# RolandFaure/Hairsplitter

Hardware: AMD Instinct MI355X
Metric: aligned read-bp/sec through call_variants+separate_reads (higher is better)
Workload: dtype u8

## Files before the change

hairsplitter_amd/csrc/hs_driver.cpp:

```cpp
#include "hs_driver.h"

#include <sys/prctl.h>
#include <algorithm>
#include <atomic>
#include <chrono>
#include <ctime>
#include <cstdio>
#include <cstdlib>
#include <cstring>
#include <fstream>
#include <iostream>
#include <sstream>
#include <condition_variable>
#include <functional>
#include <mutex>
#include <thread>

namespace hs {

int host_threads();

namespace {

double now_ms() {
    return std::chrono::duration<double, std::milli>(std::chrono::steady_clock::now().time_since_epoch()).count();
}

class WorkerPool {
public:
    static WorkerPool& get() { static thread_local WorkerPool* p = new WorkerPool(); return *p; }
    void run(int n, int n_threads, const std::function<void(int)>& f) {
        if (n <= 0) return;
        if (n_threads <= 1 || n == 1) { for (int i = 0; i < n; ++i) f(i); return; }
        std::lock_guard<std::mutex> serial(run_mu_);
        ensure(std::min(n_threads, n) - 1);
        {
            std::lock_guard<std::mutex> g(mu_);
            job_ = &f; n_ = n; next_.store(0); active_ = std::min((int)workers_.size(), std::min(n_threads, n) - 1); pending_ = active_; gen_++;
            grain_ = std::max(1, n / (8 * (active_ + 1)));
        }
        cv_.notify_all();
        const int grain = grain_;
        for (;;) { const int i = next_.fetch_add(grain); if (i >= n) break; for (int k = i; k < std::min(n, i + grain); ++k) f(k); }
        std::unique_lock<std::mutex> g(mu_);
        done_cv_.wait(g, [&] { return pending_ == 0; });
        job_ = nullptr;
    }
private:
    void ensure(int want) {
        want = std::min(want, 255);
        while ((int)workers_.size() < want) {
            const int id = (int)workers_.size();
            workers_.emplace_back([this, id] { ::prctl(PR_SET_NAME, "hs-pool", 0, 0, 0); loop(id); });
            workers_.back().detach();
        }
    }
    void loop(int id) {
        uint64_t seen = 0;
        for (;;) {
            const std::function<void(int)>* job; int n, grain;
            {
                std::unique_lock<std::mutex> g(mu_);
                cv_.wait(g, [&] { return gen_ != seen && id < active_; });
                seen = gen_; job = job_; n = n_; grain = grain_;
            }
            for (;;) { const int i = next_.fetch_add(grain); if (i >= n) break; for (int k = i; k < std::min(n, i + grain); ++k) (*job)(k); }
            {
                std::lock_guard<std::mutex> g(mu_);
                if (--pending_ == 0) done_cv_.notify_one();
            }
        }
    }
    std::mutex mu_, run_mu_;
    std::condition_variable cv_, done_cv_;
    std::vector<std::thread> workers_;
    const std::function<void(int)>* job_ = nullptr;
    std::atomic<int> next_{0};
    int n_ = 0, active_ = 0, pending_ = 0, grain_ = 1;
    uint64_t gen_ = 0;
};

class SharedPool {
public:
    static SharedPool& get() { static SharedPool* p = new SharedPool(); return *p; }
    static bool on() { static const bool v = []() { const char* e = std::getenv("HS_SHARED_POOL"); return e && e[0] == '1'; }(); return v; }
    void run(int n, int n_threads, const std::function<void(int)>& f) {
        if (n <= 0) return;
        if (n_threads <= 1 || n == 1) { for (int i = 0; i < n; ++i) f(i); return; }
        Job job;
        job.f = &f; job.n = n;
        {
            std::lock_guard<std::mutex> g(mu_);
            ensure();
            job.grain = std::max(1, n / (8 * (std::min(n_threads, (int)workers_.size() + 1))));
            jobs_.push_back(&job);
        }
        cv_.notify_all();
        for (;;) { const int i = job.next.fetch_add(job.grain); if (i >= n) break; const int e = std::min(n, i + job.grain); for (int k = i; k < e; ++k) f(k); job.done.fetch_add(e - i); }
        std::unique_lock<std::mutex> g(mu_);
        jobs_.erase(std::find(jobs_.begin(), jobs_.end(), &job));
        done_cv_.wait(g, [&] { return job.done.load() >= n; });
    }
private:
    struct Job { const std::function<void(int)>* f = nullptr; int n = 0, grain = 1; std::atomic<int> next{0}, done{0}; };
    void ensure() {
        static const int want = []() { const char* e = std::getenv("HS_POOL_THREADS"); const int v = e ? std::atoi(e) : 0; return v > 0 ? v : host_threads(); }();
        while ((int)workers_.size() < want) { workers_.emplace_back([this] { ::prctl(PR_SET_NAME, "hs-spool", 0, 0, 0); loop(); }); workers_.back().detach(); }
    }
    void loop() {
        std::unique_lock<std::mutex> g(mu_);
        for (;;) {
            Job* job = nullptr;
            for (Job* j : jobs_) if (j->next.load(std::memory_order_relaxed) < j->n) { job = j; break; }
            if (!job) { cv_.wait(g); continue; }
            const int i = job->next.fetch_add(job->grain);
            if (i >= job->n) continue;
            const int n = job->n, e = std::min(n, i + job->grain);
            const std::function<void(int)>* f = job->f;
            g.unlock();
            for (int k = i; k < e; ++k) (*f)(k);
            const bool last = job->done.fetch_add(e - i) + (e - i) >= n;
            g.lock();
            if (last) done_cv_.notify_all();
        }
    }
    std::mutex mu_;
    std::condition_variable cv_, done_cv_;
    std::vector<std::thread> workers_;
    std::vector<Job*> jobs_;
};

template <class F>
void parallel_for(int n, int n_threads, F f) {
    std::function<void(int)> fn = f;
    if (SharedPool::on()) SharedPool::get().run(n, n_threads, fn); else WorkerPool::get().run(n, n_threads, fn);
}

template <class T> T* dup_vec(const std::vector<T>& v) {
    T* p = (T*)std::malloc(std::max<size_t>(1, v.size()) * sizeof(T));
    if (!v.empty()) std::memcpy(p, v.data(), v.size() * sizeof(T));
    return p;
}

}

void hs_parallel_for(int n, int n_threads, const std::function<void(int)>& f) { if (SharedPool::on()) SharedPool::get().run(n, n_threads, f); else WorkerPool::get().run(n, n_threads, f); }

int host_threads() {
    static const int n = [] {
        long q = -1, per = 100000;
        if (FILE* f = std::fopen("/sys/fs/cgroup/cpu.max", "r")) { char a[32]; if (std::fscanf(f, "%31s %ld", a, &per) == 2 && std::strcmp(a, "max") != 0) q = std::atol(a); std::fclose(f); }
        int t = (int)std::thread::hardware_concurrency();
        if (q > 0 && per > 0) t = std::min<int>(t, (int)((q + per - 1) / per));
        return std::max(1, std::min(t, 32));
    }();
    return n;
}

void free_cv_result(hs_cv_result* r) {
    if (!r) return;
    std::free(r->mean_distance); std::free(r->depth); std::free(r->snp_off); std::free(r->snp_pos); std::free(r->snp_ref);
    std::free(r->snp_alt); std::free(r->snp_n_ref); std::free(r->snp_n_alt); std::free(r->col_off);
    if (!r->entries_borrowed) { std::free(r->col_idx); std::free(r->col_code); }
    std::free(r);
}
namespace {
struct LabelBlockHeader { uint64_t magic; size_t cap; char pad[48]; };
constexpr uint64_t kLabelMagic = 0x48534c4142454c53ull;
constexpr size_t kLabelKeepMin = 8u << 20, kLabelKeepBlocks = 4;
std::mutex g_label_mu;
std::vector<LabelBlockHeader*> g_label_free;
}

int32_t* sr_labels_alloc(size_t n_labels) {
    const size_t need = std::max<size_t>(1, n_labels) * sizeof(int32_t);
    {
        std::lock_guard<std::mutex> g(g_label_mu);
        for (size_t i = 0; i < g_label_free.size(); ++i) {
            LabelBlockHeader* h = g_label_free[i];
            if (h->cap >= need && h->cap / 2 <= need) { g_label_free.erase(g_label_free.begin() + (long)i); return (int32_t*)(h + 1); }
        }
    }
    const size_t cap = need >= kLabelKeepMin ? need + need / 8 : need;
    LabelBlockHeader* h = (LabelBlockHeader*)std::malloc(sizeof(LabelBlockHeader) + cap);
    if (!h) return nullptr;
    h->magic = kLabelMagic; h->cap = cap;
    return (int32_t*)(h + 1);
}

void sr_labels_free(int32_t* labels) {
    if (!labels) return;
    LabelBlockHeader* h = (LabelBlockHeader*)labels - 1;
    if (h->magic != kLabelMagic) { std::free(labels); return; }
    if (h->cap >= kLabelKeepMin) {
        std::lock_guard<std::mutex> g(g_label_mu);
        if (g_label_free.size() < kLabelKeepBlocks) { g_label_free.push_back(h); return; }
    }
    std::free(h);
}

void free_sr_result(hs_sr_result* r) {
    if (!r) return;
    std::free(r->win_off); std::free(r->win_start); std::free(r->win_end); std::free(r->label_off); sr_labels_free(r->labels);
    std::free(r);
}

static std::atomic<double> g_trace_origin{0.0};
void set_trace_origin() { g_trace_origin.store(std::chrono::duration<double, std::milli>(std::chrono::steady_clock::now().time_since_epoch()).count()); }
double trace_ms() { return std::chrono::duration<double, std::milli>(std::chrono::steady_clock::now().time_since_epoch()).count() - g_trace_origin.load(); }
namespace {
struct Laps {
    bool on = std::getenv("HS_TIMING") != nullptr;
    bool cpu = on && std::string(std::getenv("HS_TIMING")) == "cpu";
    bool abs_ = on && std::string(std::getenv("HS_TIMING")) == "abs";
    double t = now_ms(), c = cpu_ms();
    std::string line;
    const char* tag;
    explicit Laps(const char* t_) : tag(t_) {}
    static double cpu_ms() { timespec ts; clock_gettime(CLOCK_THREAD_CPUTIME_ID, &ts); return ts.tv_sec * 1e3 + ts.tv_nsec * 1e-6; }
    void lap(const char* what) {
        if (!on) return;
        const double n = now_ms();
        char buf[96];
        if (abs_) std::snprintf(buf, sizeof buf, " %s @%.2f", what, n - g_trace_origin.load());
        else if (cpu) { const double cn = cpu_ms(); std::snprintf(buf, sizeof buf, " %s %.2f/%.2f", what, n - t, cn - c); c = cn; }
        else std::snprintf(buf, sizeof buf, " %s %.2f", what, n - t);
        line += buf; t = n;
    }
    ~Laps() { if (on) std::fprintf(stderr, "[hs timing] %s laps (ms) thread %zu:%s\n", tag, std::hash<std::thread::id>()(std::this_thread::get_id()) % 1000, line.c_str()); }
};
}

int cv_pileup(CvDeviceOps& dev, const CvMeta& b, CvSelection& sel) {
    const double t_start = now_ms();
    for (int k = 0; k < 4; ++k) sel.k_ms[k] = 0;
    sel.rec_stats.assign((size_t)b.n_rec * 4, 0);
    if (int rc = dev.pileup(sel.rec_stats, sel.k_ms)) return rc;
    sel.t_device_ms = now_ms() - t_start; sel.t_host_ms = 0;
    return HS_OK;
}

int cv_run_range(CvDeviceOps& dev, const CvMeta& b, const std::vector<int32_t>& rec_stats, int c0, int c1, float automatic_snp_threshold, int n_threads,
                 hs_cv_result** out, bool resident, const std::function<void(const float*)>* on_mean_distance) {
    if (n_threads <= 0) n_threads = host_threads();
    if (c0 < 0 || c1 > b.n_contigs || c0 > c1) { set_error("cv_run_range: bad contig range"); return HS_EINVAL; }
    const int C = c1 - c0;
    const double t_start = now_ms();
    float k_ms[4] = {0, 0, 0, 0};
    float k_ms_k4 = 0;
    std::vector<ContigCvResult> res((size_t)C);
    const bool derive = rec_stats.empty() && b.n_rec > 0;
    std::vector<int32_t> min_reads((size_t)(derive ? 0 : C), 5);
    for (int c = 0; c < C; ++c) {
        const int gc = c0 + c;
        ContigCvResult& o = res[(size_t)c];
        if (!derive) {
            int64_t nerr = 0, nlen = 0;
            for (int r = b.contig_rec_off[(size_t)gc]; r < b.contig_rec_off[(size_t)gc + 1]; ++r) { nerr += rec_stats[(size_t)r * 4 + 1]; nlen += rec_stats[(size_t)r * 4 + 2]; }
            o.mean_distance = mean_distance_from_counts(nerr, nlen);
            min_reads[(size_t)c] = o.mean_distance < 0.015 ? 3 : 5;
        }
        const int64_t L = b.contig_off[(size_t)gc + 1] - b.contig_off[(size_t)gc];
        const int64_t entries = b.pile_off[(size_t)b.contig_rec_off[(size_t)gc + 1]] - b.pile_off[(size_t)b.contig_rec_off[(size_t)gc]];
        o.depth = (float)((double)entries / (double)L);
    }
    CvCandidates cand;
    float k_ms_x[3] = {0, 0, 0};
    if (int rc = dev.extract_candidates(c0, c1, min_reads, automatic_snp_threshold, cand, k_ms_x, true)) return rc;
    k_ms[1] = k_ms_x[0]; k_ms[2] = k_ms_x[1] + k_ms_x[2];
    if (derive) {
        if ((int)cand.contig_mean_distance.size() != C) { set_error("cv_run_range: the device interface did not report the contigs' mean distances"); return HS_EINVAL; }
        for (int c = 0; c < C; ++c) res[(size_t)c].mean_distance = cand.contig_mean_distance[(size_t)c];
    }
    if (on_mean_distance) { std::vector<float> md((size_t)C); for (int c = 0; c < C; ++c) md[(size_t)c] = res[(size_t)c].mean_distance; (*on_mean_distance)(md.data()); }
    const double t_dev_done = now_ms();
    Laps laps("cv glue");
    std::vector<int64_t> cand_base((size_t)C + 1, 0);
    for (int c = 0; c < C; ++c) cand_base[(size_t)c + 1] = cand_base[(size_t)c] + cand.contig_n_cand[(size_t)c];
    if (cand_base[(size_t)C] != cand.n_cand) { set_error("cv_run_range: candidate counts do not add up"); return HS_EINVAL; }

    std::vector<CvContigState*> cst((size_t)C, nullptr);
    for (int c = 0; c < C; ++c) cst[(size_t)c] = cv_state_new();
    std::vector<int32_t> n_reads_of((size_t)C);
    parallel_for(C, n_threads, [&](int c) {
        const int gc = c0 + c;
        const int r0 = b.contig_rec_off[(size_t)gc];
        const int n_reads_c = b.contig_rec_off[(size_t)gc + 1] - r0;
        n_reads_of[(size_t)c] = n_reads_c;
        cv_phase_begin(*cst[(size_t)c], n_reads_c, cand.contig_n_cand[(size_t)c], res[(size_t)c].mean_distance, res[(size_t)c]);
    });
    laps.lap("begin");
    const bool some_on_device = (int)cand.contig_on_device.size() == C;
    auto on_device = [&](int c) { return some_on_device && cand.contig_on_device[(size_t)c] != 0; };
    bool host_has_bits = cand.bits != nullptr || cand.n_cand == 0;
    auto candidates_of = [&](int c) {
        CandidateSet cs;
        cs.n = cand.contig_n_cand[(size_t)c];
        cs.rec = cand.rec + cand_base[(size_t)c]; cs.bits = cand.bits + cand_base[(size_t)c]; cs.words = cand.words;
        if (cand.idx) { cs.off = cand.off + cand_base[(size_t)c]; cs.idx = cand.idx; cs.code = cand.code; }
        return cs;
    };
    static const bool loop_b_pairs = []() { const char* e = std::getenv("HS_LOOP_B_PAIRS_ON_DEVICE"); return e && e[0] != '0'; }();
    const bool pairs_on_device = loop_b_pairs && dev.has_partition_pairs();
    const bool ranked = (int)b.rank_of.size() == b.n_rec && (int)b.orig_of.size() == b.n_rec;
    auto walk_on_host = [&](int c) {
        const int r0 = b.contig_rec_off[(size_t)(c0 + c)];
        cv_phase_a_host(*cst[(size_t)c], candidates_of(c), b.rec_pos.data() + r0, ranked ? b.rank_of.data() + r0 : nullptr, ranked ? b.orig_of.data() + r0 : nullptr);
        if (!pairs_on_device) cv_phase_b(*cst[(size_t)c], res[(size_t)c]);
    };
    std::vector<int> host_list, dev_list;
    for (int c = 0; c < C; ++c) (on_device(c) ? dev_list : host_list).push_back(c);
    std::stable_sort(host_list.begin(), host_list.end(), [&](int x, int y) { return cand.contig_n_cand[(size_t)x] > cand.contig_n_cand[(size_t)y]; });
    if (!host_list.empty() && !host_has_bits) { set_error("cv_run_range: the device interface handed no bit sets of the candidate columns"); return HS_EINVAL; }
    parallel_for((int)host_list.size(), n_threads, [&](int k) { walk_on_host(host_list[(size_t)k]); });
    laps.lap("loop_a_host");
    int n_dev_failed = 0;
    if (!dev_list.empty()) {
        CvLoopAResult la;
        if (int rc = dev.collect_partitions(la)) return rc;
        if ((int)la.failed.size() != C || (int)la.part_base.size() != C + 1) { set_error("cv_run_range: the device interface did not hand over the partitions of its contigs"); return HS_EINVAL; }
        laps.lap("loop_a_device");
        std::vector<int> redo;
        for (int c : dev_list) if (la.failed[(size_t)c]) redo.push_back(c);
        n_dev_failed = (int)redo.size();
        if (!redo.empty()) {
            if (int rc = dev.fetch_candidates(cand)) return rc;
            if (cand.n_cand > 0 && !cand.bits) { set_error("cv_run_range: the device interface handed no bit sets of the candidate columns"); return HS_EINVAL; }
        }
        std::stable_sort(dev_list.begin(), dev_list.end(), [&](int x, int y) { return cand.contig_n_cand[(size_t)x] > cand.contig_n_cand[(size_t)y]; });
        parallel_for((int)dev_list.size(), n_threads, [&](int k) {
            const int c = dev_list[(size_t)k];
            if (la.failed[(size_t)c]) { walk_on_host(c); return; }
            const int r0 = b.contig_rec_off[(size_t)(c0 + c)];
            cv_phase_a_import(*cst[(size_t)c], b.rec_pos.data() + r0, (int)(la.part_base[(size_t)c + 1] - la.part_base[(size_t)c]), la.rec + la.part_base[(size_t)c], la.bits, la.cnt,
                              ranked ? b.rank_of.data() + r0 : nullptr, ranked ? b.orig_of.data() + r0 : nullptr);
            if (!pairs_on_device) cv_phase_b(*cst[(size_t)c], res[(size_t)c]);
        });
    }
    if (pairs_on_device) {
        std::vector<int32_t> n_surv((size_t)C, 0);
        parallel_for(C, n_threads, [&](int c) { n_surv[(size_t)c] = cv_loop_b_survivors(*cst[(size_t)c]); });
        std::vector<int64_t> part_first((size_t)C + 1, 0), elem_first((size_t)C + 1, 0), pair_first((size_t)C + 1, 0);
        for (int c = 0; c < C; ++c) {
            part_first[(size_t)c + 1] = part_first[(size_t)c] + n_surv[(size_t)c];
            elem_first[(size_t)c + 1] = elem_first[(size_t)c] + (int64_t)n_surv[(size_t)c] * n_reads_of[(size_t)c];
            pair_first[(size_t)c + 1] = pair_first[(size_t)c] + (int64_t)n_surv[(size_t)c] * (n_surv[(size_t)c] - 1) / 2;
        }
        std::vector<int8_t> pstate((size_t)elem_first[(size_t)C]);
        std::vector<int32_t> pmore((size_t)elem_first[(size_t)C]), pless((size_t)elem_first[(size_t)C]), part_n((size_t)part_first[(size_t)C]);
        std::vector<int64_t> part_off((size_t)part_first[(size_t)C]);
        std::vector<int32_t> pair_a((size_t)pair_first[(size_t)C]), pair_b((size_t)pair_first[(size_t)C]);
        parallel_for(C, n_threads, [&](int c) {
            const int S = n_surv[(size_t)c], N = n_reads_of[(size_t)c];
            cv_export_survivors(*cst[(size_t)c], pstate.data() + elem_first[(size_t)c], pmore.data() + elem_first[(size_t)c], pless.data() + elem_first[(size_t)c]);
            for (int k = 0; k < S; ++k) { part_off[(size_t)part_first[(size_t)c] + k] = elem_first[(size_t)c] + (int64_t)k * N; part_n[(size_t)part_first[(size_t)c] + k] = N; }
            int64_t q = pair_first[(size_t)c];
            for (int j = 1; j < S; ++j) for (int i = 0; i < j; ++i, ++q) { pair_a[(size_t)q] = (int32_t)(part_first[(size_t)c] + i); pair_b[(size_t)q] = (int32_t)(part_first[(size_t)c] + j); }
        });
        std::vector<int32_t> table;
        if (int rc = dev.partition_pairs(pstate, pmore, pless, part_off, part_n, pair_a, pair_b, cv_three_sigma_table(), table)) return rc;
        parallel_for(C, n_threads, [&](int c) { cv_phase_b(*cst[(size_t)c], res[(size_t)c], table.data() + 8 * pair_first[(size_t)c]); });
        if (std::getenv("HS_TIMING")) std::fprintf(stderr, "[hs timing] cv loop B: %ld partition pairs of %ld gated partitions from the device\n", (long)pair_first[(size_t)C], (long)part_first[(size_t)C]);
    }
    if (std::getenv("HS_TIMING") && !dev_list.empty()) std::fprintf(stderr, "[hs timing] cv loop A: %zu of %d contigs on the device (%d handed back), %zu on the host\n", dev_list.size(), C, n_dev_failed, host_list.size());
    laps.lap("phase_ab");
    CvSnpSet snps;
    {
        CvPartitionTest t;
        t.part_off.assign((size_t)C + 1, 0);
        t.contig_n_reads.resize((size_t)C);
        std::vector<int64_t> st_base((size_t)C + 1, 0);
        for (int c = 0; c < C; ++c) {
            t.contig_n_reads[(size_t)c] = b.contig_rec_off[(size_t)(c0 + c) + 1] - b.contig_rec_off[(size_t)(c0 + c)];
            const int nf = cv_final_partitions(*cst[(size_t)c]);
            t.part_off[(size_t)c + 1] = t.part_off[(size_t)c] + nf;
            st_base[(size_t)c + 1] = st_base[(size_t)c] + (int64_t)nf * t.contig_n_reads[(size_t)c];
        }
        t.part_state.resize((size_t)st_base[(size_t)C]); t.part_state_off.resize((size_t)t.part_off[(size_t)C]);
        parallel_for(C, n_threads, [&](int c) {
            cv_export_partitions(*cst[(size_t)c], t.part_state.data() + st_base[(size_t)c], st_base[(size_t)c], t.part_state_off.data() + t.part_off[(size_t)c]);
            cv_state_free(cst[(size_t)c]);
        });
        laps.lap("k4_prep");
        if (int rc = dev.finish_columns(t, !resident, snps, &k_ms_k4)) return rc;
        laps.lap("k4+snps");
    }
    const double t_glue_done = now_ms();

    hs_cv_result* R = (hs_cv_result*)std::calloc(1, sizeof(hs_cv_result));
    R->n_contigs = C;
    std::vector<float> md((size_t)C), dp((size_t)C);
    std::vector<int64_t> snp_off((size_t)C + 1, 0);
    float total_error = 0; int n_err_contigs = 0;
    for (int c = 0; c < C; ++c) {
        md[(size_t)c] = res[(size_t)c].mean_distance; dp[(size_t)c] = res[(size_t)c].depth;
        if (res[(size_t)c].mean_distance > 0) { total_error += res[(size_t)c].mean_distance; n_err_contigs++; }
        snp_off[(size_t)c + 1] = snp_off[(size_t)c] + snps.contig_n_snp[(size_t)c];
    }
    const int64_t S = snps.n_snp, E = snps.n_entries;
    if (snp_off[(size_t)C] != S) { set_error("cv_run_range: SNP counts do not add up"); return HS_EINVAL; }
    R->snp_pos = (int32_t*)std::malloc(std::max<int64_t>(1, S) * sizeof(int32_t));
    R->snp_ref = (uint8_t*)std::malloc(std::max<int64_t>(1, S));
    R->snp_alt = (uint8_t*)std::malloc(std::max<int64_t>(1, S));
    R->snp_n_ref = (int32_t*)std::malloc(std::max<int64_t>(1, S) * sizeof(int32_t));
    R->snp_n_alt = (int32_t*)std::malloc(std::max<int64_t>(1, S) * sizeof(int32_t));
    R->col_off = (int64_t*)std::malloc((S + 1) * sizeof(int64_t));
    const bool with_entries = snps.idx != nullptr || E == 0;
    R->col_idx = with_entries ? (int32_t*)std::malloc(std::max<int64_t>(1, E) * sizeof(int32_t)) : nullptr;
    R->col_code = with_entries ? (uint8_t*)std::malloc(std::max<int64_t>(1, E)) : nullptr;
    R->n_columns_extracted = cand.n_columns;
    R->n_columns_downloaded = cand.n_cand;
    R->n_columns_downloaded_late = cand.n_tie;
    {
        const int nb = (int)std::min<int64_t>(std::max<int64_t>(1, S / 4096), 4 * (int64_t)n_threads);
        parallel_for(nb, n_threads, [&](int blk) {
            const int64_t a = S * blk / nb, e = S * (blk + 1) / nb;
            for (int64_t s = a; s < e; ++s) {
                const hs_colrec& r = snps.rec[s];
                R->snp_pos[s] = r.pos; R->snp_ref[s] = r.k0; R->snp_alt[s] = r.k1; R->snp_n_ref[s] = r.c0; R->snp_n_alt[s] = r.c1;
            }
            if (S) std::memcpy(R->col_off + a, snps.off + a, (size_t)(e - a) * sizeof(int64_t));
            if (with_entries && e > a) {
                const int64_t ea = snps.off[a], ee = snps.off[e];
                std::memcpy(R->col_idx + ea, snps.idx + ea, (size_t)(ee - ea) * sizeof(int32_t));
                std::memcpy(R->col_code + ea, snps.code + ea, (size_t)(ee - ea));
            }
        });
        R->col_off[S] = E;
        if (S == 0) R->col_off[0] = 0;
    }
    laps.lap("result");
    R->mean_distance = dup_vec(md); R->depth = dup_vec(dp); R->snp_off = dup_vec(snp_off);
    R->error_rate = total_error / n_err_contigs;
    R->n_contigs_with_error_rate = n_err_contigs;
    R->t_kernel_ms[0] = k_ms[0]; R->t_kernel_ms[1] = k_ms[1]; R->t_kernel_ms[2] = k_ms[2]; R->t_kernel_ms[3] = k_ms[3]; R->t_kernel_k4_ms = k_ms_k4;
    R->t_device_ms = t_dev_done - t_start;
    R->t_host_ms = now_ms() - t_dev_done;
    if (std::getenv("HS_TIMING"))
        std::fprintf(stderr, "[hs timing] cv range [%d,%d): columns + candidates %.2f ms, host glue %.2f ms (up to the SNPs %.2f); columns: %lld extracted, %lld candidates, %lld with tied counts (%lld beyond 16 keys), %lld SNPs\n",
                     c0, c1, t_dev_done - t_start, R->t_host_ms, t_glue_done - t_dev_done, (long long)cand.n_columns,
                     (long long)cand.n_cand, (long long)cand.n_tie, (long long)cand.n_tie_big, (long long)S);
    *out = R;
    return HS_OK;
}


int cv_attach_entries(CvDeviceOps& dev, hs_cv_result* R, int n_threads, bool borrow) {
    if (!R || R->col_idx) return HS_OK;
    const int64_t S = R->snp_off[R->n_contigs], E = R->col_off[S];
    CvSnpSet snps;
    if (int rc = dev.late_entries(snps)) return rc;
    if (E > 0 && (!snps.idx || !snps.code)) return HS_OK;
    if (borrow && E > 0) {
        R->col_idx = const_cast<int32_t*>(snps.idx); R->col_code = const_cast<uint8_t*>(snps.code); R->entries_borrowed = 1;
        return HS_OK;
    }
    R->col_idx = (int32_t*)std::malloc(std::max<int64_t>(1, E) * sizeof(int32_t));
    R->col_code = (uint8_t*)std::malloc(std::max<int64_t>(1, E));
    if (n_threads <= 0) n_threads = host_threads();
    const int nb = (int)std::min<int64_t>(std::max<int64_t>(1, E >> 20), 4 * (int64_t)n_threads);
    parallel_for(nb, n_threads, [&](int blk) {
        const int64_t a = E * blk / nb, e = E * (blk + 1) / nb;
        if (e > a) { std::memcpy(R->col_idx + a, snps.idx + a, (size_t)(e - a) * sizeof(int32_t)); std::memcpy(R->col_code + a, snps.code + a, (size_t)(e - a)); }
    });
    return HS_OK;
}

hs_cv_result* cv_concat_results(hs_cv_result* a, hs_cv_result* b) {
    hs_cv_result* R = (hs_cv_result*)std::calloc(1, sizeof(hs_cv_result));
    const int Ca = a->n_contigs, Cb = b->n_contigs, C = Ca + Cb;
    const int64_t Sa = a->snp_off[Ca], Sb = b->snp_off[Cb], S = Sa + Sb;
    const int64_t Ea = a->col_off[Sa], Eb = b->col_off[Sb], E = Ea + Eb;
    R->n_contigs = C;
    R->mean_distance = (float*)std::malloc(std::max(1, C) * sizeof(float)); R->depth = (float*)std::malloc(std::max(1, C) * sizeof(float));
    R->snp_off = (int64_t*)std::malloc(((size_t)C + 1) * sizeof(int64_t));
    R->snp_pos = (int32_t*)std::malloc(std::max<int64_t>(1, S) * sizeof(int32_t));
    R->snp_ref = (uint8_t*)std::malloc(std::max<int64_t>(1, S)); R->snp_alt = (uint8_t*)std::malloc(std::max<int64_t>(1, S));
    R->snp_n_ref = (int32_t*)std::malloc(std::max<int64_t>(1, S) * sizeof(int32_t)); R->snp_n_alt = (int32_t*)std::malloc(std::max<int64_t>(1, S) * sizeof(int32_t));
    R->col_off = (int64_t*)std::malloc(((size_t)S + 1) * sizeof(int64_t));
    const bool with_entries = (a->col_idx || Ea == 0) && (b->col_idx || Eb == 0);
    R->col_idx = with_entries ? (int32_t*)std::malloc(std::max<int64_t>(1, E) * sizeof(int32_t)) : nullptr;
    R->col_code = with_entries ? (uint8_t*)std::malloc(std::max<int64_t>(1, E)) : nullptr;
    float total_error = 0; int n_err = 0;
    auto put = [&](const hs_cv_result* r, int cbase, int64_t sbase, int64_t ebase) {
        const int Cr = r->n_contigs; const int64_t Sr = r->snp_off[Cr], Er = r->col_off[Sr];
        for (int c = 0; c < Cr; ++c) {
            R->mean_distance[cbase + c] = r->mean_distance[c]; R->depth[cbase + c] = r->depth[c];
            if (r->mean_distance[c] > 0) { total_error += r->mean_distance[c]; n_err++; }
            R->snp_off[cbase + c] = sbase + r->snp_off[c];
        }
        if (Sr) {
            std::memcpy(R->snp_pos + sbase, r->snp_pos, (size_t)Sr * sizeof(int32_t)); std::memcpy(R->snp_ref + sbase, r->snp_ref, (size_t)Sr); std::memcpy(R->snp_alt + sbase, r->snp_alt, (size_t)Sr);
            std::memcpy(R->snp_n_ref + sbase, r->snp_n_ref, (size_t)Sr * sizeof(int32_t)); std::memcpy(R->snp_n_alt + sbase, r->snp_n_alt, (size_t)Sr * sizeof(int32_t));
        }
        for (int64_t q = 0; q < Sr; ++q) R->col_off[sbase + q] = ebase + r->col_off[q];
        if (with_entries && Er) { std::memcpy(R->col_idx + ebase, r->col_idx, (size_t)Er * sizeof(int32_t)); std::memcpy(R->col_code + ebase, r->col_code, (size_t)Er); }
        R->t_device_ms += r->t_device_ms; R->t_host_ms += r->t_host_ms;
        for (int k = 0; k < 4; ++k) R->t_kernel_ms[k] += r->t_kernel_ms[k];
        R->t_kernel_k4_ms += r->t_kernel_k4_ms;
        R->n_columns_extracted += r->n_columns_extracted; R->n_columns_downloaded += r->n_columns_downloaded; R->n_columns_downloaded_late += r->n_columns_downloaded_late;
    };
    put(a, 0, 0, 0); put(b, Ca, Sa, Ea);
    R->snp_off[C] = S; R->col_off[S] = E;
    R->error_rate = total_error / n_err; R->n_contigs_with_error_rate = n_err;
    free_cv_result(a); free_cv_result(b);
    return R;
}

int cv_run(CvDeviceOps& dev, const CvMeta& b, float automatic_snp_threshold, int n_threads, hs_cv_result** out) {
    CvSelection sel;
    if (int rc = cv_pileup(dev, b, sel)) return rc;
    if (int rc = cv_run_range(dev, b, sel.rec_stats, 0, b.n_contigs, automatic_snp_threshold, n_threads, out)) return rc;
    hs_cv_result* R = *out;
    R->t_kernel_ms[0] = sel.k_ms[0]; R->t_kernel_ms[3] = sel.k_ms[3];
    R->t_device_ms += sel.t_device_ms; R->t_host_ms += sel.t_host_ms;
    return HS_OK;
}

int sr_run(SrDeviceOps& dev, const hs_sr_contig* contigs, int32_t n_contigs, int32_t window_size, float error_rate,
           int32_t low_memory, uint32_t seed, int32_t n_threads, hs_sr_result** out, SrSparseLabels* sparse, SrWorkspace* keep, SrTaps* taps) {
    Laps laps("sr");
    if (n_threads <= 0) n_threads = host_threads();
    const int C = n_contigs;
    const bool lowmem = low_memory != 0;
    const double t_start = now_ms();
    double dev_ms = 0;
    float k_ms[4] = {0, 0, 0, 0};

    const bool resident = dev.columns_resident();
    std::vector<hs_sr_contig> cs_local(contigs, contigs + C);
    std::vector<SrContigState> st_local;
    if (keep) keep->st.resize((size_t)C); else st_local.resize((size_t)C);
    std::vector<SrContigState>& st = keep ? keep->st : st_local;
    parallel_for(C, n_threads, [&](int c) {
        SrContigState& s = st[(size_t)c];
        s.c = &cs_local[(size_t)c];
        s.N = contigs[c].n_reads;
        s.low_memory_now = lowmem || sr_coverage_above_1000(contigs[c]);
        if (contigs[c].n_snps == 0) { for (SrWindowPlan& old : s.windows) s.spare.push_back(std::move(old)); s.windows.clear(); return; }
        s.words = (contigs[c].n_snps + 63) / 64;
        if (!s.low_memory_now && ((int)s.pos_key.size() != s.N || std::memcmp(s.pos_key.data(), contigs[c].read_start, (size_t)s.N * 4) != 0)) {
            s.pos_key.assign(contigs[c].read_start, contigs[c].read_start + s.N);
            s.pos_orig.resize((size_t)s.N); s.pos_rank.resize((size_t)s.N);
            for (int k = 0; k < s.N; ++k) s.pos_orig[(size_t)k] = k;
            const int32_t* st0 = contigs[c].read_start;
            std::sort(s.pos_orig.begin(), s.pos_orig.end(), [st0](int32_t a, int32_t b2) { return st0[a] != st0[b2] ? st0[a] < st0[b2] : a < b2; });
            for (int k = 0; k < s.N; ++k) s.pos_rank[(size_t)s.pos_orig[(size_t)k]] = k;
        }
        if (s.perm_n != s.N || s.perm_seed != seed) {
            s.perm = shuffled_order(s.N, seed);
            s.rank.resize((size_t)s.N);
            for (int k = 0; k < s.N; ++k) s.rank[(size_t)s.perm[(size_t)k]] = k;
            s.perm_n = s.N; s.perm_seed = seed;
        }
    });

    laps.lap("perm");
    const bool lm_on_device = dev.low_memory_graphs();
    bool matrices_by_position = false;
    CwChain ch;
    std::vector<int64_t> col_base_of_contig((size_t)C, 0);
    {
        SimdiffJob job;
        job.cols = &ch;
        job.contig_snp_base.assign((size_t)C, 0); job.plane_off.assign((size_t)C, 0); job.out_off.assign((size_t)C, 0);
        job.n_reads.assign((size_t)C, 0); job.words.assign((size_t)C, 0); job.plane_n.assign((size_t)C, 0); job.read_base.assign((size_t)C, 0);
        int64_t n_ent = 0, n_col = 0;
        for (int c = 0; c < C; ++c) { n_col += contigs[c].n_snps; if (contigs[c].n_snps) n_ent += contigs[c].col_off[contigs[c].n_snps] - contigs[c].col_off[0]; }
        bool contiguous = n_col > 0;
        {
            const int64_t* off_next = nullptr; const int32_t* idx0 = nullptr; const uint8_t* code0 = nullptr;
            bool first = true;
            for (int c = 0; c < C && contiguous; ++c) {
                const hs_sr_contig& hc = contigs[c];
                if (hc.n_snps == 0) continue;
                if (first) { first = false; idx0 = hc.col_idx; code0 = hc.col_code; if (hc.col_off[0] != 0) contiguous = false; }
                else if (hc.col_idx != idx0 || hc.col_code != code0 || hc.col_off != off_next) contiguous = false;
                off_next = hc.col_off + hc.n_snps;
            }
        }
        if (resident && n_col > 0 && !contiguous) { set_error("sr_run: resident columns need one offset array in contig order"); return HS_EINVAL; }
        int64_t* own_off = nullptr; int32_t* own_idx = nullptr; uint8_t* own_code = nullptr;
        if (contiguous) {
            const hs_sr_contig* first = nullptr;
            for (int c = 0; c < C && !first; ++c) if (contigs[c].n_snps) first = &contigs[c];
            ch.col_off.view(first->col_off, (size_t)n_col + 1);
            if (!resident) { ch.col_idx.view(first->col_idx, (size_t)n_ent); ch.col_code.view(first->col_code, (size_t)n_ent); }
        } else {
            own_off = ch.col_off.alloc((size_t)n_col + 1); own_idx = ch.col_idx.alloc((size_t)n_ent); own_code = ch.col_code.alloc((size_t)n_ent);
            own_off[0] = 0;
        }
        job.snp_ref.resize((size_t)n_col); job.snp_alt.resize((size_t)n_col); job.snp_contig.resize((size_t)n_col);
        std::vector<int64_t> ent_base_of_contig((size_t)C, 0);
        {
            int64_t cb = 0, eb = 0, rows_total = 0;
            for (int c = 0; c < C; ++c) {
                col_base_of_contig[(size_t)c] = cb; ent_base_of_contig[(size_t)c] = eb;
                job.contig_snp_base[(size_t)c] = cb;
                const hs_sr_contig& hc = contigs[c];
                if (hc.n_snps == 0) continue;
                cb += hc.n_snps; eb += hc.col_off[hc.n_snps] - hc.col_off[0];
                if (st[(size_t)c].low_memory_now && !lm_on_device) continue;
                job.plane_off[(size_t)c] = job.plane_total; job.words[(size_t)c] = st[(size_t)c].words; job.plane_n[(size_t)c] = st[(size_t)c].N;
                job.plane_total += (int64_t)st[(size_t)c].N * st[(size_t)c].words;
                job.read_base[(size_t)c] = rows_total; rows_total += st[(size_t)c].N;
                if (st[(size_t)c].low_memory_now) continue;
                job.out_off[(size_t)c] = job.out_total;
                job.n_reads[(size_t)c] = st[(size_t)c].N;
                job.out_total += (int64_t)st[(size_t)c].N * st[(size_t)c].N;
            }
        }
        {
            const bool read_order = false;
            int64_t rows_all = 0;
            for (int c = 0; c < C; ++c) rows_all = std::max<int64_t>(rows_all, job.read_base[(size_t)c] + job.plane_n[(size_t)c]);
            if (!read_order) job.pos_orig.assign((size_t)rows_all, 0);
            if (!read_order) for (int c = 0; c < C; ++c) if (job.plane_n[(size_t)c] > 0 && job.n_reads[(size_t)c] == 0)
                for (int k = 0; k < job.plane_n[(size_t)c]; ++k) job.pos_orig[(size_t)(job.read_base[(size_t)c] + k)] = k;
        }
        parallel_for(C, n_threads, [&](int c) {
            const hs_sr_contig& hc = contigs[c];
            if (hc.n_snps == 0) return;
            const int64_t cb = col_base_of_contig[(size_t)c], e_base = ent_base_of_contig[(size_t)c], o0 = hc.col_off[0];
            if (!contiguous) {
                for (int s = 0; s < hc.n_snps; ++s) own_off[(size_t)(cb + s) + 1] = e_base + hc.col_off[s + 1] - o0;
                const int64_t n = hc.col_off[hc.n_snps] - o0;
                std::memcpy(own_idx + e_base, hc.col_idx + o0, (size_t)n * sizeof(int32_t));
                std::memcpy(own_code + e_base, hc.col_code + o0, (size_t)n);
            }
            if (!job.pos_orig.empty() && job.n_reads[(size_t)c] > 0) {
                if ((int)st[(size_t)c].pos_orig.size() == st[(size_t)c].N) std::memcpy(job.pos_orig.data() + job.read_base[(size_t)c], st[(size_t)c].pos_orig.data(), (size_t)st[(size_t)c].N * 4);
                else for (int k = 0; k < st[(size_t)c].N; ++k) job.pos_orig[(size_t)(job.read_base[(size_t)c] + k)] = k;
            }
            std::memcpy(job.snp_ref.data() + cb, hc.snp_ref, (size_t)hc.n_snps);
            std::memcpy(job.snp_alt.data() + cb, hc.snp_alt, (size_t)hc.n_snps);
            std::fill(job.snp_contig.begin() + cb, job.snp_contig.begin() + cb + hc.n_snps, c);
        });
        laps.lap("columns");
        matrices_by_position = !job.pos_orig.empty();
        const double t0 = now_ms();
        if (int rc = dev.simdiff_columns(job, &k_ms[0])) return rc;
        dev_ms += now_ms() - t0;
    }

    const double t_simdiff_done = now_ms();
    laps.lap("simdiff");
    std::vector<int32_t> fetched_idx; std::vector<uint8_t> fetched_code;
    bool columns_here = !resident;
    auto need_columns = [&]() -> int {
        if (columns_here) return HS_OK;
        const double t0 = now_ms();
        if (int rc = dev.fetch_columns(fetched_idx, fetched_code)) return rc;
        dev_ms += now_ms() - t0;
        for (int c = 0; c < C; ++c) { cs_local[(size_t)c].col_idx = fetched_idx.data(); cs_local[(size_t)c].col_code = fetched_code.data(); }
        ch.col_idx.view(fetched_idx.data(), fetched_idx.size()); ch.col_code.view(fetched_code.data(), fetched_code.size());
        columns_here = true;
        return HS_OK;
    };
    parallel_for(C, n_threads, [&](int c) {
        if (contigs[c].n_snps == 0) return;
        sr_plan_windows(st[(size_t)c], window_size, error_rate, lowmem, !resident);
    });
    laps.lap("plan_windows");
    if (resident) {
        struct WR { int c, w; };
        std::vector<WR> wr;
        for (int c = 0; c < C; ++c)
            for (size_t w = 0; w < st[(size_t)c].windows.size(); ++w) if (st[(size_t)c].windows[w].has_snps) wr.push_back(WR{c, (int)w});
        const size_t W = wr.size();
        std::vector<int64_t> col_a(W), col_b(W), slot_off(W + 1, 0);
        for (size_t i = 0; i < W; ++i) {
            const SrWindowPlan& wp = st[(size_t)wr[i].c].windows[(size_t)wr[i].w];
            col_a[i] = col_base_of_contig[(size_t)wr[i].c] + wp.col_a; col_b[i] = col_base_of_contig[(size_t)wr[i].c] + wp.col_b;
            slot_off[i + 1] = slot_off[i] + (ch.col_off[(size_t)col_a[i] + 1] - ch.col_off[(size_t)col_a[i]]);
        }
        std::vector<int32_t> ids, win_m;
        if (W) {
            const double t0 = now_ms();
            if (int rc = dev.window_masks(col_a, col_b, slot_off, ids, win_m)) return rc;
            dev_ms += now_ms() - t0;
        }
        parallel_for((int)W, n_threads, [&](int i) {
            SrWindowPlan& wp = st[(size_t)wr[(size_t)i].c].windows[(size_t)wr[(size_t)i].w];
            wp.ids.assign(ids.begin() + slot_off[(size_t)i], ids.begin() + slot_off[(size_t)i] + win_m[(size_t)i]);
        });
        laps.lap("window_masks");
    }
    struct WRef { int c, w; };
    std::vector<WRef> wrefs;
    SrWindowSet ws;
    ws.error_rate = error_rate;
    {
        std::vector<uint8_t> lm_dev((size_t)C, 0);
        bool any_lm = false;
        for (int c = 0; c < C; ++c) if (contigs[c].n_snps > 0 && st[(size_t)c].low_memory_now) any_lm = true;
        if (any_lm && lm_on_device) {
            if (int rc = need_columns()) return rc;
            parallel_for(C, n_threads, [&](int c) {
                const hs_sr_contig& hc = cs_local[(size_t)c];
                if (hc.n_snps == 0 || !st[(size_t)c].low_memory_now) return;
                std::vector<int32_t> first((size_t)st[(size_t)c].N, -1), last((size_t)st[(size_t)c].N, -1), cnt((size_t)st[(size_t)c].N, 0);
                for (int s = 0; s < hc.n_snps; ++s)
                    for (int64_t e = hc.col_off[s]; e < hc.col_off[s + 1]; ++e) {
                        const int r = hc.col_idx[e];
                        if (first[(size_t)r] < 0) first[(size_t)r] = s;
                        last[(size_t)r] = s; cnt[(size_t)r]++;
                    }
                bool ok = true;
                for (int r = 0; r < st[(size_t)c].N && ok; ++r) if (cnt[(size_t)r] > 0 && cnt[(size_t)r] != last[(size_t)r] - first[(size_t)r] + 1) ok = false;
                lm_dev[(size_t)c] = ok ? 1 : 0;
            });
        }
        if (any_lm && std::getenv("HS_TIMING")) {
            int n_lm = 0, n_ok = 0;
            for (int c = 0; c < C; ++c) if (contigs[c].n_snps > 0 && st[(size_t)c].low_memory_now) { n_lm++; n_ok += lm_dev[(size_t)c]; }
            std::fprintf(stderr, "[hs timing] sr: %d contigs on the low-memory path, %d of them with graphs from the device\n", n_lm, n_ok);
        }
        std::vector<WRef> lm_w, host_w;
        for (int c = 0; c < C; ++c)
            for (size_t w = 0; w < st[(size_t)c].windows.size(); ++w) {
                if (!st[(size_t)c].windows[w].has_snps) continue;
                (!st[(size_t)c].low_memory_now ? wrefs : (lm_dev[(size_t)c] ? lm_w : host_w)).push_back(WRef{c, (int)w});
            }
        ws.n_matrix_windows = (int32_t)wrefs.size();
        wrefs.insert(wrefs.end(), lm_w.begin(), lm_w.end());
        ws.n_dev_windows = (int32_t)wrefs.size();
        wrefs.insert(wrefs.end(), host_w.begin(), host_w.end());
        ws.ctg_reads.resize((size_t)C);
        for (int c = 0; c < C; ++c) ws.ctg_reads[(size_t)c] = st[(size_t)c].N;
        const size_t W = wrefs.size();
        ws.win_contig.resize(W); ws.win_row0.assign(W + 1, 0); ws.win_final_empty.resize(W);
        for (size_t i = 0; i < W; ++i) {
            SrWindowPlan& wp = st[(size_t)wrefs[i].c].windows[(size_t)wrefs[i].w];
            wp.row0 = ws.win_row0[i];
            ws.win_contig[i] = wrefs[i].c;
            ws.win_final_empty[i] = wp.final_graph_empty ? 1 : 0;
            ws.win_row0[i + 1] = ws.win_row0[i] + (int64_t)wp.ids.size();
        }
        ws.mask_ids.resize((size_t)ws.win_row0[W]);
        parallel_for((int)W, n_threads, [&](int i) {
            const SrWindowPlan& wp = st[(size_t)wrefs[(size_t)i].c].windows[(size_t)wrefs[(size_t)i].w];
            std::copy(wp.ids.begin(), wp.ids.end(), ws.mask_ids.begin() + ws.win_row0[(size_t)i]);
        });
        ws.ctg_rank_off.assign((size_t)C, 0);
        int64_t ro = 0;
        for (int c = 0; c < C; ++c) { ws.ctg_rank_off[(size_t)c] = ro; ro += (int64_t)st[(size_t)c].rank.size(); }
        ws.rank.resize((size_t)ro);
        parallel_for(C, n_threads, [&](int c) { std::copy(st[(size_t)c].rank.begin(), st[(size_t)c].rank.end(), ws.rank.begin() + ws.ctg_rank_off[(size_t)c]); });
        if (matrices_by_position) {
            ws.pos_rank.assign((size_t)ro, 0);
            parallel_for(C, n_threads, [&](int c) {
                const SrContigState& s = st[(size_t)c];
                if (s.rank.empty()) return;
                int32_t* o = ws.pos_rank.data() + ws.ctg_rank_off[(size_t)c];
                if (!s.low_memory_now && (int)s.pos_rank.size() == s.N) std::copy(s.pos_rank.begin(), s.pos_rank.end(), o);
                else for (int k = 0; k < (int)s.rank.size(); ++k) o[k] = k;
            });
        }
        const int n_host = (int)host_w.size();
        if (n_host > 0) {
            if (int rc = need_columns()) return rc;
            std::vector<std::vector<std::vector<int32_t>>> lists((size_t)n_host);
            parallel_for(n_host, n_threads, [&](int i) {
                const WRef& r = wrefs[(size_t)ws.n_dev_windows + (size_t)i];
                sr_build_window_graph_low_memory(st[(size_t)r.c], st[(size_t)r.c].windows[(size_t)r.w], error_rate, lists[(size_t)i]);
            });
            ws.host_off.assign(1, 0);
            for (auto& wl : lists)
                for (auto& row : wl) { ws.host_nbr.insert(ws.host_nbr.end(), row.begin(), row.end()); ws.host_off.push_back((int64_t)ws.host_nbr.size()); }
        }
    }
    laps.lap("window_set");
    int64_t rows_on_host = 0, n_finish_host = 0;
    float k6_ms = 0;
    const bool two_phase = !wrefs.empty() && dev.two_phase_graphs();
    if (!wrefs.empty()) {
        const double t0 = now_ms();
        if (two_phase) { if (int rc = dev.build_graphs_begin(ws, &k6_ms)) return rc; }
        else if (int rc = dev.build_graphs(ws, &rows_on_host, &k6_ms)) return rc;
        dev_ms += now_ms() - t0;
    }
    const double t_plan_done = now_ms();
    laps.lap("build_graphs");

    int64_t n_cw = 0;
    std::vector<int64_t> chain_index(wrefs.size(), -1);
    {
        ch.win_seed_begin.assign(1, 0);
        ch.chain_row0.assign(1, 0);
        ch.finish_on_device = !lowmem;
        for (int c = 0; c < C && ch.finish_on_device; ++c)
            if (contigs[c].n_snps > 0 && !st[(size_t)c].snp_pos_sorted) ch.finish_on_device = false;
        if (ch.finish_on_device) {
            ch.col_pos.reserve(ch.col_off.size());
            for (int c = 0; c < C; ++c) ch.col_pos.insert(ch.col_pos.end(), contigs[c].snp_pos, contigs[c].snp_pos + contigs[c].n_snps);
        }
        for (size_t i = 0; i < wrefs.size(); ++i) {
            const SrWindowPlan& w = st[(size_t)wrefs[i].c].windows[(size_t)wrefs[i].w];
            if (w.local_snps.empty()) continue;
            chain_index[i] = (int64_t)ch.win.size();
            ch.win.push_back((int32_t)i);
            ch.win_seed_begin.push_back(ch.win_seed_begin.back() + (int64_t)w.local_snps.size());
            ch.chain_row0.push_back(ch.chain_row0.back() + (int64_t)w.ids.size());
            n_cw += (int64_t)w.local_snps.size() + 2;
        }
        const size_t Wc = ch.win.size();
        ch.seed_col.resize((size_t)ch.win_seed_begin.back());
        if (ch.finish_on_device) { ch.win_snp_first.resize(Wc); ch.win_snp_last.resize(Wc); ch.win_pos_lo.resize(Wc); ch.win_pos_hi.resize(Wc); }
        parallel_for((int)Wc, n_threads, [&](int k) {
            const size_t i = (size_t)ch.win[(size_t)k];
            const SrWindowPlan& w = st[(size_t)wrefs[i].c].windows[(size_t)wrefs[i].w];
            const int64_t base = col_base_of_contig[(size_t)wrefs[i].c];
            int64_t at = ch.win_seed_begin[(size_t)k];
            for (int snp : w.local_snps) ch.seed_col[(size_t)at++] = base + snp;
            if (ch.finish_on_device) {
                const hs_sr_contig& hc = contigs[wrefs[i].c];
                ch.win_snp_first[(size_t)k] = base + (std::lower_bound(hc.snp_pos, hc.snp_pos + hc.n_snps, w.final_lo) - hc.snp_pos);
                ch.win_snp_last[(size_t)k] = base + (std::lower_bound(hc.snp_pos, hc.snp_pos + hc.n_snps, w.final_hi) - hc.snp_pos);
                ch.win_pos_lo[(size_t)k] = w.final_lo; ch.win_pos_hi[(size_t)k] = w.final_hi;
            }
        });
    }
    laps.lap("chain_build");
    if (two_phase) {
        const double t0 = now_ms();
        if (int rc = dev.build_graphs_end(ws, &rows_on_host)) return rc;
        dev_ms += now_ms() - t0;
        laps.lap("graphs_end");
    }
    std::vector<int32_t> chain_labels, final_labels;
    std::vector<uint8_t> final_ok;
    SrChainStats cst;
    {
        const double t0 = now_ms();
        if (taps) dev.tap_chain(&taps->run_off, &taps->run_labels);
        if (!ch.win.empty()) { if (int rc = dev.cw_chain(ch, chain_labels, final_labels, final_ok, &k_ms[1], &cst)) return rc; }
        dev_ms += now_ms() - t0;
    }
    if (taps) {
        dev.tap_chain(nullptr, nullptr);
        taps->win_row0.assign(1, 0); taps->run_begin.assign(1, 0);
        for (size_t k = 0; k < ch.win.size(); ++k) {
            const WRef& wr = wrefs[(size_t)ch.win[k]];
            const SrWindowPlan& w = st[(size_t)wr.c].windows[(size_t)wr.w];
            taps->win_contig.push_back(wr.c); taps->win_start.push_back(w.start);
            taps->mask_ids.insert(taps->mask_ids.end(), w.ids.begin(), w.ids.end());
            taps->win_row0.push_back((int64_t)taps->mask_ids.size());
            for (int snp : w.local_snps) taps->run_snp.push_back(snp);
            taps->run_begin.push_back((int64_t)taps->run_snp.size());
        }
        taps->third = chain_labels;
    }

    const double t_waves_done = now_ms();
    laps.lap("cw_chain");
    std::vector<int64_t> g_off; std::vector<int32_t> g_nbr;
    bool graphs_here = false;
    auto need_graphs = [&]() -> int {
        if (graphs_here) return HS_OK;
        const double t0 = now_ms();
        if (int rc = dev.fetch_graphs(g_off, g_nbr)) return rc;
        dev_ms += now_ms() - t0;
        graphs_here = true;
        return HS_OK;
    };
    {
        bool any_host = false;
        for (size_t i = 0; i < wrefs.size() && !any_host; ++i)
            if (chain_index[i] >= 0 && (final_ok.empty() || !final_ok[(size_t)chain_index[i]])) any_host = true;
        if (any_host) { if (int rc = need_graphs()) return rc; if (int rc = need_columns()) return rc; }
    }
    parallel_for((int)wrefs.size(), n_threads, [&](int i) {
        SrContigState& s = st[(size_t)wrefs[(size_t)i].c];
        SrWindowPlan& w = s.windows[(size_t)wrefs[(size_t)i].w];
        const int64_t k = chain_index[(size_t)i];
        if (k < 0) w.labels.assign(w.ids.size(), -1);
        else if (!final_ok.empty() && final_ok[(size_t)k]) {
            const int32_t* f = final_labels.data() + ch.chain_row0[(size_t)k];
            w.labels.assign(f, f + w.ids.size());
        } else {
            SrLocalGraph g; g.off = g_off.data() + w.row0; g.nbr = g_nbr.data();
            sr_finish_window(s, w, chain_labels.data() + ch.chain_row0[(size_t)k], g, lowmem);
        }
    });
    for (size_t i = 0; i < wrefs.size(); ++i)
        if (chain_index[i] >= 0 && (final_ok.empty() || !final_ok[(size_t)chain_index[i]])) n_finish_host++;

    const double t_finish_done = now_ms();
    laps.lap("finish");
    {
        CwWave w4;
        std::vector<size_t> who;
        for (size_t i = 0; i < wrefs.size(); ++i) {
            SrContigState& s = st[(size_t)wrefs[i].c];
            SrWindowPlan& w = s.windows[(size_t)wrefs[i].w];
            if (contigs[wrefs[i].c].ploidy <= 0) continue;
            std::vector<int32_t> init(w.ids.size());
            if (!sr_ploidy_init_labels(w, contigs[wrefs[i].c].ploidy, init.data())) continue;
            who.push_back(i);
            w4.inst_win.push_back((int32_t)i);
            w4.inst_label_off.push_back((int64_t)w4.labels.size());
            w4.labels.insert(w4.labels.end(), init.begin(), init.end());
        }
        if (!w4.inst_win.empty()) {
            const double t0 = now_ms();
            if (int rc = dev.cw(w4, &k_ms[3])) return rc;
            n_cw += (int64_t)w4.inst_win.size();
            dev_ms += now_ms() - t0;
        }
        for (size_t k = 0; k < who.size(); ++k) {
            SrWindowPlan& w = st[(size_t)wrefs[who[k]].c].windows[(size_t)wrefs[who[k]].w];
            w.labels.assign(w4.labels.begin() + w4.inst_label_off[k], w4.labels.begin() + w4.inst_label_off[k] + (int64_t)w.ids.size());
        }
    }

    hs_sr_result* R = (hs_sr_result*)std::calloc(1, sizeof(hs_sr_result));
    R->n_contigs = C;
    std::vector<int64_t> win_off((size_t)C + 1, 0), label_off(1, 0);
    std::vector<int32_t> ws_, we_;
    std::vector<const SrWindowPlan*> wl;
    for (int c = 0; c < C; ++c) {
        for (auto& w : st[(size_t)c].windows) {
            ws_.push_back(w.start); we_.push_back(w.end);
            wl.push_back(&w);
            label_off.push_back(label_off.back() + (int64_t)st[(size_t)c].N);
        }
        win_off[(size_t)c + 1] = (int64_t)ws_.size();
    }
    R->win_off = dup_vec(win_off); R->win_start = dup_vec(ws_); R->win_end = dup_vec(we_); R->label_off = dup_vec(label_off);
    if (sparse) {
        sparse->off.assign(wl.size() + 1, 0);
        for (size_t i = 0; i < wl.size(); ++i) sparse->off[i + 1] = sparse->off[i] + (int64_t)wl[i]->ids.size();
        sparse->ids.resize((size_t)sparse->off.back()); sparse->labels.resize((size_t)sparse->off.back());
        parallel_for((int)wl.size(), n_threads, [&](int i) {
            const SrWindowPlan& w = *wl[(size_t)i];
            std::copy(w.ids.begin(), w.ids.end(), sparse->ids.begin() + sparse->off[(size_t)i]);
            std::copy(w.labels.begin(), w.labels.end(), sparse->labels.begin() + sparse->off[(size_t)i]);
        });
        R->labels = nullptr;
    } else {
        R->labels = sr_labels_alloc((size_t)label_off.back());
        parallel_for((int)wl.size(), n_threads, [&](int i) {
            int32_t* o = R->labels + label_off[(size_t)i];
            const int64_t n = label_off[(size_t)i + 1] - label_off[(size_t)i];
            std::fill(o, o + n, -2);
            const SrWindowPlan& w = *wl[(size_t)i];
            for (size_t j = 0; j < w.ids.size(); ++j) o[w.ids[j]] = w.labels[j];
        });
    }
    laps.lap("result");
    R->n_cw_instances = n_cw;
    R->t_kernel_graph_ms = k6_ms; R->n_graph_rows_host = rows_on_host; R->n_windows_finished_on_host = n_finish_host;
    R->n_cw_sweeps = cst.sweeps; R->cw_bytes = cst.bytes; R->graph_nnz = cst.graph_nnz; R->n_graph_rows = ws.rows();
    for (int c = 0; c < C; ++c)
        if (contigs[c].n_snps > 0 && !st[(size_t)c].low_memory_now)
            R->simdiff_bytes += (int64_t)st[(size_t)c].N * contigs[c].n_snps / 4 + 16 * (int64_t)st[(size_t)c].N * st[(size_t)c].N;
    for (int k = 0; k < 4; ++k) R->t_kernel_ms[k] = k_ms[k];
    R->t_device_ms = dev_ms;
    R->t_host_ms = (now_ms() - t_start) - dev_ms;
    if (std::getenv("HS_TIMING"))
        std::fprintf(stderr, "[hs timing] sr: graph rows resolved by std::sort on the host: %ld, k_read_graph_rows %.3f ms; windows finished on the host: %ld of %zu\n",
                     (long)rows_on_host, k6_ms, (long)n_finish_host, ch.win.size());
    if (std::getenv("HS_TIMING"))
        std::fprintf(stderr, "[hs timing] sr: planes+simdiff %.2f ms, plan windows+graphs %.2f ms, clustering chain %.2f ms, finish %.2f ms, total %.2f ms (device %.2f)\n",
                     t_simdiff_done - t_start, t_plan_done - t_simdiff_done, t_waves_done - t_plan_done, t_finish_done - t_waves_done, now_ms() - t_start, dev_ms);
    *out = R;
    return HS_OK;
}

void sr_expand_labels(const SrSparseLabels& sp, const int64_t* label_off, int64_t w0, int64_t w1, int32_t* dense) {
    for (int64_t w = w0; w < w1; ++w) {
        int32_t* o = dense + (label_off[w] - label_off[0]);
        std::fill(o, o + (label_off[w + 1] - label_off[w]), -2);
        for (int64_t e = sp.off[(size_t)w]; e < sp.off[(size_t)w + 1]; ++e) o[sp.ids[(size_t)e]] = sp.labels[(size_t)e];
    }
}

int sr_run_from_cv(SrDeviceOps& dev, const CvMeta& b, int c0, int c1, const hs_cv_result* cv, float error_rate, float rsa, int32_t low_memory,
                   int32_t amplicon, uint32_t seed, int32_t n_threads, int32_t window_size, hs_sr_result** out, SrSparseLabels* sparse, SrWorkspace* keep) {
    if (c0 < 0 || c1 > b.n_contigs || c0 > c1 || cv->n_contigs != c1 - c0) { set_error("sr_run_from_cv: contig range does not match the stage-3 result"); return HS_EINVAL; }
    const int C = c1 - c0;
    const double t_prep0 = now_ms();
    std::vector<int32_t> fetched_idx; std::vector<uint8_t> fetched_code;
    const int32_t* cv_idx = cv->col_idx; const uint8_t* cv_code = cv->col_code;
    const bool have_snps = cv->snp_off[C] > 0 && cv->col_off[cv->snp_off[C]] > 0;
    const bool resident_in = have_snps && (cv->col_idx == nullptr || dev.columns_resident());
    if (resident_in && !dev.columns_resident()) { set_error("sr_run_from_cv: the stage-3 result has no columns and the device has none either"); return HS_EINVAL; }
    if (resident_in) {
        bool all = true;
        for (int64_t s = 0; s < cv->snp_off[C] && all; ++s)
            if (!((float)cv->snp_n_alt[s] >= rsa * (float)(cv->snp_n_ref[s] + cv->snp_n_alt[s]))) all = false;
        if (!all) {
            if (int rc = dev.fetch_columns(fetched_idx, fetched_code)) return rc;
            dev.drop_resident_columns();
            cv_idx = fetched_idx.data(); cv_code = fetched_code.data();
        }
    } else if (dev.columns_resident()) dev.drop_resident_columns();
    std::vector<hs_sr_contig> hc((size_t)C);
    std::vector<std::vector<int32_t>> rs((size_t)C), re((size_t)C), spos((size_t)C);
    std::vector<std::vector<uint8_t>> sref((size_t)C), salt((size_t)C);
    std::vector<std::vector<int64_t>> coff((size_t)C);
    if (n_threads <= 0) n_threads = host_threads();
    parallel_for(C, n_threads, [&](int c) {
        const int gc = c0 + c;
        const int r0 = b.contig_rec_off[(size_t)gc], r1 = b.contig_rec_off[(size_t)gc + 1];
        rs[(size_t)c].resize((size_t)(r1 - r0)); re[(size_t)c].resize((size_t)(r1 - r0));
        for (int r = r0; r < r1; ++r) {
            rs[(size_t)c][(size_t)(r - r0)] = b.rec_pos[(size_t)r];
            re[(size_t)c][(size_t)(r - r0)] = (int32_t)(b.rec_pos[(size_t)r] + 1 + b.rec_refspan[(size_t)r]);
        }
        const int64_t s0 = cv->snp_off[c], s1 = cv->snp_off[c + 1];
        bool all_kept = true;
        std::vector<char> keep((size_t)(s1 - s0), 1);
        for (int64_t s = s0; s < s1; ++s) {
            int maj = 0, sec = 0;
            if (cv->snp_n_ref && cv->snp_n_alt) { maj = cv->snp_n_ref[s]; sec = cv->snp_n_alt[s]; }
            else for (int64_t e = cv->col_off[s]; e < cv->col_off[s + 1]; ++e) { if (cv_code[e] == cv->snp_ref[s]) maj++; else if (cv_code[e] == cv->snp_alt[s]) sec++; }
            if (!((float)sec >= rsa * (float)(maj + sec))) { keep[(size_t)(s - s0)] = 0; all_kept = false; }
        }
        hs_sr_contig& h = hc[(size_t)c];
        h.length = b.contig_off[(size_t)gc + 1] - b.contig_off[(size_t)gc];
        h.n_reads = r1 - r0; h.read_start = rs[(size_t)c].data(); h.read_end = re[(size_t)c].data();
        h.col_idx = cv_idx; h.col_code = cv_code; h.ploidy = b.ploidy.empty() ? 0 : b.ploidy[(size_t)gc];
        if (all_kept) {
            h.n_snps = (int32_t)(s1 - s0); h.snp_pos = cv->snp_pos + s0; h.snp_ref = cv->snp_ref + s0; h.snp_alt = cv->snp_alt + s0;
            h.col_off = cv->col_off + s0;
        } else {
            coff[(size_t)c].assign(1, 0);
            for (int64_t s = s0; s < s1; ++s) {
                if (!keep[(size_t)(s - s0)]) continue;
                spos[(size_t)c].push_back(cv->snp_pos[s]); sref[(size_t)c].push_back(cv->snp_ref[s]); salt[(size_t)c].push_back(cv->snp_alt[s]);
            }
            h.n_snps = -1;
        }
    });
    std::vector<std::vector<int32_t>> cidx((size_t)C);
    std::vector<std::vector<uint8_t>> ccode((size_t)C);
    for (int c = 0; c < C; ++c) {
        hs_sr_contig& h = hc[(size_t)c];
        if (h.n_snps != -1) continue;
        size_t k = 0;
        for (int64_t s = cv->snp_off[c]; s < cv->snp_off[c + 1]; ++s) {
            if (k < spos[(size_t)c].size() && cv->snp_pos[s] == spos[(size_t)c][k]) {
                cidx[(size_t)c].insert(cidx[(size_t)c].end(), cv_idx + cv->col_off[s], cv_idx + cv->col_off[s + 1]);
                ccode[(size_t)c].insert(ccode[(size_t)c].end(), cv_code + cv->col_off[s], cv_code + cv->col_off[s + 1]);
                coff[(size_t)c].push_back((int64_t)cidx[(size_t)c].size());
                k++;
            }
        }
        h.n_snps = (int32_t)spos[(size_t)c].size(); h.snp_pos = spos[(size_t)c].data(); h.snp_ref = sref[(size_t)c].data(); h.snp_alt = salt[(size_t)c].data();
        h.col_off = coff[(size_t)c].data(); h.col_idx = cidx[(size_t)c].data(); h.col_code = ccode[(size_t)c].data();
    }
    if (std::getenv("HS_TIMING")) std::fprintf(stderr, "[hs timing] sr hand-over from stage 3: %.2f ms\n", now_ms() - t_prep0);
    const int32_t w = window_size > 0 ? window_size : sr_window_size(hc.data(), C, amplicon != 0);
    return sr_run(dev, hc.data(), C, w, error_rate, low_memory, seed, n_threads, out, sparse, keep);
}

}
```

hairsplitter_amd/csrc/hs_driver.h:

```cpp
#pragma once
#include <cstdint>
#include <functional>
#include <vector>
#include "hs_host.h"
#include "hs_host_sr.h"

namespace hs {

struct CvMeta {
    int32_t n_contigs = 0, n_rec = 0;
    std::vector<int64_t> contig_off;
    std::vector<int32_t> contig_rec_off;
    std::vector<int64_t> pile_off;
    std::vector<int32_t> rec_pos;
    std::vector<int64_t> rec_refspan;
    int64_t total_len = 0;
    std::vector<int32_t> ploidy;
    std::vector<int32_t> rank_of, orig_of;
};

struct CvPartitionTest {
    std::vector<int32_t> contig_n_reads;
    std::vector<int32_t> part_off;
    std::vector<int64_t> part_state_off;
    std::vector<int8_t> part_state;
};

struct CvCandidates {
    int64_t n_columns = 0, n_entries = 0;
    int64_t n_tie = 0, n_tie_big = 0;
    std::vector<int32_t> contig_n_cand;
    std::vector<float> contig_mean_distance;
    int64_t n_cand = 0;
    const hs_colrec* rec = nullptr;
    const int32_t* col = nullptr;
    const int64_t* off = nullptr;
    const int32_t* idx = nullptr;
    const uint8_t* code = nullptr;
    const CandBits* bits = nullptr;
    const uint64_t* words = nullptr;
    std::vector<uint8_t> contig_on_device;
};
struct CvSnpSet {
    std::vector<int32_t> contig_n_snp;
    int64_t n_snp = 0, n_entries = 0;
    const hs_colrec* rec = nullptr;
    const int64_t* off = nullptr;
    const int32_t* idx = nullptr;
    const uint8_t* code = nullptr;
};

struct CvLoopAResult {
    std::vector<uint8_t> on_device;
    std::vector<int32_t> failed;
    std::vector<int64_t> part_base;
    const CvPartRecord* rec = nullptr;
    const uint64_t* bits = nullptr;
    const int32_t* cnt = nullptr;
};

struct CvDeviceOps {
    virtual ~CvDeviceOps() {}
    virtual int pileup(std::vector<int32_t>& rec_stats, float k_ms[4]) = 0;
    virtual int extract_candidates(int c0, int c1, const std::vector<int32_t>& min_reads, float automatic_snp_threshold, CvCandidates& out,
                                   float k_ms[3], bool want_entries = true) = 0;
    virtual int fetch_candidates(CvCandidates& out) { (void)out; return -1; }
    virtual int finish_columns(const CvPartitionTest& t, bool want_entries, CvSnpSet& out, float* k_ms) = 0;
    virtual int late_entries(CvSnpSet& out) { (void)out; return 0; }
    virtual bool has_partition_pairs() const { return false; }
    virtual int partition_pairs(const std::vector<int8_t>& state, const std::vector<int32_t>& more, const std::vector<int32_t>& less, const std::vector<int64_t>& part_off,
                                const std::vector<int32_t>& part_n, const std::vector<int32_t>& pair_a, const std::vector<int32_t>& pair_b, const std::vector<float>& sigma3,
                                std::vector<int32_t>& out) { (void)state; (void)more; (void)less; (void)part_off; (void)part_n; (void)pair_a; (void)pair_b; (void)sigma3; (void)out; return -1; }
    virtual int collect_partitions(CvLoopAResult& out) { out = CvLoopAResult(); return 0; }
};

struct CvSelection {
    std::vector<int32_t> rec_stats;
    float k_ms[4] = {0, 0, 0, 0};
    double t_device_ms = 0, t_host_ms = 0;
};
int cv_pileup(CvDeviceOps& dev, const CvMeta& meta, CvSelection& sel);
int cv_run_range(CvDeviceOps& dev, const CvMeta& meta, const std::vector<int32_t>& rec_stats, int c0, int c1, float automatic_snp_threshold, int n_threads,
                 hs_cv_result** out, bool resident = false, const std::function<void(const float*)>* on_mean_distance = nullptr);
int cv_run(CvDeviceOps& dev, const CvMeta& meta, float automatic_snp_threshold, int n_threads, hs_cv_result** out);
hs_cv_result* cv_concat_results(hs_cv_result* a, hs_cv_result* b);
int cv_attach_entries(CvDeviceOps& dev, hs_cv_result* r, int n_threads, bool borrow = false);

struct SrWindowSet {
    std::vector<int32_t> win_contig;
    std::vector<int64_t> win_row0;
    std::vector<int32_t> mask_ids;
    int32_t n_dev_windows = 0;
    int32_t n_matrix_windows = 0;
    std::vector<int32_t> ctg_reads;
    std::vector<int64_t> host_off;
    std::vector<int32_t> host_nbr;
    std::vector<uint8_t> win_final_empty;
    std::vector<int32_t> rank;
    std::vector<int32_t> pos_rank;
    std::vector<int64_t> ctg_rank_off;
    float error_rate = 0;
    int64_t rows() const { return win_row0.empty() ? 0 : win_row0.back(); }
};

template <class T> struct ArrayView {
    const T* p = nullptr;
    size_t n = 0;
    std::vector<T> own;
    void view(const T* ptr, size_t count) { own.clear(); p = ptr; n = count; }
    T* alloc(size_t count) { own.resize(count); p = own.data(); n = count; return own.data(); }
    const T* data() const { return p; }
    size_t size() const { return n; }
    const T& operator[](size_t i) const { return p[i]; }
};

struct CwChain {
    ArrayView<int64_t> col_off;
    ArrayView<int32_t> col_idx;
    ArrayView<uint8_t> col_code;
    std::vector<int32_t> win;
    std::vector<int64_t> chain_row0;
    std::vector<int64_t> win_seed_begin;
    std::vector<int64_t> seed_col;
    bool finish_on_device = false;
    std::vector<int32_t> col_pos;
    std::vector<int64_t> win_snp_first, win_snp_last;
    std::vector<int32_t> win_pos_lo, win_pos_hi;
};

struct CwWave {
    std::vector<int32_t> inst_win;
    std::vector<int64_t> inst_label_off;
    std::vector<int32_t> labels;
};

struct SimdiffJob {
    const CwChain* cols = nullptr;
    std::vector<uint8_t> snp_ref, snp_alt;
    std::vector<int32_t> snp_contig;
    std::vector<int64_t> contig_snp_base;
    std::vector<int64_t> plane_off, out_off;
    std::vector<int32_t> n_reads, words;
    std::vector<int32_t> plane_n;
    int64_t plane_total = 0, out_total = 0;
    std::vector<int32_t> pos_orig;
    std::vector<int64_t> read_base;
};

struct SrChainStats {
    int64_t n_instances = 0;
    int64_t sweeps = 0;
    int64_t bytes = 0;
    int64_t graph_nnz = 0;
};

struct SrDeviceOps {
    virtual ~SrDeviceOps() {}
    virtual int simdiff_columns(const SimdiffJob& job, float* k_ms) = 0;
    virtual int build_graphs(const SrWindowSet& ws, int64_t* rows_on_host, float* k_ms) = 0;
    virtual bool two_phase_graphs() const { return false; }
    virtual int build_graphs_begin(const SrWindowSet& ws, float* k_ms) { (void)ws; (void)k_ms; return -1; }
    virtual int build_graphs_end(const SrWindowSet& ws, int64_t* rows_on_host) { (void)ws; (void)rows_on_host; return -1; }
    virtual int fetch_graphs(std::vector<int64_t>& off, std::vector<int32_t>& nbr) = 0;
    virtual int cw_chain(const CwChain& chain, std::vector<int32_t>& labels, std::vector<int32_t>& final_labels,
                         std::vector<uint8_t>& final_ok, float k_ms[3], SrChainStats* stats) = 0;
    virtual int cw(CwWave& wave, float* k_ms) = 0;
    virtual void tap_chain(std::vector<int64_t>* run_off, std::vector<int32_t>* run_labels) { (void)run_off; (void)run_labels; }
    virtual bool low_memory_graphs() const { return false; }
    virtual bool columns_resident() const { return false; }
    virtual void drop_resident_columns() {}
    virtual int window_masks(const std::vector<int64_t>& col_a, const std::vector<int64_t>& col_b, const std::vector<int64_t>& slot_off,
                             std::vector<int32_t>& ids, std::vector<int32_t>& win_m) { (void)col_a; (void)col_b; (void)slot_off; (void)ids; (void)win_m; return -1; }
    virtual int fetch_columns(std::vector<int32_t>& idx, std::vector<uint8_t>& code) { (void)idx; (void)code; return -1; }
};

void set_trace_origin();
double trace_ms();
int host_threads();

struct SrSparseLabels {
    std::vector<int64_t> off;
    std::vector<int32_t> ids, labels;
};
struct SrWorkspace { std::vector<SrContigState> st; };
struct SrTaps {
    std::vector<int32_t> win_contig, win_start;
    std::vector<int64_t> win_row0;
    std::vector<int32_t> mask_ids;
    std::vector<int64_t> run_begin;
    std::vector<int32_t> run_snp;
    std::vector<int64_t> run_off;
    std::vector<int32_t> run_labels, third;
};
int sr_run(SrDeviceOps& dev, const hs_sr_contig* contigs, int32_t n_contigs, int32_t window_size, float error_rate,
           int32_t low_memory, uint32_t seed, int32_t n_threads, hs_sr_result** out, SrSparseLabels* sparse = nullptr, SrWorkspace* keep = nullptr, SrTaps* taps = nullptr);

int sr_run_from_cv(SrDeviceOps& dev, const CvMeta& meta, int c0, int c1, const hs_cv_result* cv, float error_rate, float rarest_strain_abundance,
                   int32_t low_memory, int32_t amplicon, uint32_t seed, int32_t n_threads, int32_t window_size, hs_sr_result** out,
                   SrSparseLabels* sparse = nullptr, SrWorkspace* keep = nullptr);

int32_t* sr_labels_alloc(size_t n_labels);
void sr_labels_free(int32_t* labels);
void sr_expand_labels(const SrSparseLabels& sp, const int64_t* label_off, int64_t w0, int64_t w1, int32_t* dense);

struct ColFileContig {
    std::string contig_line, name;
    long length = 0;
    std::vector<std::string> read_lines;
    std::vector<int32_t> read_start, read_end;
    std::vector<int32_t> snp_pos;
    std::vector<uint8_t> snp_ref, snp_alt;
    std::vector<int64_t> col_off{0};
    std::vector<int32_t> col_idx;
    std::vector<uint8_t> col_code;
};
int parse_col(const std::string& path, float rarest_strain_abundance, std::vector<ColFileContig>& cs, int n_threads = 1);
int read_col_sidecar(const std::string& col_path, float rarest_strain_abundance, std::vector<ColFileContig>& cs, int n_threads = 1);

int write_cv_outputs(const CvFileInput& in, const hs_cv_result* res, const std::string& error_rate_out,
                     const std::string& col_path, const std::string& vcf_path, int n_threads = 1);
int write_gro(const std::vector<ColFileContig>& cs, const hs_sr_result* res, const std::string& path, int n_threads = 1);
int write_gro_companion(const std::string& col_path, const std::vector<ColFileContig>& cs, const hs_sr_result* res, float error_rate, float rsa, bool low_memory, bool amplicon,
                        uint32_t seed, int32_t window, int n_threads);
int take_gro_companion(const std::string& col_path, float error_rate, float rsa, bool low_memory, bool amplicon, uint32_t seed, const std::string& outfile, int n_threads);
void remove_gro_companion(const std::string& col_path);
bool mark_gro_companion_pending(const std::string& col_path, float error_rate, float rsa, bool low_memory, bool amplicon, uint32_t seed);

void free_cv_result(hs_cv_result* r);
void free_sr_result(hs_sr_result* r);

}
```

hairsplitter_amd/csrc/hs_kernels_graph.hip:

```cpp
#pragma once

namespace hsdev {

static __device__ __forceinline__ float wave_max_f01(float v) { return __int_as_float(wave_max_i32(__float_as_int(v))); }

template <int FILTER>
static __device__ __forceinline__ void next_level(const float* __restrict__ dv, int m, int lane, float cur, float below, float above,
                                                  int extra_zeros, float* v_out, int* c_out) {
    float best = -1.f;
    for (int j = lane; j < m; j += 64) {
        const float d = dv[j];
        const bool ok = FILTER == 0 ? (d != 1.f) : (d > below && d != 1.f && d < above);
        if (ok && d < cur && d > best) best = d;
    }
    if (FILTER == 0 && extra_zeros > 0 && 0.f < cur && best < 0.f) best = 0.f;
    const int key = best < 0.f ? -1 : __float_as_int(best);
    const int kmax = wave_max_i32(key);
    const float vv = kmax < 0 ? -1.f : __int_as_float(kmax);
    int c = 0;
    if (kmax >= 0) {
        for (int j = lane; j < m; j += 64) {
            const float d = dv[j];
            const bool ok = FILTER == 0 ? (d != 1.f) : (d > below && d != 1.f && d < above);
            if (ok && d == vv) c++;
        }
        c = wave_sum_i32(c);
        if (FILTER == 0 && vv == 0.f) c += extra_zeros;
    }
    *v_out = vv; *c_out = c;
}

template <bool LM>
__global__ __launch_bounds__(256) void k_read_graph_rows(
    const int32_t* __restrict__ sim, const int32_t* __restrict__ diff, const int64_t* __restrict__ ctg_out_off,
    const int32_t* __restrict__ ctg_n, const int32_t* __restrict__ win_contig, const int64_t* __restrict__ win_mask_off,
    const int32_t* __restrict__ mask_ids, const int32_t* __restrict__ row_win, const int64_t* __restrict__ win_bits_off,
    int row_base, int n_rows, float below, int cap, unsigned long long* __restrict__ bits, unsigned long long* __restrict__ amb_head ,
    int32_t* __restrict__ amb_rows, int amb_cap, const int64_t* __restrict__ win_mat_off, int es ,
    long long* __restrict__ amb_stage_off , int32_t* __restrict__ stage_sim, int32_t* __restrict__ stage_diff,
    long long stage_cap, const int32_t* __restrict__ pos_rank , const int64_t* __restrict__ rank_off) {
    extern __shared__ unsigned char s_dyn[];
    const int lane = lane_id();
    const int wv = wave_id(), waves = (int)(blockDim.x >> 6);
    const int row = row_base + (int)blockIdx.x * waves + wv;
    if (row >= row_base + n_rows) return;
    float* __restrict__ dv = reinterpret_cast<float*>(s_dyn) + (size_t)wv * 2 * cap;
    int* __restrict__ tv = reinterpret_cast<int*>(dv + cap);
    const int w = row_win[row];
    const int64_t m0 = win_mask_off[w];
    const int m = (int)(win_mask_off[w + 1] - m0);
    const int i = row - (int)m0;
    const int c = win_contig[w];
    const int N = ctg_n[c];
    const int32_t* __restrict__ ids = mask_ids + m0;
    const int r1 = ids[i];
    const int32_t* __restrict__ prk = (!LM && pos_rank) ? pos_rank + rank_off[c] : nullptr;
    const int r1k = prk ? prk[r1] : r1;
    const int32_t* __restrict__ srow = LM ? sim + (win_mat_off[w] + (int64_t)i * m) * es : sim + (ctg_out_off[c] + (int64_t)r1k * N) * es;
    const int32_t* __restrict__ drow = LM ? diff + (win_mat_off[w] + (int64_t)i * m) * es : diff + (ctg_out_off[c] + (int64_t)r1k * N) * es;
    auto give_up = [&]() {
        const int len = LM ? m : N;
        long long so = -1;
        if (lane == 0) {
            const long long k = (long long)atomicAdd(&amb_head[0], 1ull);
            if (k < amb_cap) {
                amb_rows[k] = row;
                if (stage_sim) { so = (long long)atomicAdd(&amb_head[1], (unsigned long long)len); if (so + len > stage_cap) so = -1; }
                amb_stage_off[k] = so;
            }
        }
        so = (long long)(((unsigned long long)(unsigned)__builtin_amdgcn_readlane((int)(so & 0xffffffffll), 0)) |
                         ((unsigned long long)(unsigned)__builtin_amdgcn_readlane((int)((unsigned long long)so >> 32), 0) << 32));
        if (so >= 0) for (int j = lane; j < len; j += 64) { const int64_t at = (int64_t)(prk ? prk[j] : j) * es; stage_sim[so + j] = srow[at]; stage_diff[so + j] = drow[at]; }
    };
    if (m > cap || N < 2 || !(below >= 0.f)) { give_up(); return; }

    int max_compat = 0;
    bool nan_l = false;
    for (int j = lane; j < m; j += 64) {
        const int r = ids[j];
        const int64_t at = (int64_t)(LM ? j : (prk ? prk[r] : r)) * es;
        const int s = srow[at], dd = drow[at];
        float d = 0.f;
        if (LM) {
            if (r != r1) {
                const float df = (float)(dd - 1 > 0 ? dd - 1 : 0);
                d = 1.f - df / (float)(s + dd);
                if (s > max_compat) max_compat = s;
            }
        } else if (r != r1 && s > 0) {
            const float df = (float)(dd - 1 > 0 ? dd - 1 : 0);
            d = 1.f - df / (float)(s + dd);
            if (s > max_compat) max_compat = s;
        }
        dv[j] = d; tv[j] = r != r1 ? s + dd : 0x7fffffff;
    }
    max_compat = wave_max_i32(max_compat);
    const double thr = 0.7 * (double)max_compat;
    for (int j = lane; j < m; j += 64) {
        if ((double)tv[j] < thr) dv[j] = 0.f;
        if (LM && dv[j] != dv[j]) nan_l = true;
    }
    wave_lds_sync();
    if (LM && __ballot(nan_l) != 0ull) { give_up(); return; }

    const int extra_zeros = N - m;
    float s0, s1; int c0, ones = 0;
    {
        float best = 0.f;
        for (int j = lane; j < m; j += 64) { const float d = dv[j]; if (d > best) best = d; if (d == 1.f) ones++; }
        s0 = wave_max_f01(best);
        ones = wave_sum_i32(ones);
        int cnt = 0; float second = -1.f;
        for (int j = lane; j < m; j += 64) { const float d = dv[j]; if (d == s0) cnt++; else if (d > second) second = d; }
        c0 = wave_sum_i32(cnt) + (s0 == 0.f ? extra_zeros : 0);
        if (extra_zeros > 0 && s0 > 0.f && second < 0.f) second = 0.f;
        const int key = second < 0.f ? -1 : __float_as_int(second);
        const int kmax = wave_max_i32(key);
        s1 = c0 >= 2 ? s0 : (kmax < 0 ? -1.f : __int_as_float(kmax));
    }
    float above = s0 - (s0 - s1) * 3;
    if (above == 1.f && ones < N) {
        const int idx = (ones + 4) < (N - 1) ? (ones + 4) : (N - 1);
        int k = idx - ones;
        float cur = 2.f, v = 0.f; int cc = 0;
        for (int it = 0; it < 5; ++it) {
            next_level<0>(dv, m, lane, cur, below, above, extra_zeros, &v, &cc);
            if (cc == 0) { v = 0.f; break; }
            if (k < cc) break;
            k -= cc; cur = v;
        }
        above = v;
    }
    const int mw64 = (m + 63) >> 6;
    unsigned long long* __restrict__ wb = bits + win_bits_off[w];
    int nA = 0;
    for (int j = lane; j < m; j += 64) { const float d = dv[j]; if (d > below && (d == 1.f || d >= above)) nA++; }
    nA = wave_sum_i32(nA);
    float cut = 3.f;
    if (nA < 5) {
        const int need = 5 - nA;
        int nB = 0;
        for (int j = lane; j < m; j += 64) { const float d = dv[j]; if (d > below && d != 1.f && d < above) nB++; }
        nB = wave_sum_i32(nB);
        if (nB > 0 && nB <= need) cut = -1.f;
        else if (nB > need) {
            int remaining = need; float cur = 2.f, v = 0.f; int cc = 0;
            bool ambiguous = false;
            for (int it = 0; it < 5; ++it) {
                next_level<1>(dv, m, lane, cur, below, above, 0, &v, &cc);
                if (remaining <= cc) { ambiguous = remaining != cc; break; }
                remaining -= cc; cur = v;
            }
            if (ambiguous) { give_up(); return; }
            cut = v;
        }
    }
    for (int j = lane; j < m; j += 64) {
        const float d = dv[j];
        const bool take = d > below && ((d == 1.f || d >= above) || (d != 1.f && d < above && d >= cut));
        if (take) {
            atomicOr(&wb[(int64_t)i * mw64 + (j >> 6)], 1ull << (j & 63));
            atomicOr(&wb[(int64_t)j * mw64 + (i >> 6)], 1ull << (i & 63));
        }
    }
}

__global__ __launch_bounds__(256) void k_read_graph_fetch_rows(
    const int32_t* __restrict__ sim, const int32_t* __restrict__ diff, const int64_t* __restrict__ src_off,
    const int32_t* __restrict__ len, const int64_t* __restrict__ dst_off, int32_t* __restrict__ out_sim, int32_t* __restrict__ out_diff, int es) {
    const int k = (int)blockIdx.x;
    const int n = len[k];
    for (int j = (int)threadIdx.x; j < n; j += 256) { out_sim[dst_off[k] + j] = sim[(src_off[k] + j) * es]; out_diff[dst_off[k] + j] = diff[(src_off[k] + j) * es]; }
}

__global__ __launch_bounds__(256) void k_read_graph_patch(const int64_t* __restrict__ base, const int32_t* __restrict__ mw64,
                                                         const int32_t* __restrict__ pi, const int32_t* __restrict__ pj, int n,
                                                         unsigned long long* __restrict__ bits) {
    const int k = (int)(blockIdx.x * 256 + threadIdx.x);
    if (k >= n) return;
    unsigned long long* wb = bits + base[k];
    atomicOr(&wb[(int64_t)pi[k] * mw64[k] + (pj[k] >> 6)], 1ull << (pj[k] & 63));
    atomicOr(&wb[(int64_t)pj[k] * mw64[k] + (pi[k] >> 6)], 1ull << (pi[k] & 63));
}

__global__ __launch_bounds__(256) void k_read_graph_degrees(const unsigned long long* __restrict__ bits, const int32_t* __restrict__ row_win,
                                                           const int64_t* __restrict__ win_mask_off, const int64_t* __restrict__ win_bits_off,
                                                           int n_rows, int32_t* __restrict__ deg) {
    const int row = (int)(blockIdx.x * 256 + threadIdx.x);
    if (row >= n_rows) return;
    const int w = row_win[row];
    const int m = (int)(win_mask_off[w + 1] - win_mask_off[w]);
    const int mw64 = (m + 63) >> 6;
    const unsigned long long* p = bits + win_bits_off[w] + (int64_t)(row - win_mask_off[w]) * mw64;
    int d = 0;
    for (int k = 0; k < mw64; ++k) d += __popcll(p[k]);
    deg[row] = d;
}

#define HS_SCAN_TILE 4096
__global__ __launch_bounds__(256) void k_scan_tile_sums(const int32_t* __restrict__ in, int n, long long* __restrict__ tile_sum) {
    __shared__ int s_w[4];
    const int t = (int)threadIdx.x;
    const int64_t base = (int64_t)blockIdx.x * HS_SCAN_TILE;
    int s = 0;
#pragma unroll
    for (int k = 0; k < HS_SCAN_TILE / 256; ++k) { const int64_t i = base + k * 256 + t; if (i < n) s += in[i]; }
    s = wave_sum_i32(s);
    if ((t & 63) == 0) s_w[t >> 6] = s;
    __syncthreads();
    if (t == 0) tile_sum[blockIdx.x] = (long long)s_w[0] + s_w[1] + s_w[2] + s_w[3];
}

__global__ __launch_bounds__(1024) void k_scan_tile_offsets(const long long* __restrict__ tile_sum, int n_tiles, long long* __restrict__ tile_off,
                                                           int64_t* __restrict__ total_out) {
    __shared__ long long s_part[1024];
    const int t = (int)threadIdx.x;
    long long carry = 0;
    for (int base = 0; base < n_tiles; base += 1024) {
        const long long v = base + t < n_tiles ? tile_sum[base + t] : 0;
        s_part[t] = v;
        __syncthreads();
        for (int d = 1; d < 1024; d <<= 1) {
            const long long a = t >= d ? s_part[t - d] : 0;
            __syncthreads();
            s_part[t] += a;
            __syncthreads();
        }
        if (base + t < n_tiles) tile_off[base + t] = carry + s_part[t] - v;
        carry += s_part[1023];
        __syncthreads();
    }
    if (t == 0) *total_out = carry;
}

__global__ __launch_bounds__(256) void k_scan_apply(const int32_t* __restrict__ in, int n, const long long* __restrict__ tile_off,
                                                    int64_t* __restrict__ out) {
    __shared__ int s_w[2][4];
    const int t = (int)threadIdx.x, lane = t & 63, wv = t >> 6;
    const int64_t base = (int64_t)blockIdx.x * HS_SCAN_TILE;
    long long run = tile_off[blockIdx.x];
#pragma unroll 1
    for (int k = 0; k < HS_SCAN_TILE / 256; ++k) {
        const int64_t i = base + k * 256 + t;
        const int v = i < n ? in[i] : 0;
        const int incl = wave_scan_incl(v);
        if (lane == 63) s_w[k & 1][wv] = incl;
        __syncthreads();
        const int w0 = s_w[k & 1][0], w1 = s_w[k & 1][1], w2 = s_w[k & 1][2], w3 = s_w[k & 1][3];
        const int before = (wv > 0 ? w0 : 0) + (wv > 1 ? w1 : 0) + (wv > 2 ? w2 : 0);
        if (i < n) out[i] = run + before + incl - v;
        run += (long long)w0 + w1 + w2 + w3;
    }
}

__global__ __launch_bounds__(256) void k_read_graph_fill(const unsigned long long* __restrict__ bits, const int32_t* __restrict__ row_win,
                                                        const int64_t* __restrict__ win_mask_off, const int64_t* __restrict__ win_bits_off,
                                                        const int64_t* __restrict__ nbr_off, int n_rows, int32_t* __restrict__ nbr) {
    const int row = (int)(blockIdx.x * 256 + threadIdx.x);
    if (row >= n_rows) return;
    const int w = row_win[row];
    const int64_t m0 = win_mask_off[w];
    const int m = (int)(win_mask_off[w + 1] - m0);
    const int mw64 = (m + 63) >> 6;
    const unsigned long long* p = bits + win_bits_off[w] + (int64_t)(row - m0) * mw64;
    int32_t* o = nbr + nbr_off[row];
    for (int k = 0; k < mw64; ++k) {
        unsigned long long x = p[k];
        while (x) { const int b = __builtin_ctzll(x); x &= x - 1; *o++ = (k << 6) + b; }
    }
}

}
```

hairsplitter_amd/csrc/hs_rh8.h:

```cpp
#pragma once
#include <stdint.h>
#include "hs_rules.h"

namespace hs {

struct Rh8 {
    static constexpr int kCap = 784;
    uint64_t mult;
    int mask;
    int nslots;
    int count, limit;
    uint32_t inc, shift;
    uint8_t info[kCap];
    uint8_t key[kCap];

    HS_HD void clear() { mult = kRh8Mult; mask = 0; nslots = 0; count = 0; limit = 0; inc = 32; shift = 0; }

    HS_HD static int load_limit(int buckets) { return buckets * 80 / 100; }
    HS_HD static int slots_for(int buckets) { int m = load_limit(buckets); return buckets + (m < 255 ? m : 255); }

    HS_HD void home(uint8_t k, int& idx, uint32_t& inf) const {
        const uint64_t h = rh8_mix(k, mult);
        inf = inc + (uint32_t)((h & 31u) >> shift);
        idx = (int)((h >> 5) & (uint64_t)mask);
    }
    HS_HD void alloc(int buckets) {
        mask = buckets - 1; nslots = slots_for(buckets); count = 0; limit = load_limit(buckets);
        inc = 32; shift = 0;
        for (int i = 0; i < nslots + 8; ++i) info[i] = 0;
    }
    HS_HD bool widen_distance_bits() {
        if (inc <= 2) return false;
        inc >>= 1; shift++;
        for (int i = 0; i < nslots; ++i) info[i] = (uint8_t)((info[i] >> 1) & 0x7f);
        limit = load_limit(mask + 1);
        return true;
    }
    HS_HD void place(uint8_t k, int idx, uint32_t inf) {
        const int ins = idx;
        const uint32_t ins_inf = inf;
        if (ins_inf + inc > 0xFF) limit = 0;
        while (info[idx] != 0) idx++;
        for (int i = idx; i != ins; --i) {
            key[i] = key[i - 1];
            info[i] = (uint8_t)(info[i - 1] + inc);
            if ((uint32_t)info[i] + inc > 0xFF) limit = 0;
        }
        key[ins] = k; info[ins] = (uint8_t)ins_inf; count++;
    }
    HS_HD void reinsert(uint8_t k) {
        if (limit == 0) widen_distance_bits();
        int idx; uint32_t inf;
        home(k, idx, inf);
        while (inf <= info[idx]) { idx++; inf += inc; }
        place(k, idx, inf);
    }
    HS_HD void rebuild(int buckets) {
        uint8_t old_key[kCap];
        int n_old = 0;
        for (int i = 0; i < nslots; ++i) if (info[i] != 0) old_key[n_old++] = key[i];
        alloc(buckets);
        for (int i = 0; i < n_old; ++i) reinsert(old_key[i]);
    }
    HS_HD void grow() {
        if (mask == 0) { alloc(8); return; }
        if (count < load_limit(mask + 1) && widen_distance_bits()) return;
        mult += kRh8MultStep;
        if (count * 2 < load_limit(mask + 1)) rebuild(mask + 1);
        else rebuild((mask + 1) * 2);
    }
    HS_HD void insert(uint8_t k) {
        for (int attempt = 0; attempt < 256; ++attempt) {
            if (mask == 0) { grow(); continue; }
            int idx; uint32_t inf;
            home(k, idx, inf);
            while (inf < info[idx]) { idx++; inf += inc; }
            while (inf == info[idx]) {
                if (key[idx] == k) return;
                idx++; inf += inc;
            }
            if (count >= limit) { grow(); continue; }
            place(k, idx, inf);
            return;
        }
    }
    HS_HD int order(uint8_t* out) const {
        int n = 0;
        for (int i = 0; i < nslots; ++i) if (info[i] != 0) out[n++] = key[i];
        return n;
    }
};


struct Rh8View {
    uint8_t* info; uint8_t* key; uint8_t* tmp;
    int cap;
    uint64_t mult;
    int mask, nslots, count, limit;
    uint32_t inc, shift;
    bool overflow;

    HS_HD void init(uint8_t* info_, uint8_t* key_, uint8_t* tmp_, int cap_) {
        info = info_; key = key_; tmp = tmp_; cap = cap_;
        mult = kRh8Mult; mask = 0; nslots = 0; count = 0; limit = 0; inc = 32; shift = 0; overflow = false;
    }
    HS_HD void home(uint8_t k, int& idx, uint32_t& inf) const {
        const uint64_t h = rh8_mix(k, mult);
        inf = inc + (uint32_t)((h & 31u) >> shift);
        idx = (int)((h >> 5) & (uint64_t)mask);
    }
    HS_HD bool alloc(int buckets) {
        if (Rh8::slots_for(buckets) + 8 > cap) { overflow = true; return false; }
        mask = buckets - 1; nslots = Rh8::slots_for(buckets); count = 0; limit = Rh8::load_limit(buckets);
        inc = 32; shift = 0;
        for (int i = 0; i < nslots + 8; ++i) info[i] = 0;
        return true;
    }
    HS_HD bool widen_distance_bits() {
        if (inc <= 2) return false;
        inc >>= 1; shift++;
        for (int i = 0; i < nslots; ++i) info[i] = (uint8_t)((info[i] >> 1) & 0x7f);
        limit = Rh8::load_limit(mask + 1);
        return true;
    }
    HS_HD void place(uint8_t k, int idx, uint32_t inf) {
        const int ins = idx;
        const uint32_t ins_inf = inf;
        if (ins_inf + inc > 0xFF) limit = 0;
        while (info[idx] != 0) idx++;
        for (int i = idx; i != ins; --i) {
            key[i] = key[i - 1];
            info[i] = (uint8_t)(info[i - 1] + inc);
            if ((uint32_t)info[i] + inc > 0xFF) limit = 0;
        }
        key[ins] = k; info[ins] = (uint8_t)ins_inf; count++;
    }
    HS_HD void reinsert(uint8_t k) {
        if (limit == 0) widen_distance_bits();
        int idx; uint32_t inf;
        home(k, idx, inf);
        while (inf <= info[idx]) { idx++; inf += inc; }
        place(k, idx, inf);
    }
    HS_HD void rebuild(int buckets) {
        int n_old = 0;
        for (int i = 0; i < nslots; ++i) if (info[i] != 0) tmp[n_old++] = key[i];
        if (!alloc(buckets)) return;
        for (int i = 0; i < n_old; ++i) reinsert(tmp[i]);
    }
    HS_HD void grow() {
        if (mask == 0) { alloc(8); return; }
        if (count < Rh8::load_limit(mask + 1) && widen_distance_bits()) return;
        mult += kRh8MultStep;
        if (count * 2 < Rh8::load_limit(mask + 1)) rebuild(mask + 1);
        else rebuild((mask + 1) * 2);
    }
    HS_HD void insert(uint8_t k) {
        for (int attempt = 0; attempt < 256 && !overflow; ++attempt) {
            if (mask == 0) { grow(); continue; }
            int idx; uint32_t inf;
            home(k, idx, inf);
            while (inf < info[idx]) { idx++; inf += inc; }
            while (inf == info[idx]) {
                if (key[idx] == k) return;
                idx++; inf += inc;
            }
            if (count >= limit) { grow(); continue; }
            place(k, idx, inf);
            return;
        }
    }
    HS_HD int order(uint8_t* out) const {
        int n = 0;
        for (int i = 0; i < nslots; ++i) if (info[i] != 0) out[n++] = key[i];
        return n;
    }
};

struct CountSort {
    static HS_HD bool comp(uint32_t a, uint32_t b) { return (a >> 8) > (b >> 8); }
    static HS_HD void swp(uint32_t* a, int i, int j) { const uint32_t t = a[i]; a[i] = a[j]; a[j] = t; }
    static HS_HD void unguarded_linear_insert(uint32_t* a, int last) {
        const uint32_t val = a[last];
        int next = last - 1;
        while (comp(val, a[next])) { a[last] = a[next]; last = next; --next; }
        a[last] = val;
    }
    static HS_HD void insertion_sort(uint32_t* a, int first, int last) {
        if (first == last) return;
        for (int i = first + 1; i != last; ++i) {
            if (comp(a[i], a[first])) { const uint32_t val = a[i]; for (int j = i; j > first; --j) a[j] = a[j - 1]; a[first] = val; }
            else unguarded_linear_insert(a, i);
        }
    }
    static HS_HD void adjust_heap(uint32_t* a, int first, int hole, int len, uint32_t value) {
        const int top = hole;
        int child = hole;
        while (child < (len - 1) / 2) {
            child = 2 * (child + 1);
            if (comp(a[first + child], a[first + (child - 1)])) child--;
            a[first + hole] = a[first + child];
            hole = child;
        }
        if ((len & 1) == 0 && child == (len - 2) / 2) {
            child = 2 * (child + 1);
            a[first + hole] = a[first + (child - 1)];
            hole = child - 1;
        }
        int parent = (hole - 1) / 2;
        while (hole > top && comp(a[first + parent], value)) { a[first + hole] = a[first + parent]; hole = parent; parent = (hole - 1) / 2; }
        a[first + hole] = value;
    }
    static HS_HD void heap_sort(uint32_t* a, int first, int last) {
        const int len = last - first;
        if (len >= 2) {
            for (int parent = (len - 2) / 2;; --parent) { adjust_heap(a, first, parent, len, a[first + parent]); if (parent == 0) break; }
        }
        while (last - first > 1) {
            --last;
            const uint32_t value = a[last];
            a[last] = a[first];
            adjust_heap(a, first, 0, last - first, value);
        }
    }
    static HS_HD int partition_pivot(uint32_t* a, int first, int last) {
        const int mid = first + (last - first) / 2;
        const int x = first + 1, y = mid, z = last - 1;
        if (comp(a[x], a[y])) {
            if (comp(a[y], a[z])) swp(a, first, y);
            else if (comp(a[x], a[z])) swp(a, first, z);
            else swp(a, first, x);
        } else if (comp(a[x], a[z])) swp(a, first, x);
        else if (comp(a[y], a[z])) swp(a, first, z);
        else swp(a, first, y);
        int lo = first + 1, hi = last;
        for (;;) {
            while (comp(a[lo], a[first])) ++lo;
            --hi;
            while (comp(a[first], a[hi])) --hi;
            if (!(lo < hi)) return lo;
            swp(a, lo, hi);
            ++lo;
        }
    }
    static HS_HD void sort(uint32_t* a, int n) { int stack[120]; sort_with_stack(a, n, stack); }
    static HS_HD void sort_with_stack(uint32_t* a, int n, int* stack) {
        if (n <= 0) return;
        int lg = 0;
        for (int v = n; v > 1; v >>= 1) lg++;
        int* st_first = stack; int* st_last = stack + 40; int* st_depth = stack + 80;
        int sp = 0;
        st_first[0] = 0; st_last[0] = n; st_depth[0] = 2 * lg; sp = 1;
        while (sp > 0) {
            --sp;
            const int first = st_first[sp];
            int last = st_last[sp], depth = st_depth[sp];
            while (last - first > 16) {
                if (depth == 0) { heap_sort(a, first, last); break; }
                --depth;
                const int cut = partition_pivot(a, first, last);
                if (sp < 40) { st_first[sp] = cut; st_last[sp] = last; st_depth[sp] = depth; ++sp; }
                last = cut;
            }
        }
        if (n > 16) { insertion_sort(a, 0, 16); for (int i = 16; i < n; ++i) unguarded_linear_insert(a, i); }
        else insertion_sort(a, 0, n);
    }
};

}
```

hairsplitter_amd/csrc/hs_sr_backend.inc:

```
struct GraphRows {
    DBuf d_oo, d_n, d_wc, d_row0, d_ids, d_rw, d_bo, d_fe, d_rank, d_rank_off, d_pos_rank;
    bool by_pos = false;
    UploadPack pack;
    DBuf d_off, d_nbr, d_visit, d_visit_n, d_prog_info, d_prog_bytes, d_prog_steps, d_prog_adj;
    int64_t rows = 0, rows_dev = 0, total = 0;
    bool total_exact = true;
    int W = 0, max_m = 1;
    std::vector<int32_t> win_m;
    DBuf d_bits, d_amb, d_deg, d_scan, d_wmo, d_ltw, d_lti, d_ltj, d_wsim, d_wdiff, d_stage, d_src, d_len, d_dst, d_os, d_od, d_pb, d_pm, d_pi, d_pj;
    UploadPack pk_amb, pk_patch;
    HBuf h_amb, h_rows, h_deg, h_nbr;
    std::vector<int32_t> row_win;
    std::vector<int64_t> win_bits_off, win_mat_off;
    std::vector<int32_t> lt_w, lt_i, lt_j;
    int Wd = 0, Wmx = 0, rows_mx = 0;
    size_t amb_cap = 0;
    int64_t stage_cap = 0, stage_hint = 0;
    EventPair ev;
    bool timed = false, begun = false;
    const int32_t* d_sim = nullptr; const int32_t* d_diff = nullptr; int es = 1;
    std::vector<int64_t> ctg_out_off; std::vector<int32_t> ctg_n;
    float* k_ms = nullptr;
};

struct PlaneRows { const uint64_t* d_alt = nullptr; const uint64_t* d_ref = nullptr; const int64_t* d_plane_off = nullptr; const int32_t* d_words = nullptr; };

static int graph_rows_begin(const int32_t* d_sim, const int32_t* d_diff, const std::vector<int64_t>& ctg_out_off, const std::vector<int32_t>& ctg_n_matrix,
                            const hs::SrWindowSet& ws, GraphRows& G, hipStream_t stream, float* k_ms, KernelClock* kc = nullptr,
                            const PlaneRows* planes = nullptr, int es = 1 ) {
    G.ctg_n = ws.ctg_reads.empty() ? ctg_n_matrix : ws.ctg_reads;
    G.ctg_out_off = ctg_out_off;
    const std::vector<int32_t>& ctg_n = G.ctg_n;
    const int W = (int)ws.win_contig.size();
    G.W = W; G.rows = ws.rows(); G.total = 0; G.total_exact = true; G.max_m = 1; G.begun = true; G.timed = false; G.k_ms = k_ms;
    G.d_sim = d_sim; G.d_diff = d_diff; G.es = es;
    if (G.rows > 0x7fffffff) { set_error("read graphs: too many rows"); return HS_EINVAL; }
    const int rows = (int)G.rows;
    const int Wd = ws.n_dev_windows;
    const int Wmx = ws.ctg_reads.empty() ? Wd : ws.n_matrix_windows;
    const int rows_dev = (int)ws.win_row0[(size_t)Wd];
    const int rows_mx = (int)ws.win_row0[(size_t)Wmx];
    G.rows_dev = rows_dev; G.Wd = Wd; G.Wmx = Wmx; G.rows_mx = rows_mx;
    if (Wmx < Wd && (!planes || !planes->d_alt)) { set_error("read graphs: low-memory windows without bit rows"); return HS_EINVAL; }
    if ((int64_t)ws.host_off.size() != (int64_t)(rows - rows_dev) + 1 && rows != rows_dev) { set_error("read graphs: host rows do not match the window set"); return HS_EINVAL; }
    std::vector<int32_t>& row_win = G.row_win; row_win.assign((size_t)rows_dev, 0);
    std::vector<int64_t>& win_bits_off = G.win_bits_off; win_bits_off.assign((size_t)Wd + 1, 0);
    G.win_m.resize((size_t)W);
    int max_m_dev = 1, max_len = 1;
    for (int w = 0; w < W; ++w) {
        const int64_t m0 = ws.win_row0[(size_t)w], m = ws.win_row0[(size_t)w + 1] - m0;
        G.win_m[(size_t)w] = (int32_t)m;
        G.max_m = std::max(G.max_m, (int)m);
        if (w < Wd) {
            for (int64_t r = 0; r < m; ++r) row_win[(size_t)(m0 + r)] = w;
            win_bits_off[(size_t)w + 1] = win_bits_off[(size_t)w] + m * ((m + 63) >> 6);
            max_m_dev = std::max(max_m_dev, (int)m);
            max_len = std::max(max_len, w < Wmx ? ctg_n[(size_t)ws.win_contig[(size_t)w]] : (int)m);
        }
    }
    std::vector<int64_t>& win_mat_off = G.win_mat_off; win_mat_off.assign((size_t)Wd + 1, 0);
    std::vector<int32_t>& lt_w = G.lt_w; std::vector<int32_t>& lt_i = G.lt_i; std::vector<int32_t>& lt_j = G.lt_j;
    lt_w.clear(); lt_i.clear(); lt_j.clear();
    for (int w = 0; w < Wd; ++w) {
        const int64_t m = w >= Wmx ? G.win_m[(size_t)w] : 0;
        win_mat_off[(size_t)w + 1] = win_mat_off[(size_t)w] + m * m;
        const int nt = (int)((m + 63) / 64);
        for (int i = 0; i < nt; ++i) for (int j = 0; j < nt; ++j) { lt_w.push_back(w); lt_i.push_back(i); lt_j.push_back(j); }
    }
    if (Wmx < Wd) { G.pack.add(win_mat_off, G.d_wmo); G.pack.add(lt_w, G.d_ltw); G.pack.add(lt_i, G.d_lti); G.pack.add(lt_j, G.d_ltj); }
    G.pack.add(ctg_out_off, G.d_oo);
    G.pack.add(ctg_n, G.d_n);
    G.pack.add(ws.win_contig, G.d_wc);
    G.pack.add(ws.win_row0, G.d_row0);
    G.pack.add(ws.mask_ids, G.d_ids);
    G.pack.add(row_win, G.d_rw);
    G.pack.add(win_bits_off, G.d_bo);
    G.pack.add(ws.win_final_empty, G.d_fe);
    G.pack.add(ws.rank, G.d_rank);
    G.pack.add(ws.ctg_rank_off, G.d_rank_off);
    G.by_pos = !ws.pos_rank.empty();
    if (G.by_pos) G.pack.add(ws.pos_rank, G.d_pos_rank);
    if (int rc = G.pack.commit(stream)) return rc;
    if (int rc = G.d_off.alloc(((size_t)rows + 1) * 8 + 32)) return rc;
    if (int rc = G.d_visit.alloc(std::max<size_t>((size_t)rows, 1) * 4)) return rc;
    if (int rc = G.d_visit_n.alloc(std::max<size_t>((size_t)W, 1) * 4)) return rc;
    if (rows == 0) { hipLaunchKernelGGL(hsdev::k_fill16, dim3(1), dim3(64), 0, stream, G.d_off.as<uint4>(), 1ll, 0u); HS_HIP(hipGetLastError()); return HS_OK; }
    if (int rc = G.d_deg.alloc((size_t)rows * 4)) return rc;
    if (int rc = G.ev.init()) return rc;
    if (rows_dev > 0) {
        if (rows_mx > 0 && !d_sim) { set_error("read graphs before simdiff"); return HS_EINVAL; }
        const size_t bits_bytes = ((size_t)win_bits_off.back() * 8 + 15) & ~(size_t)15;
        if (int rc = G.d_bits.alloc(std::max<size_t>(bits_bytes, 16))) return rc;
        G.amb_cap = (size_t)rows_dev;
        G.stage_cap = std::max<int64_t>(G.stage_hint + G.stage_hint / 2, 64 * (int64_t)max_len);
        const size_t amb_bytes = 16 + (((size_t)G.amb_cap * 4 + 15) & ~(size_t)15) + (((size_t)G.amb_cap * 8 + 15) & ~(size_t)15);
        if (int rc = G.d_amb.alloc(amb_bytes)) return rc;
        if (int rc = G.d_stage.alloc((size_t)G.stage_cap * 8 + 32)) return rc;
        hipLaunchKernelGGL(hsdev::k_fill16, dim3((unsigned)std::min<size_t>(256, bits_bytes / 4096 + 1)), dim3(256), 0, stream, G.d_bits.as<uint4>(), (long long)(std::max<size_t>(bits_bytes, 16) / 16), 0u);
        hipLaunchKernelGGL(hsdev::k_fill16, dim3(1), dim3(64), 0, stream, G.d_amb.as<uint4>(), 1ll, 0u);
        unsigned long long* amb_head = G.d_amb.as<unsigned long long>();
        int32_t* amb_rows = reinterpret_cast<int32_t*>((char*)G.d_amb.p + 16);
        long long* amb_so = reinterpret_cast<long long*>((char*)G.d_amb.p + 16 + (((size_t)G.amb_cap * 4 + 15) & ~(size_t)15));
        int32_t* st_sim = G.d_stage.as<int32_t>(); int32_t* st_diff = st_sim + (((size_t)G.stage_cap + 3) & ~(size_t)3);
        int cap = ((max_m_dev + 63) / 64) * 64, waves = 4;
        if ((size_t)cap * 8 * 4 > 57344) waves = 1;
        if ((size_t)cap * 8 > 57344) cap = 7168;
        const float below = 1 - ws.error_rate * 2;
        HS_HIP(ev_rec(G.ev.a, stream));
        if (rows_mx > 0) {
            if (kc) { if (int rc = kc->begin(HS_K_GRAPH_ROWS, stream)) return rc; }
            hipLaunchKernelGGL(hsdev::k_read_graph_rows<false>, dim3((rows_mx + waves - 1) / waves), dim3(64 * waves), (size_t)cap * 8 * waves, stream, d_sim, d_diff,
                               G.d_oo.as<int64_t>(), G.d_n.as<int32_t>(), G.d_wc.as<int32_t>(), G.d_row0.as<int64_t>(), G.d_ids.as<int32_t>(), G.d_rw.as<int32_t>(),
                               G.d_bo.as<int64_t>(), 0, rows_mx, below, cap, G.d_bits.as<unsigned long long>(), amb_head, amb_rows, (int)G.amb_cap,
                               (const int64_t*)nullptr, es, amb_so, st_sim, st_diff, (long long)G.stage_cap, G.by_pos ? G.d_pos_rank.as<int32_t>() : nullptr, G.d_rank_off.as<int64_t>());
            HS_HIP(hipGetLastError());
            if (kc) {
                int64_t by = 0;
                for (int w = 0; w < Wmx; ++w) { const int64_t m = G.win_m[(size_t)w]; by += m * (8 * m + (m + 7) / 8); }
                if (int rc = kc->end(by, stream)) return rc;
            }
        }
        if (rows_dev > rows_mx) {
            const size_t mat = (size_t)win_mat_off.back();
            if (int rc = G.d_wsim.alloc(std::max<size_t>(mat, 1) * 8)) return rc;
            G.d_wdiff.release(); G.d_wdiff.p = (char*)G.d_wsim.p + 4; G.d_wdiff.bytes = 0; G.d_wdiff.cap = 0; G.d_wdiff.view = true;
            if (kc) { if (int rc = kc->begin(HS_K_SIMDIFF, stream)) return rc; }
            hipLaunchKernelGGL(hsdev::k_simdiff_windows, dim3((unsigned)lt_w.size()), dim3(256), 0, stream, planes->d_alt, planes->d_ref, planes->d_plane_off, planes->d_words,
                               G.d_wc.as<int32_t>(), G.d_row0.as<int64_t>(), G.d_ids.as<int32_t>(), G.d_wmo.as<int64_t>(), G.d_ltw.as<int32_t>(), G.d_lti.as<int32_t>(),
                               G.d_ltj.as<int32_t>(), G.d_wsim.as<int32_t>(), G.d_wdiff.as<int32_t>(), 2);
            HS_HIP(hipGetLastError());
            if (kc) { if (int rc = kc->end(8 * (int64_t)mat, stream)) return rc; }
            if (kc) { if (int rc = kc->begin(HS_K_GRAPH_ROWS, stream)) return rc; }
            const int n_lm = rows_dev - rows_mx;
            hipLaunchKernelGGL(hsdev::k_read_graph_rows<true>, dim3((n_lm + waves - 1) / waves), dim3(64 * waves), (size_t)cap * 8 * waves, stream, G.d_wsim.as<int32_t>(),
                               G.d_wdiff.as<int32_t>(), G.d_oo.as<int64_t>(), G.d_n.as<int32_t>(), G.d_wc.as<int32_t>(), G.d_row0.as<int64_t>(), G.d_ids.as<int32_t>(),
                               G.d_rw.as<int32_t>(), G.d_bo.as<int64_t>(), rows_mx, n_lm, below, cap, G.d_bits.as<unsigned long long>(), amb_head, amb_rows, (int)G.amb_cap,
                               G.d_wmo.as<int64_t>(), 2, amb_so, st_sim, st_diff, (long long)G.stage_cap, (const int32_t*)nullptr, (const int64_t*)nullptr);
            HS_HIP(hipGetLastError());
            if (kc) { if (int rc = kc->end(8 * (int64_t)mat, stream)) return rc; }
        }
        HS_HIP(ev_rec(G.ev.b, stream));
        G.timed = true;
        const size_t rows_part = ((size_t)G.amb_cap * 4 + 15) & ~(size_t)15, stage_half = (((size_t)G.stage_cap + 3) & ~(size_t)3) * 4;
        if (int rc = G.h_amb.alloc(amb_bytes + 2 * stage_half + 64)) return rc;
        Shipment sh;
        char* hb = (char*)G.h_amb.p;
        sh.add(hb, G.d_amb.p, 16);
        sh.add_counted(hb + 16, (char*)G.d_amb.p + 16, reinterpret_cast<const long long*>(amb_head), 4, (long long)G.amb_cap);
        sh.add_counted(hb + 16 + rows_part, (char*)G.d_amb.p + 16 + rows_part, reinterpret_cast<const long long*>(amb_head), 8, (long long)G.amb_cap);
        sh.add_counted(hb + amb_bytes, st_sim, reinterpret_cast<const long long*>(amb_head + 1), 4, G.stage_cap);
        sh.add_counted(hb + amb_bytes + stage_half, st_diff, reinterpret_cast<const long long*>(amb_head + 1), 4, G.stage_cap);
        if (kc) { if (int rc = kc->begin(HS_K_SHIP, stream)) return rc; }
        if (int rc = sh.launch(stream, 16)) return rc;
        if (kc) { if (int rc = kc->end(0, stream)) return rc; }
    }
    return HS_OK;
}

static int graph_rows_end(const hs::SrWindowSet& ws, GraphRows& G, hipStream_t stream, int64_t* rows_on_host, KernelClock* kc = nullptr) {
    if (rows_on_host) *rows_on_host = 0;
    const int rows = (int)G.rows, rows_dev = (int)G.rows_dev, rows_mx = G.rows_mx, Wd = G.Wd, Wmx = G.Wmx, W = G.W;
    if (rows == 0) return HS_OK;
    const std::vector<int32_t>& ctg_n = G.ctg_n;
    const std::vector<int32_t>& row_win = G.row_win;
    const std::vector<int64_t>& win_bits_off = G.win_bits_off;
    const std::vector<int64_t>& win_mat_off = G.win_mat_off;
    if (rows_dev > 0) {
        if (int rc = stream_wait(stream)) return rc;
        const size_t rows_part = ((size_t)G.amb_cap * 4 + 15) & ~(size_t)15, amb_bytes = 16 + rows_part + (((size_t)G.amb_cap * 8 + 15) & ~(size_t)15), stage_half = (((size_t)G.stage_cap + 3) & ~(size_t)3) * 4;
        const char* hb = (const char*)G.h_amb.p;
        const int64_t n_amb = (int64_t)((const unsigned long long*)hb)[0];
        const int64_t staged = (int64_t)((const unsigned long long*)hb)[1];
        G.stage_hint = staged;
        if (n_amb > (int64_t)G.amb_cap) { set_error("read graphs: more undecided rows than rows"); return HS_EINVAL; }
        if (n_amb > 0) {
            const int32_t* amb_rows = (const int32_t*)(hb + 16);
            const long long* amb_so = (const long long*)(hb + 16 + rows_part);
            const int32_t* st_sim = (const int32_t*)(hb + amb_bytes); const int32_t* st_diff = (const int32_t*)(hb + amb_bytes + stage_half);
            std::vector<int32_t> order((size_t)n_amb);
            for (int64_t k = 0; k < n_amb; ++k) order[(size_t)k] = (int32_t)k;
            std::sort(order.begin(), order.end(), [&](int32_t x, int32_t y) { return amb_rows[x] < amb_rows[y]; });
            std::vector<int32_t> late;
            for (int32_t k : order) if (amb_so[k] < 0) late.push_back(k);
            std::vector<int64_t> late_dst((size_t)late.size() + 1, 0);
            const int32_t* late_sim = nullptr; const int32_t* late_diff = nullptr;
            if (!late.empty()) {
                std::vector<int64_t> src(late.size()); std::vector<int32_t> len(late.size());
                int n_mx = 0;
                for (size_t q = 0; q < late.size(); ++q) {
                    const int row = amb_rows[late[q]];
                    const int w = row_win[(size_t)row];
                    const int c = ws.win_contig[(size_t)w];
                    const int N = ctg_n[(size_t)c];
                    const int r1 = ws.mask_ids[(size_t)row];
                    if (row < rows_mx) { const int r1k = G.by_pos ? ws.pos_rank[(size_t)ws.ctg_rank_off[(size_t)c] + (size_t)r1] : r1; src[q] = G.ctg_out_off[(size_t)c] + (int64_t)r1k * N; len[q] = N; n_mx++; }
                    else { const int64_t m = G.win_m[(size_t)w]; src[q] = win_mat_off[(size_t)w] + (int64_t)(row - ws.win_row0[(size_t)w]) * m; len[q] = (int32_t)m; }
                    late_dst[q + 1] = late_dst[q] + len[q];
                }
                G.pk_amb.add(src, G.d_src); G.pk_amb.add(len, G.d_len); G.pk_amb.add(late_dst, G.d_dst);
                if (int rc = G.pk_amb.commit(stream)) return rc;
                if (int rc = G.d_os.alloc((size_t)late_dst.back() * 4 + 16)) return rc;
                if (int rc = G.d_od.alloc((size_t)late_dst.back() * 4 + 16)) return rc;
                if (n_mx > 0)
                    hipLaunchKernelGGL(hsdev::k_read_graph_fetch_rows, dim3(n_mx), dim3(256), 0, stream, G.d_sim, G.d_diff, G.d_src.as<int64_t>(), G.d_len.as<int32_t>(),
                                       G.d_dst.as<int64_t>(), G.d_os.as<int32_t>(), G.d_od.as<int32_t>(), G.es);
                if ((int)late.size() > n_mx)
                    hipLaunchKernelGGL(hsdev::k_read_graph_fetch_rows, dim3((unsigned)late.size() - n_mx), dim3(256), 0, stream, G.d_wsim.as<int32_t>(), G.d_wdiff.as<int32_t>(),
                                       G.d_src.as<int64_t>() + n_mx, G.d_len.as<int32_t>() + n_mx, G.d_dst.as<int64_t>() + n_mx, G.d_os.as<int32_t>(), G.d_od.as<int32_t>(), 2);
                HS_HIP(hipGetLastError());
                const size_t row_bytes = (((size_t)late_dst.back() * 4) + 15) & ~(size_t)15;
                if (int rc = G.h_rows.alloc(2 * row_bytes + 16)) return rc;
                Shipment sh; sh.add(G.h_rows.p, G.d_os.p, row_bytes); sh.add((char*)G.h_rows.p + row_bytes, G.d_od.p, row_bytes);
                if (int rc = sh.launch(stream, 16)) return rc;
                if (int rc_w = stream_wait(stream)) return rc_w;
                late_sim = (const int32_t*)G.h_rows.p; late_diff = (const int32_t*)((const char*)G.h_rows.p + row_bytes);
                G.stage_hint = std::max<int64_t>(G.stage_hint, staged + late_dst.back());
            }
            std::vector<int64_t> pbase; std::vector<int32_t> pmw, pi, pj;
            std::vector<uint8_t> mask;
            std::vector<int> picked;
            size_t late_q = 0;
            for (int32_t k : order) {
                const int row = amb_rows[k];
                const int w = row_win[(size_t)row];
                const int64_t m0 = ws.win_row0[(size_t)w];
                const int m = (int)(ws.win_row0[(size_t)w + 1] - m0);
                const int32_t* ids = ws.mask_ids.data() + m0;
                const int N = ctg_n[(size_t)ws.win_contig[(size_t)w]];
                const int32_t* rs; const int32_t* rd;
                std::vector<int32_t> perm_s, perm_d;
                if (late_q < late.size() && late[late_q] == k) {
                    rs = late_sim + late_dst[late_q]; rd = late_diff + late_dst[late_q]; late_q++;
                    if (G.by_pos && row < rows_mx) {
                        const int32_t* pr = ws.pos_rank.data() + ws.ctg_rank_off[(size_t)ws.win_contig[(size_t)w]];
                        perm_s.resize((size_t)N); perm_d.resize((size_t)N);
                        for (int r = 0; r < N; ++r) { perm_s[(size_t)r] = rs[pr[r]]; perm_d[(size_t)r] = rd[pr[r]]; }
                        rs = perm_s.data(); rd = perm_d.data();
                    }
                }
                else { rs = st_sim + amb_so[k]; rd = st_diff + amb_so[k]; }
                mask.assign((size_t)N, 0);
                for (int j = 0; j < m; ++j) mask[(size_t)ids[j]] = 1;
                if (row < rows_mx) hs::sr_pick_row_sorted(rs, rd, N, ids[row - m0], mask.data(), ws.error_rate, picked);
                else hs::sr_pick_row_sorted_low_memory(rs, rd, ids, m, (int)(row - m0), N, mask.data(), ws.error_rate, picked);
                for (int nb : picked) {
                    const int j = (int)(std::lower_bound(ids, ids + m, nb) - ids);
                    pbase.push_back(win_bits_off[(size_t)w]); pmw.push_back((m + 63) >> 6); pi.push_back((int32_t)(row - m0)); pj.push_back(j);
                }
            }
            if (!pi.empty()) {
                G.pk_patch.add(pbase, G.d_pb); G.pk_patch.add(pmw, G.d_pm); G.pk_patch.add(pi, G.d_pi); G.pk_patch.add(pj, G.d_pj);
                if (int rc = G.pk_patch.commit(stream)) return rc;
                const int np = (int)pi.size();
                hipLaunchKernelGGL(hsdev::k_read_graph_patch, dim3((np + 255) / 256), dim3(256), 0, stream, G.d_pb.as<int64_t>(), G.d_pm.as<int32_t>(), G.d_pi.as<int32_t>(),
                                   G.d_pj.as<int32_t>(), np, G.d_bits.as<unsigned long long>());
                HS_HIP(hipGetLastError());
            }
            if (rows_on_host) *rows_on_host = n_amb;
            if (std::getenv("HS_TIMING") && Wmx < Wd) {
                int64_t n_lm = 0; for (int64_t k = 0; k < n_amb; ++k) n_lm += amb_rows[k] >= rows_mx;
                std::fprintf(stderr, "[hs timing] sr: low-memory path on the device: %d windows, %d rows, %ld of them resolved on the host (NaN distances / std::sort ties)\n",
                             Wd - Wmx, rows_dev - rows_mx, (long)n_lm);
            }
        } else if (std::getenv("HS_TIMING") && Wmx < Wd)
            std::fprintf(stderr, "[hs timing] sr: low-memory path on the device: %d windows, %d rows, none resolved on the host\n", Wd - Wmx, rows_dev - rows_mx);
        if (kc) { if (int rc = kc->begin(HS_K_GRAPH_CSR, stream)) return rc; }
        hipLaunchKernelGGL(hsdev::k_read_graph_degrees, dim3((rows_dev + 255) / 256), dim3(256), 0, stream, G.d_bits.as<unsigned long long>(), G.d_rw.as<int32_t>(),
                           G.d_row0.as<int64_t>(), G.d_bo.as<int64_t>(), rows_dev, G.d_deg.as<int32_t>());
        HS_HIP(hipGetLastError());
        if (kc) { if (int rc = kc->end((int64_t)win_bits_off.back() * 8 + 4 * (int64_t)rows_dev, stream)) return rc; }
    }
    if (rows > rows_dev) {
        const size_t nh = (size_t)(rows - rows_dev);
        if (int rc = G.h_deg.alloc(nh * 4 + 16)) return rc;
        int32_t* hd = (int32_t*)G.h_deg.p;
        for (size_t r = 0; r < nh; ++r) hd[r] = (int32_t)(ws.host_off[r + 1] - ws.host_off[r]);
        HS_HIP(HS_COPY_ASYNC(G.d_deg.as<int32_t>() + rows_dev, hd, nh * 4, hipMemcpyHostToDevice, stream));
    }
    if (int rc = exclusive_scan_launch(G.d_deg.as<int32_t>(), rows, G.d_off.as<int64_t>(), G.d_scan, stream)) return rc;
    int64_t bound = (int64_t)ws.host_nbr.size();
    for (int w = 0; w < Wd; ++w) bound += (int64_t)G.win_m[(size_t)w] * G.win_m[(size_t)w];
    int64_t total = bound;
    G.total_exact = false;
    if (!ws.host_nbr.empty() || bound > ((int64_t)1 << 28)) {
        if (int rc = d2h_pinned(&total, G.d_off.as<int64_t>() + rows, 8, stream)) return rc;
        G.total_exact = true;
    }
    G.total = total;
    if (int rc = G.d_nbr.alloc(std::max<size_t>((size_t)total, 1) * 4)) return rc;
    if (total > 0) {
        if (rows_dev > 0) {
            if (kc) { if (int rc = kc->begin(HS_K_GRAPH_CSR, stream)) return rc; }
            hipLaunchKernelGGL(hsdev::k_read_graph_fill, dim3((rows_dev + 255) / 256), dim3(256), 0, stream, G.d_bits.as<unsigned long long>(), G.d_rw.as<int32_t>(),
                               G.d_row0.as<int64_t>(), G.d_bo.as<int64_t>(), G.d_off.as<int64_t>(), rows_dev, G.d_nbr.as<int32_t>());
            HS_HIP(hipGetLastError());
            if (kc) { if (int rc = kc->end((int64_t)win_bits_off.back() * 8 + 4 * (G.total_exact ? total : (int64_t)rows_dev * 20), stream)) return rc; }
        }
        if (!ws.host_nbr.empty()) {
            const size_t nb = ws.host_nbr.size() * 4;
            if (int rc = G.h_nbr.alloc(nb)) return rc;
            std::memcpy(G.h_nbr.p, ws.host_nbr.data(), nb);
            HS_HIP(HS_COPY_ASYNC(G.d_nbr.as<int32_t>() + (total - (int64_t)ws.host_nbr.size()), G.h_nbr.p, nb, hipMemcpyHostToDevice, stream));
        }
    }
    {
        const int cap = std::min(((G.max_m + 63) / 64) * 64, 8192);
        if (int rc = G.d_prog_info.alloc(std::max<size_t>((size_t)rows, 1) * 4)) return rc;
        if (int rc = G.d_prog_bytes.alloc((size_t)total + 15 * (size_t)rows + 64)) return rc;
        const size_t steps_bytes = (std::max<size_t>((size_t)W, 1) * 4 + 15) & ~(size_t)15;
        if (int rc = G.d_prog_steps.alloc(steps_bytes)) return rc;
        if (int rc = G.d_prog_adj.alloc(std::max<size_t>((size_t)rows, 1) * 8)) return rc;
        hipLaunchKernelGGL(hsdev::k_fill16, dim3((unsigned)std::min<size_t>(64, steps_bytes / 4096 + 1)), dim3(256), 0, stream, G.d_prog_steps.as<uint4>(), (long long)(steps_bytes / 16), 0u);
        if (kc) { if (int rc = kc->begin(HS_K_VISIT_LISTS, stream)) return rc; }
        hipLaunchKernelGGL(hsdev::k_cw_visit_lists, dim3((unsigned)W), dim3(256), (size_t)cap * 4, stream, G.d_off.as<int64_t>(), G.d_nbr.as<int32_t>(), G.d_row0.as<int64_t>(),
                           G.d_ids.as<int32_t>(), G.d_wc.as<int32_t>(), G.d_rank_off.as<int64_t>(), G.d_rank.as<int32_t>(), W, cap, G.d_visit.as<int32_t>(),
                           G.d_visit_n.as<int32_t>(), G.d_prog_info.as<uint32_t>(), G.d_prog_bytes.as<uint8_t>(), G.d_prog_steps.as<int32_t>(),
                           G.d_prog_adj.as<unsigned long long>());
        HS_HIP(hipGetLastError());
        if (kc) { if (int rc = kc->end(20 * (int64_t)rows, stream)) return rc; }
    }
    return HS_OK;
}
static int graph_rows_settle(GraphRows& G, KernelClock* kc) {
    if (kc) kc->flush();
    if (G.timed) { G.timed = false; float m = 0; if (int rc = G.ev.ms(&m)) return rc; if (G.k_ms) *G.k_ms += m; }
    return HS_OK;
}
static int graph_rows_build(const int32_t* d_sim, const int32_t* d_diff, const std::vector<int64_t>& ctg_out_off, const std::vector<int32_t>& ctg_n_matrix,
                            const hs::SrWindowSet& ws, GraphRows& G, hipStream_t stream, int64_t* rows_on_host, float* k_ms, KernelClock* kc = nullptr,
                            const PlaneRows* planes = nullptr, int es = 1) {
    if (int rc = graph_rows_begin(d_sim, d_diff, ctg_out_off, ctg_n_matrix, ws, G, stream, k_ms, kc, planes, es)) return rc;
    if (int rc = graph_rows_end(ws, G, stream, rows_on_host, kc)) return rc;
    if (G.rows > 0 && !G.total_exact) { int64_t t = 0; if (int rc = d2h_pinned(&t, G.d_off.as<int64_t>() + G.rows, 8, stream)) return rc; G.total = t; G.total_exact = true; }
    else if (int rc_w = stream_wait(stream)) return rc_w;
    return graph_rows_settle(G, kc);
}

struct HipSrOps : hs::SrDeviceOps {
    hipStream_t stream = nullptr;
    DBuf d_sim, d_diff;
    std::vector<int64_t> sd_out_off;
    std::vector<int32_t> sd_n;
    GraphRows G;
    KernelClock kc;

    struct SimdiffInFlight {
        DBuf d_alt, d_ref, d_sr, d_sa, d_sc, d_cb, d_po, d_n, d_pn, d_w, d_oo, t_c, t_i, t_j, d_bc, d_bw, d_rb, d_orig, d_rng;
        std::vector<int32_t> tc, ti, tj, blk_c, blk_w;
        UploadPack pk;
        EventPair ev;
        float* k_ms = nullptr;
    };
    std::unique_ptr<SimdiffInFlight> sd_flight;
    int settle_simdiff(bool account = true) {
        if (!sd_flight) return HS_OK;
        float m = 0;
        int rc = (sd_flight->ev.a || k5_waited) ? HS_OK : stream_wait_quiet(stream);
        if (!rc) rc = sd_flight->ev.ms(&m);
        if (!rc && account && sd_flight->k_ms) *sd_flight->k_ms += m;
        sd_flight.reset();
        return rc;
    }
    bool k5_waited = false;
    ~HipSrOps() override { (void)settle_simdiff(false); }

    DBuf d_col_off, d_col_idx, d_col_code;
    UploadPack col_pack;
    const hs::CwChain* resident_cols = nullptr;
    bool adopted = false;
    int64_t adopted_cols = 0, adopted_entries = 0;
    DBuf cols_block;
    void adopt_columns(HipCvOps& cv) {
        std::swap(cols_block, cv.d_pk);
        char* base = (char*)cols_block.p;
        auto view = [&](DBuf& d, size_t off, size_t bytes) { d.release(); d.p = base + off; d.bytes = bytes; d.cap = 0; d.view = true; };
        view(d_col_off, cv.pk_layout.off, ((size_t)cv.snp_count + 1) * 8);
        view(d_col_idx, cv.pk_layout.idx, (size_t)cv.snp_entries * 4);
        view(d_col_code, cv.pk_layout.code, (size_t)cv.snp_entries);
        adopted = true; adopted_cols = cv.snp_count; adopted_entries = cv.snp_entries;
    }
    bool columns_resident() const override { return adopted; }
    bool low_memory_graphs() const override { static const bool host = std::getenv("HS_LOW_MEMORY_GRAPHS_ON_HOST") != nullptr; return !host; }
    void drop_resident_columns() override { adopted = false; resident_cols = nullptr; }
    int fetch_columns(std::vector<int32_t>& idx, std::vector<uint8_t>& code) override {
        if (!adopted) { set_error("fetch_columns: no resident columns"); return HS_EINVAL; }
        idx.resize((size_t)adopted_entries); code.resize((size_t)adopted_entries);
        if (adopted_entries == 0) return HS_OK;
        if (int rc = d2h_pinned(idx.data(), d_col_idx.p, (size_t)adopted_entries * 4, stream)) return rc;
        return d2h_pinned(code.data(), d_col_code.p, (size_t)adopted_entries, stream);
    }
    int window_masks(const std::vector<int64_t>& col_a, const std::vector<int64_t>& col_b, const std::vector<int64_t>& slot_off,
                     std::vector<int32_t>& ids, std::vector<int32_t>& win_m) override {
        if (!adopted) { set_error("window_masks: no resident columns"); return HS_EINVAL; }
        const int W = (int)col_a.size();
        const int64_t total = slot_off.back();
        ids.resize((size_t)total); win_m.assign((size_t)W, 0);
        if (W == 0) return HS_OK;
        DBuf d_a, d_b, d_so, d_ids;
        UploadPack pk;
        pk.add(col_a, d_a); pk.add(col_b, d_b); pk.add(slot_off, d_so);
        if (int rc = pk.commit(stream)) return rc;
        const size_t ids_bytes = ((size_t)total * 4 + 255) & ~(size_t)255;
        if (int rc = d_ids.alloc(ids_bytes + (size_t)W * 4 + 16)) return rc;
        int32_t* const dm = reinterpret_cast<int32_t*>((char*)d_ids.p + ids_bytes);
        if (int rc = kc.begin(HS_K_WINDOW_MASKS, stream)) return rc;
        hipLaunchKernelGGL(hsdev::k_window_masks, dim3((unsigned)((W + 3) / 4)), dim3(256), 0, stream, d_col_off.as<int64_t>(), d_col_idx.as<int32_t>(), d_a.as<int64_t>(),
                           d_b.as<int64_t>(), d_so.as<int64_t>(), W, d_ids.as<int32_t>(), dm);
        HS_HIP(hipGetLastError());
        if (int rc = kc.end(8 * total + 4 * (int64_t)W, stream)) return rc;
        HBuf h_ids;
        if (int rc = h_ids.alloc(ids_bytes + (size_t)W * 4 + 16)) return rc;
        { Shipment sh; sh.add(h_ids.p, d_ids.p, ids_bytes + (size_t)W * 4); if (int rc = sh.launch(stream, 32)) return rc; }
        if (int rc = stream_wait(stream)) return rc;
        k5_waited = true;
        if (total) std::memcpy(ids.data(), h_ids.p, (size_t)total * 4);
        std::memcpy(win_m.data(), (const char*)h_ids.p + ids_bytes, (size_t)W * 4);
        kc.flush();
        return HS_OK;
    }
    int simdiff_columns(const hs::SimdiffJob& job, float* k_ms) override {
        const hs::CwChain& ch = *job.cols;
        if (!adopted) {
            col_pack.add(ch.col_off, d_col_off); col_pack.add(ch.col_idx, d_col_idx); col_pack.add(ch.col_code, d_col_code);
            if (int rc = col_pack.commit(stream)) return rc;
        } else if ((int64_t)ch.col_off.size() != adopted_cols + 1) { set_error("simdiff_columns: the resident columns are not those of this call"); return HS_EINVAL; }
        resident_cols = job.cols;
        sd_out_off = job.out_off; sd_n = job.n_reads;
        if (job.out_total <= 0 && job.plane_total <= 0) return HS_OK;
        if (int rc = settle_simdiff()) return rc;
        sd_flight.reset(new SimdiffInFlight());
        k5_waited = false;
        SimdiffInFlight& f = *sd_flight;
        f.k_ms = k_ms;
        f.pk.add(job.snp_ref, f.d_sr);
        f.pk.add(job.snp_alt, f.d_sa);
        f.pk.add(job.snp_contig, f.d_sc);
        f.pk.add(job.contig_snp_base, f.d_cb);
        f.pk.add(job.plane_off, f.d_po);
        f.pk.add(job.n_reads, f.d_n);
        f.pk.add(job.plane_n, f.d_pn);
        f.pk.add(job.words, f.d_w);
        f.pk.add(job.out_off, f.d_oo);
        snp_planes_blocks(job.words.data(), (int)job.words.size(), f.blk_c, f.blk_w);
        simdiff_tiles(job.n_reads, f.tc, f.ti, f.tj);
        f.pk.add(f.blk_c, f.d_bc); f.pk.add(f.blk_w, f.d_bw); f.pk.add(f.tc, f.t_c); f.pk.add(f.ti, f.t_i); f.pk.add(f.tj, f.t_j);
        const bool by_pos = !job.pos_orig.empty();
        const size_t rows_all = job.pos_orig.size();
        if (by_pos) { f.pk.add(job.read_base, f.d_rb); f.pk.add(job.pos_orig, f.d_orig); }
        if (int rc = f.pk.commit(stream)) return rc;
        int32_t* rng_lo = nullptr; int32_t* rng_hi = nullptr;
        if (by_pos) {
            const size_t half = ((rows_all * 4 + 15) & ~(size_t)15);
            if (int rc = f.d_rng.alloc(2 * half + 16)) return rc;
            rng_lo = f.d_rng.as<int32_t>(); rng_hi = reinterpret_cast<int32_t*>((char*)f.d_rng.p + half);
            const unsigned gb = (unsigned)std::min<size_t>(64, half / 4096 + 1);
            hipLaunchKernelGGL(hsdev::k_fill16, dim3(gb), dim3(256), 0, stream, reinterpret_cast<uint4*>(rng_lo), (long long)(half / 16), 0x7fffffffu);
            hipLaunchKernelGGL(hsdev::k_fill16, dim3(gb), dim3(256), 0, stream, reinterpret_cast<uint4*>(rng_hi), (long long)(half / 16), 0xffffffffu);
        }
        const size_t pbytes = (size_t)job.plane_total * sizeof(uint64_t);
        if (int rc = f.d_alt.alloc(pbytes)) return rc;
        if (int rc = f.d_ref.alloc(pbytes)) return rc;
        if (int rc = d_sim.alloc(std::max<size_t>((size_t)job.out_total, 1) * 2 * sizeof(int32_t))) return rc;
        d_diff.release(); d_diff.p = (char*)d_sim.p + sizeof(int32_t); d_diff.bytes = 0; d_diff.cap = 0; d_diff.view = true;
        if (int rc = kc.begin(HS_K_SNP_PLANES, stream)) return rc;
        if (int rc = snp_planes_launch(d_col_off.as<int64_t>(), d_col_idx.as<int32_t>(), d_col_code.as<uint8_t>(), f.d_sr.as<uint8_t>(), f.d_sa.as<uint8_t>(),
                                       f.d_sc.as<int32_t>(), f.d_cb.as<int64_t>(), f.d_po.as<int64_t>(), f.d_w.as<int32_t>(), f.d_pn.as<int32_t>(), f.d_bc.as<int32_t>(),
                                       f.d_bw.as<int32_t>(), f.blk_c.size(), (int32_t)job.snp_ref.size(), f.d_alt.as<uint64_t>(), f.d_ref.as<uint64_t>(), stream,
                                       by_pos ? f.d_rb.as<int64_t>() : nullptr, rng_lo, rng_hi)) return rc;
        if (int rc = kc.end(5 * (adopted ? adopted_entries : (int64_t)ch.col_idx.size()) + 2 * (int64_t)pbytes, stream)) return rc;
        if (int rc = f.ev.init()) return rc;
        HS_HIP(ev_rec(f.ev.a, stream));
        if (int rc = kc.begin(HS_K_SIMDIFF, stream)) return rc;
        if (int rc = simdiff_launch(f.d_alt.as<uint64_t>(), f.d_ref.as<uint64_t>(), f.d_po.as<int64_t>(), f.d_n.as<int32_t>(), f.d_w.as<int32_t>(),
                                    f.d_oo.as<int64_t>(), d_sim.as<int32_t>(), d_diff.as<int32_t>(), stream, f.t_c.as<int32_t>(), f.t_i.as<int32_t>(), f.t_j.as<int32_t>(), f.tc.size(), 2,
                                    by_pos ? f.d_rb.as<int64_t>() : nullptr, by_pos ? f.d_orig.as<int32_t>() : nullptr, rng_lo, rng_hi)) return rc;
        if (int rc = kc.end(2 * (int64_t)pbytes + 8 * job.out_total, stream)) return rc;
        HS_HIP(ev_rec(f.ev.b, stream));
        return HS_OK;
    }

    struct Keep { int64_t stage_hint = 0; };
    Keep* keep = nullptr;
    PlaneRows plane_rows() const {
        PlaneRows pr;
        if (sd_flight) { pr.d_alt = sd_flight->d_alt.as<uint64_t>(); pr.d_ref = sd_flight->d_ref.as<uint64_t>(); pr.d_plane_off = sd_flight->d_po.as<int64_t>(); pr.d_words = sd_flight->d_w.as<int32_t>(); }
        return pr;
    }
    int build_graphs(const hs::SrWindowSet& ws, int64_t* rows_on_host, float* k_ms) override {
        if (int rc = build_graphs_begin(ws, k_ms)) return rc;
        return build_graphs_end(ws, rows_on_host);
    }
    bool two_phase_graphs() const override { return true; }
    int build_graphs_begin(const hs::SrWindowSet& ws, float* k_ms) override {
        const PlaneRows pr = plane_rows();
        if (keep) G.stage_hint = keep->stage_hint;
        return graph_rows_begin(d_sim.as<int32_t>(), d_diff.as<int32_t>(), sd_out_off, sd_n, ws, G, stream, k_ms, &kc, &pr, 2);
    }
    int build_graphs_end(const hs::SrWindowSet& ws, int64_t* rows_on_host) override {
        const int rc = graph_rows_end(ws, G, stream, rows_on_host, &kc);
        if (!rc) k5_waited = true;
        if (keep) keep->stage_hint = G.stage_hint;
        return rc;
    }
    int fetch_graphs(std::vector<int64_t>& off, std::vector<int32_t>& nbr) override {
        if (G.rows > 0 && !G.total_exact) { int64_t t = 0; if (int rc = d2h_pinned(&t, G.d_off.as<int64_t>() + G.rows, 8, stream)) return rc; G.total = t; G.total_exact = true; }
        off.assign((size_t)G.rows + 1, 0); nbr.assign((size_t)G.total, 0);
        if (int rc = d2h_pinned(off.data(), G.d_off.p, off.size() * 8, stream)) return rc;
        if (G.total > 0) { if (int rc = d2h_pinned(nbr.data(), G.d_nbr.p, nbr.size() * 4, stream)) return rc; }
        return HS_OK;
    }

    static int lds_nodes(int max_m, int ints_per_node, int limit_bytes) {
        const int cap = ((std::max(max_m, 1) + 63) / 64) * 64;
        return std::min(cap, (limit_bytes / (ints_per_node * 4)) / 64 * 64);
    }

    std::vector<int64_t>* tap_run_off = nullptr; std::vector<int32_t>* tap_run_labels = nullptr;
    void tap_chain(std::vector<int64_t>* run_off, std::vector<int32_t>* run_labels) override { tap_run_off = run_off; tap_run_labels = run_labels; }
    int cw_chain(const hs::CwChain& ch, std::vector<int32_t>& labels, std::vector<int32_t>& final_labels, std::vector<uint8_t>& final_ok,
                 float k_ms[3], hs::SrChainStats* stats) override {
        if (int rc = settle_simdiff()) return rc;
        const int Wc = (int)ch.win.size();
        const int64_t n_inst = (int64_t)ch.seed_col.size();
        const int64_t total_m = ch.chain_row0.back();
        if (n_inst > 0x7fffffff) { set_error("Chinese Whispers: too many runs in one call"); return HS_EINVAL; }
        std::vector<int32_t> inst_win((size_t)n_inst), list_big, list_lanes, unit_win, unit_inst0, unit_n;
        const int lanes_cap = 64;
        int max_m_small = 1;
        std::vector<int64_t> inst_slab((size_t)n_inst), chain_slab0((size_t)Wc), big_scr, tail_scr((size_t)Wc, 0);
        int64_t slab = 0, big_scr_total = 0, tail_scr_total = 0;
        int max_m_big = 1, max_m_chain = 1;
        bool all_lanes = true;
        for (int k = 0; k < Wc && all_lanes; ++k) all_lanes = G.win_m[(size_t)ch.win[(size_t)k]] <= lanes_cap;
        if (all_lanes) {
            for (int k = 0; k < Wc; ++k) {
                const int m = G.win_m[(size_t)ch.win[(size_t)k]];
                chain_slab0[(size_t)k] = slab;
                max_m_chain = std::max(max_m_chain, m);
                slab += (ch.win_seed_begin[(size_t)k + 1] - ch.win_seed_begin[(size_t)k]) * (int64_t)m;
            }
            list_lanes.resize((size_t)n_inst);
            hs::hs_parallel_for(Wc, std::min(8, host_threads()), [&](int k) {
                const int w = ch.win[(size_t)k];
                const int m = G.win_m[(size_t)w];
                int64_t sl = chain_slab0[(size_t)k];
                for (int64_t i = ch.win_seed_begin[(size_t)k]; i < ch.win_seed_begin[(size_t)k + 1]; ++i) { inst_win[(size_t)i] = w; inst_slab[(size_t)i] = sl; sl += m; list_lanes[(size_t)i] = (int32_t)i; }
            });
        } else
        for (int k = 0; k < Wc; ++k) {
            const int w = ch.win[(size_t)k];
            const int m = G.win_m[(size_t)w];
            chain_slab0[(size_t)k] = slab;
            max_m_chain = std::max(max_m_chain, m);
            for (int64_t i = ch.win_seed_begin[(size_t)k]; i < ch.win_seed_begin[(size_t)k + 1]; ++i) {
                inst_win[(size_t)i] = w; inst_slab[(size_t)i] = slab; slab += m;
                if (m > HS_CWR_CAP) { list_big.push_back((int32_t)i); max_m_big = std::max(max_m_big, m); }
                else if (m <= lanes_cap) list_lanes.push_back((int32_t)i);
            }
            if (m <= HS_CWR_CAP && m > lanes_cap) {
                max_m_small = std::max(max_m_small, m);
                for (int64_t i = ch.win_seed_begin[(size_t)k]; i < ch.win_seed_begin[(size_t)k + 1]; i += 8) {
                    unit_win.push_back(w); unit_inst0.push_back((int32_t)i);
                    unit_n.push_back((int32_t)std::min<int64_t>(8, ch.win_seed_begin[(size_t)k + 1] - i));
                }
            }
        }
        const int cap_big = lds_nodes(max_m_big, 2, 96 * 1024);
        for (int32_t i : list_big) {
            const int m = G.win_m[(size_t)inst_win[(size_t)i]];
            big_scr.push_back(big_scr_total);
            if (m > cap_big) big_scr_total += 2 * (int64_t)m;
        }
        const int cap_tail = lds_nodes(max_m_chain, 7, 56 * 1024);
        std::vector<int32_t> tail_list((size_t)Wc);
        int n_tail_small = 0;
        {
            int wide = 0;
            for (int k = 0; k < Wc; ++k) if (G.win_m[(size_t)ch.win[(size_t)k]] <= 64) n_tail_small++;
            int at_small = 0;
            for (int k = 0; k < Wc; ++k) { if (G.win_m[(size_t)ch.win[(size_t)k]] <= 64) tail_list[(size_t)at_small++] = k; else tail_list[(size_t)(n_tail_small + wide++)] = k; }
        }
        for (int k = 0; k < Wc; ++k) {
            const int m = G.win_m[(size_t)ch.win[(size_t)k]];
            tail_scr[(size_t)k] = tail_scr_total;
            if (m > cap_tail) tail_scr_total += 7 * (int64_t)m + (m & 1);
        }
        DBuf d_ll, d_sets, d_names, d_slots, d_alive, d_ovf, d_ovf_n, d_iw, d_is, d_seed, d_uw, d_ui, d_un, d_lb, d_bs, d_cw, d_cr0, d_csb, d_cs0, d_ts, d_slab, d_gs, d_l3, d_final, d_ok, d_stat,
            d_cpos, d_sf, d_sl, d_plo, d_phi, d_tl;
        if (resident_cols != &ch && !adopted) {
            col_pack.add(ch.col_off, d_col_off); col_pack.add(ch.col_idx, d_col_idx); col_pack.add(ch.col_code, d_col_code);
            if (int rc = col_pack.commit(stream)) return rc;
            resident_cols = &ch;
        }
        const bool finish = ch.finish_on_device && !std::getenv("HS_FINISH_ON_HOST");
        UploadPack pk;
        pk.add(inst_win, d_iw); pk.add(inst_slab, d_is); pk.add(ch.seed_col, d_seed); pk.add(unit_win, d_uw); pk.add(unit_inst0, d_ui); pk.add(unit_n, d_un); pk.add(list_big, d_lb); pk.add(list_lanes, d_ll);
        pk.add(big_scr, d_bs); pk.add(ch.win, d_cw); pk.add(ch.chain_row0, d_cr0); pk.add(ch.win_seed_begin, d_csb); pk.add(chain_slab0, d_cs0);
        pk.add(tail_scr, d_ts); pk.add(tail_list, d_tl);
        if (finish) { pk.add(ch.col_pos, d_cpos); pk.add(ch.win_snp_first, d_sf); pk.add(ch.win_snp_last, d_sl); pk.add(ch.win_pos_lo, d_plo); pk.add(ch.win_pos_hi, d_phi); }
        if (int rc = pk.commit(stream)) return rc;
        if (int rc = d_slab.alloc(std::max<size_t>((size_t)slab, 1) * 4)) return rc;
        if (int rc = d_gs.alloc(std::max<size_t>((size_t)std::max(big_scr_total, tail_scr_total), 2) * 4)) return rc;
        if (int rc = d_l3.alloc(std::max<size_t>((size_t)total_m, 1) * 4)) return rc;
        if (int rc = d_final.alloc(std::max<size_t>((size_t)total_m, 1) * 4)) return rc;
        if (int rc = d_ok.alloc(std::max<size_t>((size_t)Wc, 1))) return rc;
        if (int rc = d_stat.alloc(416)) return rc;
        hipLaunchKernelGGL(hsdev::k_fill16, dim3(1), dim3(64), 0, stream, d_stat.as<uint4>(), 26ll, 0u);
        EventPair e1, e2;
        if (int rc = e1.init()) return rc;
        if (int rc = e2.init()) return rc;
        HS_HIP(ev_rec(e1.a, stream));
        if (!list_lanes.empty()) {
            const int n = (int)list_lanes.size();
            const size_t npad = ((size_t)n + 63) & ~(size_t)63;
            if (int rc = d_sets.alloc(npad * 128)) return rc;
            if (int rc = d_names.alloc(npad * 16)) return rc;
            if (int rc = d_slots.alloc(npad * 64)) return rc;
            if (int rc = d_alive.alloc(npad)) return rc;
            if (int rc = d_ovf.alloc((size_t)n * 4)) return rc;
            if (int rc = d_ovf_n.alloc(16)) return rc;
            hipLaunchKernelGGL(hsdev::k_fill16, dim3(1), dim3(64), 0, stream, d_ovf_n.as<uint4>(), 1ll, 0u);
            if (int rc = kc.begin(HS_K_CW_SEED_SETS, stream)) return rc;
            hipLaunchKernelGGL(hsdev::k_cw_seed_sets, dim3((unsigned)((n + 3) / 4)), dim3(256), 0, stream, G.d_row0.as<int64_t>(), G.d_ids.as<int32_t>(), d_ll.as<int32_t>(), n,
                               d_iw.as<int32_t>(), d_seed.as<int64_t>(), d_col_off.as<int64_t>(), d_col_idx.as<int32_t>(), d_col_code.as<uint8_t>(),
                               d_sets.as<unsigned long long>(), d_names.as<uint8_t>(), d_slots.as<uint8_t>(), d_alive.as<uint8_t>(), d_ovf.as<int32_t>(), d_ovf_n.as<int32_t>());
            HS_HIP(hipGetLastError());
            if (int rc = kc.end((int64_t)npad * 209 + 5 * (int64_t)n * 40, stream)) return rc;
            if (int rc = kc.begin(HS_K_CW_SEEDED, stream)) return rc;
            hipLaunchKernelGGL(hsdev::k_cw_seeded_lanes, dim3((unsigned)(npad / 64)), dim3(64), 0, stream, G.d_off.as<int64_t>(), G.d_row0.as<int64_t>(), G.d_visit_n.as<int32_t>(),
                               G.d_prog_info.as<uint32_t>(), G.d_prog_adj.as<unsigned long long>(), d_ll.as<int32_t>(), n, d_iw.as<int32_t>(), d_is.as<int64_t>(),
                               d_sets.as<unsigned long long>(), d_names.as<uint8_t>(), d_slots.as<uint8_t>(), d_alive.as<uint8_t>(), d_slab.as<int32_t>(), d_stat.as<unsigned long long>());
            HS_HIP(hipGetLastError());
            if (int rc = kc.end((int64_t)npad * 209, stream)) return rc;
            if (std::getenv("HS_TIMING")) {
                int32_t n_ovf = 0;
                if (int rc = d2h_pinned(&n_ovf, d_ovf_n.p, 4, stream)) return rc;
                std::fprintf(stderr, "[hs timing] sr: %d per-SNP runs one per lane, %d of them with more than 16 labels alive (-> one wavefront each); %zu runs in units of 8, %zu one wavefront each\n",
                             n, n_ovf, unit_win.size() * 8, list_big.size());
            }
            if (int rc = kc.begin(HS_K_CW_SEEDED_WIDE, stream)) return rc;
            hipLaunchKernelGGL(hsdev::k_cw_seeded_wave, dim3((unsigned)std::min(n, 1024)), dim3(64), (size_t)64 * 8, stream, G.d_off.as<int64_t>(), G.d_nbr.as<int32_t>(),
                               G.d_row0.as<int64_t>(), G.d_ids.as<int32_t>(), G.d_visit.as<int32_t>(), G.d_visit_n.as<int32_t>(), d_ovf.as<int32_t>(), 0, d_ovf_n.as<int32_t>(),
                               d_iw.as<int32_t>(), d_seed.as<int64_t>(), d_is.as<int64_t>(), d_col_off.as<int64_t>(), d_col_idx.as<int32_t>(),
                               d_col_code.as<uint8_t>(), 64, (int32_t*)nullptr, (const int64_t*)nullptr, d_slab.as<int32_t>(), d_stat.as<unsigned long long>());
            HS_HIP(hipGetLastError());
            if (int rc = kc.end(0, stream)) return rc;
        }
        if (!unit_win.empty() || !list_big.empty()) { if (int rc = kc.begin(HS_K_CW_SEEDED_WIDE, stream)) return rc; }
        if (!unit_win.empty()) {
            const int n = (int)unit_win.size();
            const int m_cap = std::max(16, (max_m_small + 15) & ~15);
            const int cnt_cap = std::max(m_cap, 256);
            const int prog_cap = std::max(2048, m_cap * 32);
            const size_t lds = (size_t)2 * m_cap * 4 + (size_t)8 * cnt_cap * 4 + (size_t)prog_cap + (size_t)8 * m_cap;
            if (lds > 48 * 1024)
                HS_HIP(hipFuncSetAttribute(reinterpret_cast<const void*>(hsdev::k_cw_seeded_rows), hipFuncAttributeMaxDynamicSharedMemorySize, (int)lds));
            hipLaunchKernelGGL(hsdev::k_cw_seeded_rows, dim3((unsigned)n), dim3(128), lds, stream, G.d_off.as<int64_t>(), G.d_nbr.as<int32_t>(),
                               G.d_row0.as<int64_t>(), G.d_ids.as<int32_t>(), G.d_visit.as<int32_t>(), G.d_visit_n.as<int32_t>(), G.d_prog_info.as<uint32_t>(),
                               G.d_prog_bytes.as<uint8_t>(), G.d_prog_steps.as<int32_t>(), d_uw.as<int32_t>(), d_ui.as<int32_t>(), d_un.as<int32_t>(), n, d_seed.as<int64_t>(), d_is.as<int64_t>(), d_col_off.as<int64_t>(), d_col_idx.as<int32_t>(),
                               d_col_code.as<uint8_t>(), m_cap, prog_cap, d_slab.as<int32_t>(), d_stat.as<unsigned long long>());
            HS_HIP(hipGetLastError());
        }
        if (!list_big.empty()) {
            const int n = (int)list_big.size();
            const size_t lds = (size_t)cap_big * 8;
            if (lds > 48 * 1024)
                HS_HIP(hipFuncSetAttribute(reinterpret_cast<const void*>(hsdev::k_cw_seeded_wave), hipFuncAttributeMaxDynamicSharedMemorySize, (int)lds));
            hipLaunchKernelGGL(hsdev::k_cw_seeded_wave, dim3((unsigned)n), dim3(64), lds, stream, G.d_off.as<int64_t>(), G.d_nbr.as<int32_t>(),
                               G.d_row0.as<int64_t>(), G.d_ids.as<int32_t>(), G.d_visit.as<int32_t>(), G.d_visit_n.as<int32_t>(), d_lb.as<int32_t>(), n, (const int32_t*)nullptr,
                               d_iw.as<int32_t>(), d_seed.as<int64_t>(), d_is.as<int64_t>(), d_col_off.as<int64_t>(), d_col_idx.as<int32_t>(),
                               d_col_code.as<uint8_t>(), cap_big, d_gs.as<int32_t>(), d_bs.as<int64_t>(), d_slab.as<int32_t>(), d_stat.as<unsigned long long>());
            HS_HIP(hipGetLastError());
        }
        if (!unit_win.empty() || !list_big.empty()) { if (int rc = kc.end(0, stream)) return rc; }
        HS_HIP(ev_rec(e1.b, stream));
        HS_HIP(ev_rec(e2.a, stream));
        if (int rc = kc.begin(HS_K_WINDOW_TAIL, stream)) return rc;
        if (Wc > 0) {
            const size_t lds = (size_t)cap_tail * 7 * 4 + HS_TAIL_MAP_EXTRA;
            if (lds > 32 * 1024)
                HS_HIP(hipFuncSetAttribute(reinterpret_cast<const void*>(hsdev::k_window_tail), hipFuncAttributeMaxDynamicSharedMemorySize, (int)lds));
            for (int part = 0; part < 2; ++part) {
                const int n_part = part == 0 ? n_tail_small : Wc - n_tail_small;
                if (n_part == 0) continue;
                const int cap = part == 0 ? std::min(cap_tail, 64) : cap_tail;
                hipLaunchKernelGGL(hsdev::k_window_tail, dim3((unsigned)n_part), dim3(64), (size_t)cap * 7 * 4 + HS_TAIL_MAP_EXTRA, stream, G.d_off.as<int64_t>(), G.d_nbr.as<int32_t>(), G.d_row0.as<int64_t>(),
                                   G.d_ids.as<int32_t>(), G.d_visit.as<int32_t>(), G.d_visit_n.as<int32_t>(), G.d_fe.as<uint8_t>(), G.d_prog_info.as<uint32_t>(),
                                   G.d_prog_adj.as<unsigned long long>(), d_cw.as<int32_t>(), d_cr0.as<int64_t>(),
                                   d_csb.as<int64_t>(), d_cs0.as<int64_t>(), d_slab.as<int32_t>(), d_tl.as<int32_t>() + (part == 0 ? 0 : n_tail_small), n_part, d_col_off.as<int64_t>(),
                                   d_col_idx.as<int32_t>(), d_col_code.as<uint8_t>(), d_cpos.as<int32_t>(), d_sf.as<int64_t>(), d_sl.as<int64_t>(), d_plo.as<int32_t>(), d_phi.as<int32_t>(),
                                   finish ? 1 : 0, cap, d_gs.as<int32_t>(), d_ts.as<int64_t>(), d_l3.as<int32_t>(), d_final.as<int32_t>(), d_ok.as<uint8_t>(),
                                   d_stat.as<unsigned long long>() + 2);
            }
            HS_HIP(hipGetLastError());
        }
        if (int rc = kc.end(4 * slab + 8 * total_m, stream)) return rc;
        HS_HIP(ev_rec(e2.b, stream));
        {
            HBuf h, h4;
            const size_t o_nnz = 416, o_final = 512, o_ok = o_final + (((size_t)total_m * 4 + 255) & ~(size_t)255);
            if (int rc = h4.alloc(o_ok + (size_t)Wc + 256)) return rc;
            Shipment sh;
            sh.add(h4.p, d_stat.p, 416);
            sh.add((char*)h4.p + o_nnz, G.d_off.as<int64_t>() + (G.rows & ~(int64_t)1), 16);
            bool need_chain_labels = !finish || tap_run_labels != nullptr;
            if (finish) {
                sh.add((char*)h4.p + o_final, d_final.p, (size_t)total_m * sizeof(int32_t));
                sh.add((char*)h4.p + o_ok, d_ok.p, (size_t)Wc);
            }
            if (int rc = kc.begin(HS_K_SHIP, stream)) return rc;
            if (int rc = sh.launch(stream, 64)) return rc;
            if (int rc = kc.end(0, stream)) return rc;
            if (int rc = stream_wait(stream)) return rc;
            if (finish) {
                final_labels.resize((size_t)total_m); final_ok.resize((size_t)Wc);
                std::memcpy(final_labels.data(), (const char*)h4.p + o_final, (size_t)total_m * sizeof(int32_t));
                std::memcpy(final_ok.data(), (const char*)h4.p + o_ok, (size_t)Wc);
                for (uint8_t ok : final_ok) if (!ok) { need_chain_labels = true; break; }
            }
            if (need_chain_labels) {
                labels.resize((size_t)total_m);
                if (int rc = h.alloc(std::max<size_t>((size_t)total_m, 1) * sizeof(int32_t))) return rc;
                if (int rc = copy_d2h(h.p, d_l3.p, (size_t)total_m * sizeof(int32_t), stream)) return rc;
                std::memcpy(labels.data(), h.p, (size_t)total_m * sizeof(int32_t));
            } else labels.clear();
            if (tap_run_labels && tap_run_off) {
                tap_run_labels->resize((size_t)slab);
                if (slab) { if (int rc = d2h_pinned(tap_run_labels->data(), d_slab.p, (size_t)slab * sizeof(int32_t), stream)) return rc; }
                tap_run_off->assign(inst_slab.begin(), inst_slab.end()); tap_run_off->push_back(slab);
            }
            if (!G.total_exact) { G.total = ((const int64_t*)((const char*)h4.p + o_nnz))[G.rows & 1]; G.total_exact = true; }
            if (int rc = graph_rows_settle(G, &kc)) return rc;
            const unsigned long long* st = (const unsigned long long*)h4.p;
            if (stats) { stats->n_instances = n_inst + 2 * (int64_t)Wc; stats->sweeps = (int64_t)(st[0] + st[2]); stats->bytes = (int64_t)(st[1] + st[3]); stats->graph_nnz = G.total; }
            if (std::getenv("HS_TIMING")) {
                std::string h;
                for (int k = 0; k < 16; ++k) h += " " + std::to_string((unsigned long long)st[4 + k]);
                std::fprintf(stderr, "[hs timing] sr: per-SNP Chinese-Whispers runs by number of sweeps (0..15+):%s\n", h.c_str());
#ifdef HS_TAIL_DIAG
                std::fprintf(stderr, "[hs timing] sr: k_window_tail cycles: merged ids %llu, two runs + small clusters %llu, renumbering %llu, merge_close_clusters %llu, merge_wrongly_split_haplotypes: slots + map %llu, SNPs %llu, link counts %llu, links + output %llu; SNPs fast %llu slow %llu, keys %llu, windows with map %llu, clusters %llu\n",
                             (unsigned long long)st[20], (unsigned long long)st[21], (unsigned long long)st[22], (unsigned long long)st[23], (unsigned long long)st[25], (unsigned long long)st[26],
                             (unsigned long long)st[27], (unsigned long long)st[24], (unsigned long long)st[28], (unsigned long long)st[29], (unsigned long long)st[30], (unsigned long long)st[31], (unsigned long long)st[32]);
#endif
#ifdef HS_CW_DIAG
                h.clear(); for (int k = 0; k < 16; ++k) h += " " + std::to_string((unsigned long long)st[20 + k]);
                std::fprintf(stderr, "[hs timing] sr: runs by labels alive after seeding (0..15+):%s\n", h.c_str());
                h.clear(); for (int k = 0; k < 16; ++k) h += " " + std::to_string((unsigned long long)st[36 + k]);
                std::fprintf(stderr, "[hs timing] sr: runs by m/16:%s\n", h.c_str());
#endif
            }
            KernelClock::add_bytes(HS_K_CW_SEEDED, (int64_t)st[1]);
            KernelClock::add_bytes(HS_K_WINDOW_TAIL, (int64_t)st[3]);
            kc.flush();
        }
        float m = 0;
        if (int rc = e1.ms(&m)) return rc; k_ms[0] += m;
        if (int rc = e2.ms(&m)) return rc; k_ms[1] += m;
        return HS_OK;
    }
    int cw(hs::CwWave& wv, float* k_ms) override {
        const int n_inst = (int)wv.inst_win.size();
        if (n_inst == 0) return HS_OK;
        int max_m = 1;
        for (int w : wv.inst_win) max_m = std::max(max_m, G.win_m[(size_t)w]);
        const int cap = lds_nodes(max_m, 2, 96 * 1024);
        std::vector<int64_t> scr((size_t)n_inst, 0);
        int64_t scr_total = 0;
        for (int k = 0; k < n_inst; ++k) { const int m = G.win_m[(size_t)wv.inst_win[(size_t)k]]; scr[(size_t)k] = scr_total; if (m > cap) scr_total += 2 * (int64_t)m; }
        DBuf d_iw, d_lo, d_lab, d_scr, d_gs;
        UploadPack pk;
        pk.add(wv.inst_win, d_iw); pk.add(wv.inst_label_off, d_lo); pk.add(wv.labels, d_lab); pk.add(scr, d_scr);
        if (int rc = pk.commit(stream)) return rc;
        if (int rc = d_gs.alloc(std::max<size_t>((size_t)scr_total, 2) * 4)) return rc;
        EventPair ev; if (int rc = ev.init()) return rc;
        HS_HIP(ev_rec(ev.a, stream));
        if (int rc = kc.begin(HS_K_CW_LOCAL, stream)) return rc;
        const size_t lds = (size_t)cap * 8;
        if (lds > 48 * 1024)
            HS_HIP(hipFuncSetAttribute(reinterpret_cast<const void*>(hsdev::k_cw_local), hipFuncAttributeMaxDynamicSharedMemorySize, (int)lds));
        hipLaunchKernelGGL(hsdev::k_cw_local, dim3((unsigned)n_inst), dim3(64), lds, stream, G.d_off.as<int64_t>(), G.d_nbr.as<int32_t>(), G.d_row0.as<int64_t>(),
                           G.d_visit.as<int32_t>(), G.d_visit_n.as<int32_t>(), G.d_fe.as<uint8_t>(), d_iw.as<int32_t>(), d_lo.as<int64_t>(), n_inst, cap,
                           d_gs.as<int32_t>(), d_scr.as<int64_t>(), d_lab.as<int32_t>());
        HS_HIP(hipGetLastError());
        if (int rc = kc.end(8 * (int64_t)wv.labels.size(), stream)) return rc;
        HS_HIP(ev_rec(ev.b, stream));
        if (int rc = d2h_pinned(wv.labels.data(), d_lab.p, wv.labels.size() * sizeof(int32_t), stream)) return rc;
        float m = 0; if (int rc = ev.ms(&m)) return rc;
        if (k_ms) *k_ms += m;
        return HS_OK;
    }
};

}
```

Before: 138.1 billion.

## Resolve tied graph rows on device and defer the host sync into chain readback

Tied (ambiguous) read-graph rows were previously sent back to the host for resolution, which forced a stream wait. A new k_read_graph_ties kernel now resolves them on the device with a wave-parallel partial quicksort, and the check of its outcome is folded into the cw_chain result shipment, so no separate sync is needed. If any rows still cannot be resolved, the graphs are rebuilt on the host path and the chain is rerun. This adds complexity and a costly fallback path, and the distance and cut logic is factored into shared device helpers.

Result: slower. 130.0 billion (-5.8%).

```diff
diff --git a/hairsplitter_amd/csrc/hs_driver.cpp b/hairsplitter_amd/csrc/hs_driver.cpp
--- a/hairsplitter_amd/csrc/hs_driver.cpp
+++ b/hairsplitter_amd/csrc/hs_driver.cpp
@@ -835,6 +835,7 @@
         const double t0 = now_ms();
         if (taps) dev.tap_chain(&taps->run_off, &taps->run_labels);
         if (!ch.win.empty()) { if (int rc = dev.cw_chain(ch, chain_labels, final_labels, final_ok, &k_ms[1], &cst)) return rc; }
+        if (!wrefs.empty()) { if (int rc = dev.build_graphs_settle(&rows_on_host)) return rc; }
         dev_ms += now_ms() - t0;
     }
     if (taps) {
diff --git a/hairsplitter_amd/csrc/hs_driver.h b/hairsplitter_amd/csrc/hs_driver.h
--- a/hairsplitter_amd/csrc/hs_driver.h
+++ b/hairsplitter_amd/csrc/hs_driver.h
@@ -161,6 +161,7 @@
     virtual bool two_phase_graphs() const { return false; }
     virtual int build_graphs_begin(const SrWindowSet& ws, float* k_ms) { (void)ws; (void)k_ms; return -1; }
     virtual int build_graphs_end(const SrWindowSet& ws, int64_t* rows_on_host) { (void)ws; (void)rows_on_host; return -1; }
+    virtual int build_graphs_settle(int64_t* rows_on_host) { (void)rows_on_host; return 0; }
     virtual int fetch_graphs(std::vector<int64_t>& off, std::vector<int32_t>& nbr) = 0;
     virtual int cw_chain(const CwChain& chain, std::vector<int32_t>& labels, std::vector<int32_t>& final_labels,
                          std::vector<uint8_t>& final_ok, float k_ms[3], SrChainStats* stats) = 0;
diff --git a/hairsplitter_amd/csrc/hs_kernels_graph.hip b/hairsplitter_amd/csrc/hs_kernels_graph.hip
--- a/hairsplitter_amd/csrc/hs_kernels_graph.hip
+++ b/hairsplitter_amd/csrc/hs_kernels_graph.hip
@@ -28,6 +28,106 @@
         if (FILTER == 0 && vv == 0.f) c += extra_zeros;
     }
     *v_out = vv; *c_out = c;
+}
+
+template <bool LM>
+static __device__ __forceinline__ bool graph_row_distances(const int32_t* __restrict__ srow, const int32_t* __restrict__ drow, const int32_t* __restrict__ ids,
+                                                           const int32_t* __restrict__ prk, int es, int m, int r1, int lane, float* __restrict__ dv, int* __restrict__ tv) {
+    int max_compat = 0;
+    bool nan_l = false;
+    for (int j = lane; j < m; j += 64) {
+        const int r = ids[j];
+        const int64_t at = (int64_t)(LM ? j : (prk ? prk[r] : r)) * es;
+        const int s = srow[at], dd = drow[at];
+        float d = 0.f;
+        if (LM) {
+            if (r != r1) {
+                const float df = (float)(dd - 1 > 0 ? dd - 1 : 0);
+                d = 1.f - df / (float)(s + dd);
+                if (s > max_compat) max_compat = s;
+            }
+        } else if (r != r1 && s > 0) {
+            const float df = (float)(dd - 1 > 0 ? dd - 1 : 0);
+            d = 1.f - df / (float)(s + dd);
+            if (s > max_compat) max_compat = s;
+        }
+        dv[j] = d; tv[j] = r != r1 ? s + dd : 0x7fffffff;
+    }
+    max_compat = wave_max_i32(max_compat);
+    const double thr = 0.7 * (double)max_compat;
+    for (int j = lane; j < m; j += 64) {
+        if ((double)tv[j] < thr) dv[j] = 0.f;
+        if (LM && dv[j] != dv[j]) nan_l = true;
+    }
+    wave_lds_sync();
+    return LM && __ballot(nan_l) != 0ull;
+}
+
+struct RowCut { float above, cut, tied; int remaining; bool ambiguous; };
+static __device__ __forceinline__ RowCut graph_row_cut(const float* __restrict__ dv, int m, int N, int lane, float below) {
+    const int extra_zeros = N - m;
+    float s0, s1; int c0, ones = 0;
+    {
+        float best = 0.f;
+        for (int j = lane; j < m; j += 64) { const float d = dv[j]; if (d > best) best = d; if (d == 1.f) ones++; }
+        s0 = wave_max_f01(best);
+        ones = wave_sum_i32(ones);
+        int cnt = 0; float second = -1.f;
+        for (int j = lane; j < m; j += 64) { const float d = dv[j]; if (d == s0) cnt++; else if (d > second) second = d; }
+        c0 = wave_sum_i32(cnt) + (s0 == 0.f ? extra_zeros : 0);
+        if (extra_zeros > 0 && s0 > 0.f && second < 0.f) second = 0.f;
+        const int key = second < 0.f ? -1 : __float_as_int(second);
+        const int kmax = wave_max_i32(key);
+        s1 = c0 >= 2 ? s0 : (kmax < 0 ? -1.f : __int_as_float(kmax));
+    }
+    float above = s0 - (s0 - s1) * 3;
+    if (above == 1.f && ones < N) {
+        const int idx = (ones + 4) < (N - 1) ? (ones + 4) : (N - 1);
+        int k = idx - ones;
+        float cur = 2.f, v = 0.f; int cc = 0;
+        for (int it = 0; it < 5; ++it) {
+            next_level<0>(dv, m, lane, cur, below, above, extra_zeros, &v, &cc);
+            if (cc == 0) { v = 0.f; break; }
+            if (k < cc) break;
+            k -= cc; cur = v;
+        }
+        above = v;
+    }
+    int nA = 0;
+    for (int j = lane; j < m; j += 64) { const float d = dv[j]; if (d > below && (d == 1.f || d >= above)) nA++; }
+    nA = wave_sum_i32(nA);
+    RowCut rc; rc.cut = 3.f; rc.tied = 0.f; rc.remaining = 0; rc.ambiguous = false;
+    if (nA < 5) {
+        const int need = 5 - nA;
+        int nB = 0;
+        for (int j = lane; j < m; j += 64) { const float d = dv[j]; if (d > below && d != 1.f && d < above) nB++; }
+        nB = wave_sum_i32(nB);
+        if (nB > 0 && nB <= need) rc.cut = -1.f;
+        else if (nB > need) {
+            int remaining = need; float cur = 2.f, v = 0.f; int cc = 0;
+            for (int it = 0; it < 5; ++it) {
+                next_level<1>(dv, m, lane, cur, below, above, 0, &v, &cc);
+                if (remaining <= cc) { rc.ambiguous = remaining != cc; break; }
+                remaining -= cc; cur = v;
+            }
+            rc.cut = v; rc.tied = v; rc.remaining = remaining;
+        }
+    }
+    rc.above = above;
+    return rc;
+}
+
+static __device__ __forceinline__ void graph_row_link(const float* __restrict__ dv, int m, int i, int lane, float below, float above, float cut,
+                                                      unsigned long long* __restrict__ wb) {
+    const int mw64 = (m + 63) >> 6;
+    for (int j = lane; j < m; j += 64) {
+        const float d = dv[j];
+        const bool take = d > below && ((d == 1.f || d >= above) || (d != 1.f && d < above && d >= cut));
+        if (take) {
+            atomicOr(&wb[(int64_t)i * mw64 + (j >> 6)], 1ull << (j & 63));
+            atomicOr(&wb[(int64_t)j * mw64 + (i >> 6)], 1ull << (i & 63));
+        }
+    }
 }
 
 template <bool LM>
@@ -75,93 +175,120 @@
     };
     if (m > cap || N < 2 || !(below >= 0.f)) { give_up(); return; }
 
-    int max_compat = 0;
-    bool nan_l = false;
-    for (int j = lane; j < m; j += 64) {
-        const int r = ids[j];
-        const int64_t at = (int64_t)(LM ? j : (prk ? prk[r] : r)) * es;
-        const int s = srow[at], dd = drow[at];
-        float d = 0.f;
-        if (LM) {
-            if (r != r1) {
-                const float df = (float)(dd - 1 > 0 ? dd - 1 : 0);
-                d = 1.f - df / (float)(s + dd);
-                if (s > max_compat) max_compat = s;
+    if (graph_row_distances<LM>(srow, drow, ids, prk, es, m, r1, lane, dv, tv)) { give_up(); return; }
+
+    const RowCut rc = graph_row_cut(dv, m, N, lane, below);
+    if (rc.ambiguous) { give_up(); return; }
+    graph_row_link(dv, m, i, lane, below, rc.above, rc.cut, bits + win_bits_off[w]);
+}
+
+static __device__ __forceinline__ int wave_partition_pivot(hs::DistPair* __restrict__ pr, int first, int last, int lane, int* __restrict__ lpos, int* __restrict__ rpos) {
+    if (lane == 0) hs::DistSort::median_to_first(pr, first, last);
+    wave_lds_sync();
+    const float piv = pr[first].second;
+    const unsigned long long lt = (1ull << lane) - 1ull;
+    int nl = 0, nr = 0;
+    for (int base = 0; base < last - first; base += 64) {
+        const int ql = first + 1 + base + lane, qr = last - 1 - base - lane;
+        const bool isl = ql < last && !(pr[ql].second > piv);
+        const bool isr = qr >= first && !(piv > pr[qr].second);
+        const unsigned long long bl = __ballot(isl), br = __ballot(isr);
+        if (isl) lpos[nl + __popcll(bl & lt)] = ql;
+        if (isr) rpos[nr + __popcll(br & lt)] = qr;
+        nl += __popcll(bl); nr += __popcll(br);
+    }
+    wave_lds_sync();
+    const int nk = nl < nr ? nl : nr;
+    int cnt = 0;
+    for (int k = lane; k < nk; k += 64) cnt += lpos[k] < rpos[k] ? 1 : 0;
+    const int s = wave_sum_i32(cnt);
+    int cut = s < nl ? lpos[s] : last;
+    if (s > 0) { const int r = rpos[s - 1]; if (r < cut) cut = r; }
+    for (int k = lane; k < s; k += 64) hs::DistSort::swp(pr, lpos[k], rpos[k]);
+    wave_lds_sync();
+    return __builtin_amdgcn_readfirstlane(cut);
+}
+
+__global__ __launch_bounds__(64) void k_read_graph_ties(
+    const int32_t* __restrict__ sim, const int32_t* __restrict__ diff, const int64_t* __restrict__ ctg_out_off,
+    const int32_t* __restrict__ ctg_n, const int32_t* __restrict__ win_contig, const int64_t* __restrict__ win_mask_off,
+    const int32_t* __restrict__ mask_ids, const int32_t* __restrict__ row_win, const int64_t* __restrict__ win_bits_off,
+    float below, int cap, int max_n, unsigned long long* __restrict__ bits, unsigned long long* __restrict__ amb_head ,
+    const int32_t* __restrict__ amb_rows, int amb_cap, int es, const int32_t* __restrict__ pos_rank, const int64_t* __restrict__ rank_off) {
+    extern __shared__ unsigned char s_dyn[];
+    const int lane = lane_id();
+    hs::DistPair* __restrict__ pr = reinterpret_cast<hs::DistPair*>(s_dyn);
+    int* __restrict__ lpos = reinterpret_cast<int*>(pr + max_n); int* __restrict__ rpos = lpos + max_n;
+    float* __restrict__ dv = reinterpret_cast<float*>(rpos + max_n);
+    int* __restrict__ tv = reinterpret_cast<int*>(dv + cap);
+    int* __restrict__ st_first = tv + cap; int* __restrict__ st_last = st_first + 40; int* __restrict__ st_depth = st_first + 80;
+    const unsigned long long listed = amb_head[0];
+    const int n_list = (int)(listed < (unsigned long long)amb_cap ? listed : (unsigned long long)amb_cap);
+    for (int k = (int)blockIdx.x; k < n_list; k += (int)gridDim.x) {
+        const int row = amb_rows[k];
+        const int w = row_win[row];
+        const int64_t m0 = win_mask_off[w];
+        const int m = (int)(win_mask_off[w + 1] - m0);
+        const int i = row - (int)m0;
+        const int c = win_contig[w];
+        const int N = ctg_n[c];
+        if (m > cap || N < 2 || !(below >= 0.f) || N > max_n) { if (lane == 0) atomicAdd(&amb_head[1], 1ull); continue; }
+        const int32_t* __restrict__ ids = mask_ids + m0;
+        const int r1 = ids[i];
+        const int32_t* __restrict__ prk = pos_rank ? pos_rank + rank_off[c] : nullptr;
+        const int r1k = prk ? prk[r1] : r1;
+        const int32_t* __restrict__ srow = sim + (ctg_out_off[c] + (int64_t)r1k * N) * es;
+        const int32_t* __restrict__ drow = diff + (ctg_out_off[c] + (int64_t)r1k * N) * es;
+        wave_lds_sync();
+        (void)graph_row_distances<false>(srow, drow, ids, prk, es, m, r1, lane, dv, tv);
+        const RowCut rc = graph_row_cut(dv, m, N, lane, below);
+        if (!rc.ambiguous) { graph_row_link(dv, m, i, lane, below, rc.above, rc.cut, bits + win_bits_off[w]); continue; }
+        const float tied = rc.tied;
+        for (int r = lane; r < N; r += 64) { pr[r].first = r; pr[r].second = 0.f; }
+        wave_lds_sync();
+        for (int j = lane; j < m; j += 64) pr[ids[j]].second = dv[j];
+        int lg = 0;
+        for (int v = N; v > 1; v >>= 1) lg++;
+        if (lane == 0) { st_first[0] = 0; st_last[0] = N; st_depth[0] = 2 * lg; }
+        wave_lds_sync();
+        int sp = 1;
+        while (sp > 0) {
+            --sp;
+            const int first = st_first[sp];
+            int last = st_last[sp], depth = st_depth[sp];
+            while (last - first > 16) {
+                bool has = false;
+                for (int p = first + lane; p < last; p += 64) has |= pr[p].second == tied;
+                if (__ballot(has) == 0ull) break;
+                if (depth == 0) { if (lane == 0) hs::DistSort::heap_sort(pr, first, last); break; }
+                --depth;
+                const int cut = wave_partition_pivot(pr, first, last, lane, lpos, rpos);
+                if (sp < 40) { if (lane == 0) { st_first[sp] = cut; st_last[sp] = last; st_depth[sp] = depth; } ++sp; }
+                last = cut;
+                wave_lds_sync();
             }
-        } else if (r != r1 && s > 0) {
-            const float df = (float)(dd - 1 > 0 ? dd - 1 : 0);
-            d = 1.f - df / (float)(s + dd);
-            if (s > max_compat) max_compat = s;
-        }
-        dv[j] = d; tv[j] = r != r1 ? s + dd : 0x7fffffff;
-    }
-    max_compat = wave_max_i32(max_compat);
-    const double thr = 0.7 * (double)max_compat;
-    for (int j = lane; j < m; j += 64) {
-        if ((double)tv[j] < thr) dv[j] = 0.f;
-        if (LM && dv[j] != dv[j]) nan_l = true;
-    }
-    wave_lds_sync();
-    if (LM && __ballot(nan_l) != 0ull) { give_up(); return; }
-
-    const int extra_zeros = N - m;
-    float s0, s1; int c0, ones = 0;
-    {
-        float best = 0.f;
-        for (int j = lane; j < m; j += 64) { const float d = dv[j]; if (d > best) best = d; if (d == 1.f) ones++; }
-        s0 = wave_max_f01(best);
-        ones = wave_sum_i32(ones);
-        int cnt = 0; float second = -1.f;
-        for (int j = lane; j < m; j += 64) { const float d = dv[j]; if (d == s0) cnt++; else if (d > second) second = d; }
-        c0 = wave_sum_i32(cnt) + (s0 == 0.f ? extra_zeros : 0);
-        if (extra_zeros > 0 && s0 > 0.f && second < 0.f) second = 0.f;
-        const int key = second < 0.f ? -1 : __float_as_int(second);
-        const int kmax = wave_max_i32(key);
-        s1 = c0 >= 2 ? s0 : (kmax < 0 ? -1.f : __int_as_float(kmax));
-    }
-    float above = s0 - (s0 - s1) * 3;
-    if (above == 1.f && ones < N) {
-        const int idx = (ones + 4) < (N - 1) ? (ones + 4) : (N - 1);
-        int k = idx - ones;
-        float cur = 2.f, v = 0.f; int cc = 0;
-        for (int it = 0; it < 5; ++it) {
-            next_level<0>(dv, m, lane, cur, below, above, extra_zeros, &v, &cc);
-            if (cc == 0) { v = 0.f; break; }
-            if (k < cc) break;
-            k -= cc; cur = v;
-        }
-        above = v;
-    }
-    const int mw64 = (m + 63) >> 6;
-    unsigned long long* __restrict__ wb = bits + win_bits_off[w];
-    int nA = 0;
-    for (int j = lane; j < m; j += 64) { const float d = dv[j]; if (d > below && (d == 1.f || d >= above)) nA++; }
-    nA = wave_sum_i32(nA);
-    float cut = 3.f;
-    if (nA < 5) {
-        const int need = 5 - nA;
-        int nB = 0;
-        for (int j = lane; j < m; j += 64) { const float d = dv[j]; if (d > below && d != 1.f && d < above) nB++; }
-        nB = wave_sum_i32(nB);
-        if (nB > 0 && nB <= need) cut = -1.f;
-        else if (nB > need) {
-            int remaining = need; float cur = 2.f, v = 0.f; int cc = 0;
-            bool ambiguous = false;
-            for (int it = 0; it < 5; ++it) {
-                next_level<1>(dv, m, lane, cur, below, above, 0, &v, &cc);
-                if (remaining <= cc) { ambiguous = remaining != cc; break; }
-                remaining -= cc; cur = v;
+            wave_lds_sync();
+        }
+        unsigned long long* __restrict__ wb = bits + win_bits_off[w];
+        graph_row_link(dv, m, i, lane, below, rc.above, __int_as_float(__float_as_int(tied) + 1), wb);
+        const int mw64 = (m + 63) >> 6;
+        int remaining = rc.remaining;
+        for (int base = 0; base < N && remaining > 0; base += 64) {
+            const int p = base + lane;
+            const bool t = p < N && pr[p].second == tied;
+            const unsigned long long bal = __ballot(t);
+            const int before = __popcll(bal & ((1ull << lane) - 1ull));
+            if (t && before < remaining) {
+                const int r = pr[p].first;
+                int lo = 0, hi = m;
+                while (lo < hi) { const int mid = (lo + hi) >> 1; if (ids[mid] < r) lo = mid + 1; else hi = mid; }
+                const int j = lo;
+                if (j < m) {
+                    atomicOr(&wb[(int64_t)i * mw64 + (j >> 6)], 1ull << (j & 63));
+                    atomicOr(&wb[(int64_t)j * mw64 + (i >> 6)], 1ull << (i & 63));
+                }
             }
-            if (ambiguous) { give_up(); return; }
-            cut = v;
-        }
-    }
-    for (int j = lane; j < m; j += 64) {
-        const float d = dv[j];
-        const bool take = d > below && ((d == 1.f || d >= above) || (d != 1.f && d < above && d >= cut));
-        if (take) {
-            atomicOr(&wb[(int64_t)i * mw64 + (j >> 6)], 1ull << (j & 63));
-            atomicOr(&wb[(int64_t)j * mw64 + (i >> 6)], 1ull << (i & 63));
+            remaining -= __popcll(bal);
         }
     }
 }
diff --git a/hairsplitter_amd/csrc/hs_rh8.h b/hairsplitter_amd/csrc/hs_rh8.h
--- a/hairsplitter_amd/csrc/hs_rh8.h
+++ b/hairsplitter_amd/csrc/hs_rh8.h
@@ -177,23 +177,24 @@
     }
 };
 
-struct CountSort {
-    static HS_HD bool comp(uint32_t a, uint32_t b) { return (a >> 8) > (b >> 8); }
-    static HS_HD void swp(uint32_t* a, int i, int j) { const uint32_t t = a[i]; a[i] = a[j]; a[j] = t; }
-    static HS_HD void unguarded_linear_insert(uint32_t* a, int last) {
-        const uint32_t val = a[last];
+template <class T, class Comp>
+struct IntroSort {
+    static HS_HD bool comp(const T& a, const T& b) { return Comp()(a, b); }
+    static HS_HD void swp(T* a, int i, int j) { const T t = a[i]; a[i] = a[j]; a[j] = t; }
+    static HS_HD void unguarded_linear_insert(T* a, int last) {
+        const T val = a[last];
         int next = last - 1;
         while (comp(val, a[next])) { a[last] = a[next]; last = next; --next; }
         a[last] = val;
     }
-    static HS_HD void insertion_sort(uint32_t* a, int first, int last) {
+    static HS_HD void insertion_sort(T* a, int first, int last) {
         if (first == last) return;
         for (int i = first + 1; i != last; ++i) {
-            if (comp(a[i], a[first])) { const uint32_t val = a[i]; for (int j = i; j > first; --j) a[j] = a[j - 1]; a[first] = val; }
+            if (comp(a[i], a[first])) { const T val = a[i]; for (int j = i; j > first; --j) a[j] = a[j - 1]; a[first] = val; }
             else unguarded_linear_insert(a, i);
         }
     }
-    static HS_HD void adjust_heap(uint32_t* a, int first, int hole, int len, uint32_t value) {
+    static HS_HD void adjust_heap(T* a, int first, int hole, int len, T value) {
         const int top = hole;
         int child = hole;
         while (child < (len - 1) / 2) {
@@ -211,19 +212,19 @@
         while (hole > top && comp(a[first + parent], value)) { a[first + hole] = a[first + parent]; hole = parent; parent = (hole - 1) / 2; }
         a[first + hole] = value;
     }
-    static HS_HD void heap_sort(uint32_t* a, int first, int last) {
+    static HS_HD void heap_sort(T* a, int first, int last) {
         const int len = last - first;
         if (len >= 2) {
             for (int parent = (len - 2) / 2;; --parent) { adjust_heap(a, first, parent, len, a[first + parent]); if (parent == 0) break; }
         }
         while (last - first > 1) {
             --last;
-            const uint32_t value = a[last];
+            const T value = a[last];
             a[last] = a[first];
             adjust_heap(a, first, 0, last - first, value);
         }
     }
-    static HS_HD int partition_pivot(uint32_t* a, int first, int last) {
+    static HS_HD void median_to_first(T* a, int first, int last) {
         const int mid = first + (last - first) / 2;
         const int x = first + 1, y = mid, z = last - 1;
         if (comp(a[x], a[y])) {
@@ -233,6 +234,9 @@
         } else if (comp(a[x], a[z])) swp(a, first, x);
         else if (comp(a[y], a[z])) swp(a, first, z);
         else swp(a, first, y);
+    }
+    static HS_HD int partition_pivot(T* a, int first, int last) {
+        median_to_first(a, first, last);
         int lo = first + 1, hi = last;
         for (;;) {
             while (comp(a[lo], a[first])) ++lo;
@@ -243,8 +247,21 @@
             ++lo;
         }
     }
-    static HS_HD void sort(uint32_t* a, int n) { int stack[120]; sort_with_stack(a, n, stack); }
-    static HS_HD void sort_with_stack(uint32_t* a, int n, int* stack) {
+    static HS_HD int partition_pivot_by_ranks(T* a, int first, int last, int* lpos, int* rpos) {
+        median_to_first(a, first, last);
+        const T piv = a[first];
+        int nl = 0, nr = 0;
+        for (int q = first + 1; q < last; ++q) if (!comp(a[q], piv)) lpos[nl++] = q;
+        for (int q = last - 1; q >= first; --q) if (!comp(piv, a[q])) rpos[nr++] = q;
+        int s = 0;
+        while (s < nl && s < nr && lpos[s] < rpos[s]) ++s;
+        for (int k = 0; k < s; ++k) swp(a, lpos[k], rpos[k]);
+        int cut = s < nl ? lpos[s] : last;
+        if (s > 0 && rpos[s - 1] < cut) cut = rpos[s - 1];
+        return cut;
+    }
+    static HS_HD void sort(T* a, int n) { int stack[120]; sort_with_stack(a, n, stack); }
+    static HS_HD void loop_phase(T* a, int n, int* stack, int* ranks = nullptr) {
         if (n <= 0) return;
         int lg = 0;
         for (int v = n; v > 1; v >>= 1) lg++;
@@ -258,14 +275,25 @@
             while (last - first > 16) {
                 if (depth == 0) { heap_sort(a, first, last); break; }
                 --depth;
-                const int cut = partition_pivot(a, first, last);
+                const int cut = ranks ? partition_pivot_by_ranks(a, first, last, ranks, ranks + n) : partition_pivot(a, first, last);
                 if (sp < 40) { st_first[sp] = cut; st_last[sp] = last; st_depth[sp] = depth; ++sp; }
                 last = cut;
             }
         }
+    }
+    static HS_HD void sort_with_stack(T* a, int n, int* stack) {
+        if (n <= 0) return;
+        loop_phase(a, n, stack);
         if (n > 16) { insertion_sort(a, 0, 16); for (int i = 16; i < n; ++i) unguarded_linear_insert(a, i); }
         else insertion_sort(a, 0, n);
     }
 };
 
+struct CountGreater { HS_HD bool operator()(uint32_t a, uint32_t b) const { return (a >> 8) > (b >> 8); } };
+struct CountSort : IntroSort<uint32_t, CountGreater> {};
+
+struct DistPair { int32_t first; float second; };
+struct DistGreater { HS_HD bool operator()(const DistPair& a, const DistPair& b) const { return a.second > b.second; } };
+struct DistSort : IntroSort<DistPair, DistGreater> {};
+
 }
diff --git a/hairsplitter_amd/csrc/hs_sr_backend.inc b/hairsplitter_amd/csrc/hs_sr_backend.inc
--- a/hairsplitter_amd/csrc/hs_sr_backend.inc
+++ b/hairsplitter_amd/csrc/hs_sr_backend.inc
@@ -18,6 +18,9 @@
     int64_t stage_cap = 0, stage_hint = 0;
     EventPair ev;
     bool timed = false, begun = false;
+    bool dev_ties = false, pending = false;
+    int k6_cap = 0, max_len = 1;
+    float below = 0;
     const int32_t* d_sim = nullptr; const int32_t* d_diff = nullptr; int es = 1;
     std::vector<int64_t> ctg_out_off; std::vector<int32_t> ctg_n;
     float* k_ms = nullptr;
@@ -25,9 +28,13 @@
 
 struct PlaneRows { const uint64_t* d_alt = nullptr; const uint64_t* d_ref = nullptr; const int64_t* d_plane_off = nullptr; const int32_t* d_words = nullptr; };
 
+static bool graph_ties_on_host() { const char* e = std::getenv("HS_GRAPH_TIES"); return e && !std::strcmp(e, "host"); }
+static int graph_ties_max_n() { const char* e = std::getenv("HS_GRAPH_TIES_MAX_N"); return e ? std::max(0, std::atoi(e)) : 0x7fffffff; }
+
 static int graph_rows_begin(const int32_t* d_sim, const int32_t* d_diff, const std::vector<int64_t>& ctg_out_off, const std::vector<int32_t>& ctg_n_matrix,
                             const hs::SrWindowSet& ws, GraphRows& G, hipStream_t stream, float* k_ms, KernelClock* kc = nullptr,
-                            const PlaneRows* planes = nullptr, int es = 1 ) {
+                            const PlaneRows* planes = nullptr, int es = 1 ,
+                            bool ties_on_host = false) {
     G.ctg_n = ws.ctg_reads.empty() ? ctg_n_matrix : ws.ctg_reads;
     G.ctg_out_off = ctg_out_off;
     const std::vector<int32_t>& ctg_n = G.ctg_n;
@@ -41,6 +48,8 @@
     const int rows_dev = (int)ws.win_row0[(size_t)Wd];
     const int rows_mx = (int)ws.win_row0[(size_t)Wmx];
     G.rows_dev = rows_dev; G.Wd = Wd; G.Wmx = Wmx; G.rows_mx = rows_mx;
+    G.dev_ties = !ties_on_host && !graph_ties_on_host() && Wmx == Wd && rows == rows_dev && rows_mx > 0;
+    G.pending = false;
     if (Wmx < Wd && (!planes || !planes->d_alt)) { set_error("read graphs: low-memory windows without bit rows"); return HS_EINVAL; }
     if ((int64_t)ws.host_off.size() != (int64_t)(rows - rows_dev) + 1 && rows != rows_dev) { set_error("read graphs: host rows do not match the window set"); return HS_EINVAL; }
     std::vector<int32_t>& row_win = G.row_win; row_win.assign((size_t)rows_dev, 0);
@@ -92,20 +101,22 @@
         const size_t bits_bytes = ((size_t)win_bits_off.back() * 8 + 15) & ~(size_t)15;
         if (int rc = G.d_bits.alloc(std::max<size_t>(bits_bytes, 16))) return rc;
         G.amb_cap = (size_t)rows_dev;
-        G.stage_cap = std::max<int64_t>(G.stage_hint + G.stage_hint / 2, 64 * (int64_t)max_len);
+        G.stage_cap = G.dev_ties ? 0 : std::max<int64_t>(G.stage_hint + G.stage_hint / 2, 64 * (int64_t)max_len);
+        G.max_len = max_len;
         const size_t amb_bytes = 16 + (((size_t)G.amb_cap * 4 + 15) & ~(size_t)15) + (((size_t)G.amb_cap * 8 + 15) & ~(size_t)15);
         if (int rc = G.d_amb.alloc(amb_bytes)) return rc;
-        if (int rc = G.d_stage.alloc((size_t)G.stage_cap * 8 + 32)) return rc;
+        if (!G.dev_ties) { if (int rc = G.d_stage.alloc((size_t)G.stage_cap * 8 + 32)) return rc; }
         hipLaunchKernelGGL(hsdev::k_fill16, dim3((unsigned)std::min<size_t>(256, bits_bytes / 4096 + 1)), dim3(256), 0, stream, G.d_bits.as<uint4>(), (long long)(std::max<size_t>(bits_bytes, 16) / 16), 0u);
         hipLaunchKernelGGL(hsdev::k_fill16, dim3(1), dim3(64), 0, stream, G.d_amb.as<uint4>(), 1ll, 0u);
         unsigned long long* amb_head = G.d_amb.as<unsigned long long>();
         int32_t* amb_rows = reinterpret_cast<int32_t*>((char*)G.d_amb.p + 16);
         long long* amb_so = reinterpret_cast<long long*>((char*)G.d_amb.p + 16 + (((size_t)G.amb_cap * 4 + 15) & ~(size_t)15));
-        int32_t* st_sim = G.d_stage.as<int32_t>(); int32_t* st_diff = st_sim + (((size_t)G.stage_cap + 3) & ~(size_t)3);
+        int32_t* st_sim = G.dev_ties ? nullptr : G.d_stage.as<int32_t>(); int32_t* st_diff = G.dev_ties ? nullptr : st_sim + (((size_t)G.stage_cap + 3) & ~(size_t)3);
         int cap = ((max_m_dev + 63) / 64) * 64, waves = 4;
         if ((size_t)cap * 8 * 4 > 57344) waves = 1;
         if ((size_t)cap * 8 > 57344) cap = 7168;
         const float below = 1 - ws.error_rate * 2;
+        G.k6_cap = cap; G.below = below;
         HS_HIP(ev_rec(G.ev.a, stream));
         if (rows_mx > 0) {
             if (kc) { if (int rc = kc->begin(HS_K_GRAPH_ROWS, stream)) return rc; }
@@ -141,6 +152,7 @@
         }
         HS_HIP(ev_rec(G.ev.b, stream));
         G.timed = true;
+        if (G.dev_ties) return HS_OK;
         const size_t rows_part = ((size_t)G.amb_cap * 4 + 15) & ~(size_t)15, stage_half = (((size_t)G.stage_cap + 3) & ~(size_t)3) * 4;
         if (int rc = G.h_amb.alloc(amb_bytes + 2 * stage_half + 64)) return rc;
         Shipment sh;
@@ -165,7 +177,20 @@
     const std::vector<int32_t>& row_win = G.row_win;
     const std::vector<int64_t>& win_bits_off = G.win_bits_off;
     const std::vector<int64_t>& win_mat_off = G.win_mat_off;
-    if (rows_dev > 0) {
+    if (rows_dev > 0 && G.dev_ties) {
+        const int max_n = std::max(0, std::min(std::min(G.max_len, graph_ties_max_n()), (int)((96 * 1024 - 480 - (int64_t)G.k6_cap * 8) / 16)));
+        const size_t lds = (size_t)max_n * 16 + (size_t)G.k6_cap * 8 + 480;
+        if (lds > 48 * 1024)
+            HS_HIP(hipFuncSetAttribute(reinterpret_cast<const void*>(hsdev::k_read_graph_ties), hipFuncAttributeMaxDynamicSharedMemorySize, (int)lds));
+        if (kc) { if (int rc = kc->begin(HS_K_GRAPH_ROWS, stream)) return rc; }
+        hipLaunchKernelGGL(hsdev::k_read_graph_ties, dim3((unsigned)std::min(rows_mx, 256)), dim3(64), lds, stream, G.d_sim, G.d_diff, G.d_oo.as<int64_t>(), G.d_n.as<int32_t>(),
+                           G.d_wc.as<int32_t>(), G.d_row0.as<int64_t>(), G.d_ids.as<int32_t>(), G.d_rw.as<int32_t>(), G.d_bo.as<int64_t>(), G.below, G.k6_cap, max_n,
+                           G.d_bits.as<unsigned long long>(), G.d_amb.as<unsigned long long>(), reinterpret_cast<const int32_t*>((char*)G.d_amb.p + 16), (int)G.amb_cap, G.es,
+                           G.by_pos ? G.d_pos_rank.as<int32_t>() : nullptr, G.d_rank_off.as<int64_t>());
+        HS_HIP(hipGetLastError());
+        if (kc) { if (int rc = kc->end(0, stream)) return rc; }
+        G.pending = true;
+    } else if (rows_dev > 0) {
         if (int rc = stream_wait(stream)) return rc;
         const size_t rows_part = ((size_t)G.amb_cap * 4 + 15) & ~(size_t)15, amb_bytes = 16 + rows_part + (((size_t)G.amb_cap * 8 + 15) & ~(size_t)15), stage_half = (((size_t)G.stage_cap + 3) & ~(size_t)3) * 4;
         const char* hb = (const char*)G.h_amb.p;
@@ -264,6 +289,8 @@
             }
         } else if (std::getenv("HS_TIMING") && Wmx < Wd)
             std::fprintf(stderr, "[hs timing] sr: low-memory path on the device: %d windows, %d rows, none resolved on the host\n", Wd - Wmx, rows_dev - rows_mx);
+    }
+    if (rows_dev > 0) {
         if (kc) { if (int rc = kc->begin(HS_K_GRAPH_CSR, stream)) return rc; }
         hipLaunchKernelGGL(hsdev::k_read_graph_degrees, dim3((rows_dev + 255) / 256), dim3(256), 0, stream, G.d_bits.as<unsigned long long>(), G.d_rw.as<int32_t>(),
                            G.d_row0.as<int64_t>(), G.d_bo.as<int64_t>(), rows_dev, G.d_deg.as<int32_t>());
@@ -321,6 +348,25 @@
     }
     return HS_OK;
 }
+static int graph_rows_check(const hs::SrWindowSet& ws, GraphRows& G, hipStream_t stream, const unsigned long long* head, int64_t* rows_on_host, KernelClock* kc, bool* redone) {
+    *redone = false;
+    if (!G.pending) return HS_OK;
+    G.pending = false;
+    if (head[0] > (unsigned long long)G.amb_cap) { set_error("read graphs: more undecided rows than rows"); return HS_EINVAL; }
+    if (head[1] == 0) {
+        if (rows_on_host) *rows_on_host = (int64_t)head[0];
+        G.stage_hint = std::max<int64_t>(G.stage_hint, (int64_t)head[0] * G.max_len);
+        return HS_OK;
+    }
+    if (std::getenv("HS_TIMING")) std::fprintf(stderr, "[hs timing] sr: %llu of %llu tied graph rows left to the host: the graphs are built again\n", head[1], head[0]);
+    const std::vector<int64_t> oo = G.ctg_out_off; const std::vector<int32_t> cn = G.ctg_n;
+    if (kc) kc->flush();
+    if (G.timed) { G.timed = false; float m = 0; if (int rc = G.ev.ms(&m)) return rc; if (G.k_ms) *G.k_ms += m; }
+    if (int rc = graph_rows_begin(G.d_sim, G.d_diff, oo, cn, ws, G, stream, G.k_ms, kc, nullptr, G.es, true)) return rc;
+    if (int rc = graph_rows_end(ws, G, stream, rows_on_host, kc)) return rc;
+    *redone = true;
+    return HS_OK;
+}
 static int graph_rows_settle(GraphRows& G, KernelClock* kc) {
     if (kc) kc->flush();
     if (G.timed) { G.timed = false; float m = 0; if (int rc = G.ev.ms(&m)) return rc; if (G.k_ms) *G.k_ms += m; }
@@ -331,6 +377,21 @@
                             const PlaneRows* planes = nullptr, int es = 1) {
     if (int rc = graph_rows_begin(d_sim, d_diff, ctg_out_off, ctg_n_matrix, ws, G, stream, k_ms, kc, planes, es)) return rc;
     if (int rc = graph_rows_end(ws, G, stream, rows_on_host, kc)) return rc;
+    if (G.pending) {
+        HBuf h;
+        if (int rc = h.alloc(64)) return rc;
+        Shipment sh;
+        sh.add(h.p, G.d_amb.p, 16);
+        sh.add((char*)h.p + 16, G.d_off.as<int64_t>() + (G.rows & ~(int64_t)1), 16);
+        if (int rc = sh.launch(stream, 1)) return rc;
+        if (int rc_w = stream_wait(stream)) return rc_w;
+        bool redone = false;
+        if (int rc = graph_rows_check(ws, G, stream, (const unsigned long long*)h.p, rows_on_host, kc, &redone)) return rc;
+        if (!redone) {
+            if (!G.total_exact) { G.total = ((const int64_t*)((const char*)h.p + 16))[G.rows & 1]; G.total_exact = true; }
+            return graph_rows_settle(G, kc);
+        }
+    }
     if (G.rows > 0 && !G.total_exact) { int64_t t = 0; if (int rc = d2h_pinned(&t, G.d_off.as<int64_t>() + G.rows, 8, stream)) return rc; G.total = t; G.total_exact = true; }
     else if (int rc_w = stream_wait(stream)) return rc_w;
     return graph_rows_settle(G, kc);
@@ -496,11 +557,32 @@
         if (keep) G.stage_hint = keep->stage_hint;
         return graph_rows_begin(d_sim.as<int32_t>(), d_diff.as<int32_t>(), sd_out_off, sd_n, ws, G, stream, k_ms, &kc, &pr, 2);
     }
+    const hs::SrWindowSet* ws_pending = nullptr;
+    int64_t tied_rows = 0;
     int build_graphs_end(const hs::SrWindowSet& ws, int64_t* rows_on_host) override {
-        const int rc = graph_rows_end(ws, G, stream, rows_on_host, &kc);
+        const int rc = graph_rows_end(ws, G, stream, &tied_rows, &kc);
+        if (!rc && !G.pending) k5_waited = true;
+        ws_pending = G.pending ? &ws : nullptr;
+        if (rows_on_host) *rows_on_host = tied_rows;
+        if (keep) keep->stage_hint = G.stage_hint;
+        return rc;
+    }
+    int check_graphs(const unsigned long long* head, bool* redone) {
+        const int rc = graph_rows_check(*ws_pending, G, stream, head, &tied_rows, &kc, redone);
+        ws_pending = nullptr;
         if (!rc) k5_waited = true;
         if (keep) keep->stage_hint = G.stage_hint;
         return rc;
+    }
+    int build_graphs_settle(int64_t* rows_on_host) override {
+        if (G.pending) {
+            unsigned long long head[2] = {0, 0};
+            if (int rc = d2h_pinned(head, G.d_amb.p, 16, stream)) return rc;
+            bool redone = false;
+            if (int rc = check_graphs(head, &redone)) return rc;
+        }
+        if (rows_on_host) *rows_on_host = tied_rows;
+        return HS_OK;
     }
     int fetch_graphs(std::vector<int64_t>& off, std::vector<int32_t>& nbr) override {
         if (G.rows > 0 && !G.total_exact) { int64_t t = 0; if (int rc = d2h_pinned(&t, G.d_off.as<int64_t>() + G.rows, 8, stream)) return rc; G.total = t; G.total_exact = true; }
@@ -519,6 +601,13 @@
     void tap_chain(std::vector<int64_t>* run_off, std::vector<int32_t>* run_labels) override { tap_run_off = run_off; tap_run_labels = run_labels; }
     int cw_chain(const hs::CwChain& ch, std::vector<int32_t>& labels, std::vector<int32_t>& final_labels, std::vector<uint8_t>& final_ok,
                  float k_ms[3], hs::SrChainStats* stats) override {
+        bool redo = false;
+        if (int rc = cw_chain_once(ch, labels, final_labels, final_ok, k_ms, stats, &redo)) return rc;
+        return redo ? cw_chain_once(ch, labels, final_labels, final_ok, k_ms, stats, &redo) : HS_OK;
+    }
+    int cw_chain_once(const hs::CwChain& ch, std::vector<int32_t>& labels, std::vector<int32_t>& final_labels, std::vector<uint8_t>& final_ok,
+                      float k_ms[3], hs::SrChainStats* stats, bool* redo) {
+        *redo = false;
         if (int rc = settle_simdiff()) return rc;
         const int Wc = (int)ch.win.size();
         const int64_t n_inst = (int64_t)ch.seed_col.size();
@@ -698,11 +787,13 @@
         HS_HIP(ev_rec(e2.b, stream));
         {
             HBuf h, h4;
-            const size_t o_nnz = 416, o_final = 512, o_ok = o_final + (((size_t)total_m * 4 + 255) & ~(size_t)255);
+            const size_t o_nnz = 416, o_head = 448, o_final = 512, o_ok = o_final + (((size_t)total_m * 4 + 255) & ~(size_t)255);
             if (int rc = h4.alloc(o_ok + (size_t)Wc + 256)) return rc;
             Shipment sh;
             sh.add(h4.p, d_stat.p, 416);
             sh.add((char*)h4.p + o_nnz, G.d_off.as<int64_t>() + (G.rows & ~(int64_t)1), 16);
+            const bool head_pending = G.pending;
+            if (head_pending) sh.add((char*)h4.p + o_head, G.d_amb.p, 16);
             bool need_chain_labels = !finish || tap_run_labels != nullptr;
             if (finish) {
                 sh.add((char*)h4.p + o_final, d_final.p, (size_t)total_m * sizeof(int32_t));
@@ -712,6 +803,10 @@
             if (int rc = sh.launch(stream, 64)) return rc;
             if (int rc = kc.end(0, stream)) return rc;
             if (int rc = stream_wait(stream)) return rc;
+            if (head_pending) {
+                if (int rc = check_graphs((const unsigned long long*)((const char*)h4.p + o_head), redo)) return rc;
+                if (*redo) return HS_OK;
+            }
             if (finish) {
                 final_labels.resize((size_t)total_m); final_ok.resize((size_t)Wc);
                 std::memcpy(final_labels.data(), (const char*)h4.p + o_final, (size_t)total_m * sizeof(int32_t));
```
